# mmp/pbrt-v1

Hardware: AMD Instinct MI355X
Metric: Mrays/s (primary+secondary: every Scene::Intersect + Scene::IntersectP) (higher is better)
Workload: dtype f32

## Files before the change

include/pbrt_hip.h:

```cpp
#ifndef PBRT_HIP_H
#define PBRT_HIP_H
#include <stdint.h>
#include <stddef.h>
#ifdef __cplusplus
extern "C" {
#endif

#define RT_OK 0
#define RT_EINVAL (-1)
#define RT_EDEVICE (-2)
#define RT_ESTATE (-3)
#define RT_ENOMEM (-4)

typedef struct RtScene RtScene;

enum { RT_MAT_MATTE = 0, RT_MAT_MIRROR = 1, RT_MAT_GLASS = 2, RT_MAT_PLASTIC = 3, RT_MAT_UBER = 4, RT_MAT_SHINYMETAL = 5, RT_MAT_TRANSLUCENT = 6 };
typedef struct RtMaterial {
    int32_t type;
    float kd[3];
    float kt[3];
    float sigma;
    float ior;
    float ks[3];
    float roughness;
    float kr[3];
} RtMaterial;

enum { RT_LIGHT_POINT = 0, RT_LIGHT_AREA = 1, RT_LIGHT_SPOT = 2, RT_LIGHT_DISTANT = 3, RT_LIGHT_INFINITE = 4 };
typedef struct RtLight {
    int32_t type;
    float color[3];
    float pos[3];
    int32_t n_samples;
    uint32_t first_tri;
    uint32_t n_tris;
    int32_t reverse_orientation;
    int32_t flip_normal;
    float dir[3];
    float world_to_light[9];
    float cos_total_width, cos_falloff_start;
    int32_t quadric_plus1;
} RtLight;

enum { RT_CAMERA_PERSPECTIVE = 0, RT_CAMERA_ORTHOGRAPHIC = 1, RT_CAMERA_ENVIRONMENT = 2 };
typedef struct RtCamera {
    float raster_to_camera[16];
    float camera_to_world[16];
    float lens_radius, focal_distance, hither, yon;
    float shutter_open, shutter_close;
    int32_t type;
    int32_t x_res, y_res;
} RtCamera;

typedef struct RtVolume {
    int32_t present;
    float world_to_volume[16];
    float p0[3], p1[3];
    float sigma_a[3], sigma_s[3], le[3];
    float g;
} RtVolume;

enum { RT_DENSITY_NONE = 0, RT_DENSITY_EXPONENTIAL = 1, RT_DENSITY_GRID = 2 };
typedef struct RtDensityRegion {
    int32_t kind;
    float a, b;
    float updir[3];
    int32_t nx, ny, nz;
    const float *density;
} RtDensityRegion;

enum { RT_ACCEL_KDTREE = 0, RT_ACCEL_GRID = 1 };
typedef struct RtAccelParams {
    int32_t kind;
    int32_t isect_cost, trav_cost, max_prims, max_depth;
    float empty_bonus;
    int32_t build_threads;
} RtAccelParams;

enum { RT_QUADRIC_SPHERE = 0, RT_QUADRIC_DISK = 1, RT_QUADRIC_CYLINDER = 2, RT_QUADRIC_CONE = 3, RT_QUADRIC_PARABOLOID = 4, RT_QUADRIC_HYPERBOLOID = 5 };
typedef struct RtQuadric {
    int32_t type;
    float object_to_world[16], world_to_object[16];
    float radius, zmin, zmax, theta_min, theta_max, phi_max;
    float p1[3], p2[3], a, c;
} RtQuadric;

enum { RT_SHADING_UV = 1, RT_SHADING_N = 2, RT_SHADING_S = 4 };
typedef struct RtTriShading {
    uint32_t flags;
    uint32_t xform;
    float uv[6];
    float n[9];
    float s[9];
} RtTriShading;

typedef struct RtSceneDesc {
    uint32_t n_tris;
    const float *tri_verts;
    const uint16_t *tri_material;
    const int32_t *tri_light;
    const uint8_t *tri_flags;
    uint32_t n_materials;
    const RtMaterial *materials;
    uint32_t n_lights;
    const RtLight *lights;
    uint32_t n_light_tris;
    const float *light_tris;
    RtCamera camera;
    RtVolume volume;
    RtAccelParams accel;
    uint32_t n_quadrics;
    const RtQuadric *quadrics;
    const int32_t *tri_shading;
    uint32_t n_shading;
    const RtTriShading *shading;
    uint32_t n_xforms;
    const float *xforms;
} RtSceneDesc;

enum { RT_INTEGRATOR_WHITTED = 0, RT_INTEGRATOR_DIRECT = 1, RT_INTEGRATOR_PATH = 2 };
enum { RT_STRATEGY_ALL = 0, RT_STRATEGY_ONE = 1, RT_STRATEGY_WEIGHTED = 2 };
enum { RT_VOLUME_NONE = 0, RT_VOLUME_EMISSION = 1, RT_VOLUME_SINGLE = 2 };
enum { RT_SAMPLER_STRATIFIED = 0, RT_SAMPLER_LOWDISCREPANCY = 1, RT_SAMPLER_RANDOM = 2 };

typedef struct RtRenderDesc {
    int32_t integrator, max_depth, strategy;
    int32_t volume_integrator;
    float step_size;
    int32_t sampler, x_samples, y_samples, jitter, pixel_samples;
    uint32_t seed;
    int32_t x_res, y_res;
    int32_t x_pixel_start, y_pixel_start, x_pixel_count, y_pixel_count;
    int32_t x_start, x_end, y_start, y_end;
    float filter_x_width, filter_y_width;
    float filter_table[256];
    int32_t shard_index, shard_count, tile_pixels;
} RtRenderDesc;

typedef struct RtCounters {
    uint64_t camera_rays;
    uint64_t closest_rays;
    uint64_t any_rays;
    uint64_t nodes_visited;
    uint64_t leaf_refs;
    uint64_t tri_tests;
    uint64_t bad_samples;
    uint64_t stack_overflows;
} RtCounters;

typedef struct RtRay { float o[3], d[3], mint, maxt; } RtRay;
typedef struct RtHit { int32_t prim; float t, b1, b2; } RtHit;
typedef struct RtAccelInfo {
    uint32_t n_nodes, n_leaf_refs, max_depth, n_tris;
    float bounds[6];
    double build_seconds;
    int32_t kind;
    int32_t grid_nvoxels[3];
    float grid_width[3], grid_inv_width[3];
} RtAccelInfo;

const char *rt_last_error(void);
int rt_device_count(int *count);

int rt_scene_create(const RtSceneDesc *desc, int device, RtScene **out);
typedef struct RtPrebuiltAccel {
    int32_t kind;
    uint32_t n_nodes, n_leaf_refs, max_depth;
    const uint32_t *nodes;
    const uint32_t *leaf_refs;
    float bounds[6];
    int32_t grid_nvoxels[3]; float grid_width[3], grid_inv_width[3];
} RtPrebuiltAccel;
int rt_scene_create_prebuilt(const RtSceneDesc *desc, int device, const RtPrebuiltAccel *accel, RtScene **out);
int rt_scene_set_density(RtScene *s, const RtDensityRegion *region);
int rt_scene_destroy(RtScene *s);
int rt_scene_set_stream(RtScene *s, void *hip_stream);
int rt_scene_accel_info(const RtScene *s, RtAccelInfo *info);
int rt_scene_accel_copy(const RtScene *s, uint32_t *nodes, uint32_t *leaf_refs);

typedef struct RtKdTree RtAccel;
int rt_accel_build(const float *tri_verts, uint32_t n_tris, const RtAccelParams *params, RtAccel **out);
int rt_accel_info(const RtAccel *t, RtAccelInfo *info);
int rt_accel_copy(const RtAccel *t, uint32_t *nodes, uint32_t *leaf_refs);
typedef struct RtLeafLayoutInfo { uint64_t n_nodes, n_slots, n_entries; uint32_t stride, pad; } RtLeafLayoutInfo;
int rt_accel_leaf_layout(const RtAccel *t, int runs, int copies, uint32_t *tnodes, uint32_t *slot_prim, uint32_t *entries, RtLeafLayoutInfo *info);
int rt_accel_destroy(RtAccel *t);
typedef struct RtKdTree RtKdTree;
int rt_kdtree_build(const float *tri_verts, uint32_t n_tris, const RtAccelParams *params, RtKdTree **out);
int rt_kdtree_info(const RtKdTree *t, RtAccelInfo *info);
int rt_kdtree_copy(const RtKdTree *t, uint32_t *nodes, uint32_t *leaf_refs);
int rt_kdtree_destroy(RtKdTree *t);

int rt_camera_rays(RtScene *s, const RtRenderDesc *rd, uint64_t first, uint32_t count, RtRay *rays_out);
int rt_trace_closest(RtScene *s, const RtRay *rays, uint32_t n, RtHit *hits_out);
int rt_trace_any(RtScene *s, const RtRay *rays, uint32_t n, uint8_t *occluded_out);

int rt_film_bind(RtScene *s, void *device_accum, int32_t x_pixel_count, int32_t y_pixel_count);
int rt_film_clear(RtScene *s);
int rt_film_read(RtScene *s, float *host_accum);
int rt_film_resolve(RtScene *s, int premultiply_alpha, float *rgb_out, float *alpha_out);

int rt_render(RtScene *s, const RtRenderDesc *rd);
int rt_sync(RtScene *s);
int rt_samples_read(RtScene *s, uint64_t first, uint64_t count, float *out);
int rt_counters(RtScene *s, RtCounters *out);
int rt_counters_reset(RtScene *s);
int rt_set_counting(RtScene *s, int enabled);
int rt_last_render_ms(RtScene *s, float *total_ms, float *kernel_ms);
typedef struct RtRenderStats {
    float total_ms, render_ms, trace_ms, gather_ms;
    int32_t pipeline, iterations, timed_iterations;
    uint32_t slots;
    float shade_ms;
    int32_t bands;
    float march_ms;
    uint64_t weighted_points;
    float weighted_ms[5];
} RtRenderStats;
int rt_film_resolve_device(RtScene *s, const float *dev_accum, uint64_t n, int premultiply, float *dev_rgb, float *dev_alpha);
int rt_film_resolve_device_rgba(RtScene *s, const float *dev_accum, uint64_t n, int premultiply, float *dev_rgba);
int rt_film_pack_parts(RtScene *s, const float *dev_accum, int32_t w, int32_t h, int32_t world, int32_t rows, float *dev_parts);
int rt_last_render_stats(RtScene *s, RtRenderStats *out);

#ifdef __cplusplus
}
#endif
#endif
```

pbrt-v1_amd/__init__.py:

```python
from __future__ import annotations

import ctypes as C
import os
import subprocess
import numpy as np

_HERE = os.path.dirname(os.path.abspath(__file__))
LIB_DIR = os.path.join(_HERE, "lib")
HIP_LIB = os.path.join(LIB_DIR, "libpbrt_hip.so")
if os.environ.get("PBRT_HIP_TUNE") and os.environ.get("PBRT_HIP_LIB_PATH"):
    HIP_LIB = os.environ["PBRT_HIP_LIB_PATH"]
HOST_LIB = os.path.join(LIB_DIR, "libpbrt_host.so")
CSRC = os.path.join(_HERE, "csrc")

HIPCC_FLAGS = ["--offload-arch=gfx950", "-O3", "-std=c++17", "-ffp-contract=off", "-fno-slp-vectorize", "-fPIC", "-shared",
               "-Wno-unused-value"]
HOST_FLAGS = ["-O2", "-std=c++17", "-fPIC", "-shared", "-msse2", "-mfpmath=sse", "-fvisibility=hidden", "-fvisibility-inlines-hidden"]


HIP_UNITS = ("rt_kernels.hip", "rt_scene.hip", "rt_film.hip", "rt_trace.hip", "rt_mega_w.hip", "rt_mega_d.hip", "rt_mega_dw.hip", "rt_mega_p.hip", "rt_pipe_w.hip", "rt_pipe_d.hip",
             "rt_pipe_p.hip", "rt_pipe_v.hip", "rt_march.hip", "kd_build.cpp", "grid_build.cpp", "leaf_layout.cpp")


def build(force: bool = False, verbose: bool = False, defines=(), jobs: int | None = None) -> None:
    from concurrent.futures import ThreadPoolExecutor
    os.makedirs(LIB_DIR, exist_ok=True)
    obj_dir = os.path.join(LIB_DIR, "obj")
    os.makedirs(obj_dir, exist_ok=True)
    hip_dir = os.path.join(CSRC, "hip")
    hip_dep = [os.path.join(hip_dir, f) for f in os.listdir(hip_dir)] + [os.path.join(_HERE, "..", "include", "pbrt_hip.h")]
    headers = [d for d in hip_dep if d.endswith((".h", ".inc"))]
    host_src = [os.path.join(CSRC, "host", "scene_api.cpp")]
    host_dep = [os.path.join(CSRC, "host", f) for f in os.listdir(os.path.join(CSRC, "host"))] + \
               [os.path.join(_HERE, "..", "include", f) for f in ("pbrt_hip.h", "pbrt_hip_desc.h", "pbrt_hip_plugin.h", "pbrt_hip_material.h")]

    def stale(out, deps):
        return force or not os.path.exists(out) or any(os.path.getmtime(d) > os.path.getmtime(out) for d in deps)

    def closure(path, seen=None):
        import re
        seen = set() if seen is None else seen
        if path in seen or not os.path.exists(path):
            return seen
        seen.add(path)
        for inc in re.findall(r'^\s*#\s*include\s+"([^"]+)"', open(path).read(), re.M):
            closure(os.path.normpath(os.path.join(os.path.dirname(path), inc)), seen)
        return seen

    stamp = os.path.join(obj_dir, "defines.txt")
    dtext = " ".join(HIPCC_FLAGS) + " | " + " ".join(HOST_FLAGS) + " | " + " ".join(defines)
    if (open(stamp).read() if os.path.exists(stamp) else "") != dtext:
        force = True
    todo = []
    for u in HIP_UNITS:
        obj = os.path.join(obj_dir, u.rsplit(".", 1)[0] + ".o")
        if stale(obj, sorted(closure(os.path.join(hip_dir, u)))):
            todo.append(["hipcc"] + [f for f in HIPCC_FLAGS if f != "-shared"] + list(defines) + ["-c", os.path.join(hip_dir, u), "-o", obj])
    if todo:
        def run(cmd):
            if verbose:
                print(" ".join(cmd))
            if not cmd[-3].endswith(".hip"):
                subprocess.check_call(cmd)
                return
            r = subprocess.run(cmd + ["-Rpass-analysis=kernel-resource-usage"], capture_output=True, text=True)
            keep = [ln for ln in r.stderr.splitlines() if "remark:" in ln and any(k in ln for k in ("Function Name", " VGPRs:", "VGPRs Spill", "Occupancy", "ScratchSize", "LDS Size"))]
            open(cmd[-1][:-2] + ".resources.txt", "w").write("\n".join(keep) + "\n")
            if r.returncode != 0:
                raise RuntimeError("hipcc failed:\n" + r.stderr[-4000:])
        with ThreadPoolExecutor(max_workers=jobs or min(len(todo), os.cpu_count() or 4)) as ex:
            list(ex.map(run, todo))
        open(stamp, "w").write(dtext)
    objs = [os.path.join(obj_dir, u.rsplit(".", 1)[0] + ".o") for u in HIP_UNITS]
    if stale(HIP_LIB, objs):
        cmd = ["hipcc", "--offload-arch=gfx950", "-shared", "-fPIC"] + objs + ["-o", HIP_LIB]
        if verbose:
            print(" ".join(cmd))
        subprocess.check_call(cmd)
    if stale(HOST_LIB, host_dep):
        cmd = ["g++"] + HOST_FLAGS + host_src + ["-Wl,--version-script=" + os.path.join(CSRC, "host", "exports.map"), "-ldl", "-o", HOST_LIB]
        if verbose:
            print(" ".join(cmd))
        subprocess.check_call(cmd)


class RtCounters(C.Structure):
    _fields_ = [(n, C.c_uint64) for n in ("camera_rays", "closest_rays", "any_rays", "nodes_visited", "leaf_refs",
                                          "tri_tests", "bad_samples", "stack_overflows")]

    def as_dict(self):
        return {n: int(getattr(self, n)) for n, _ in self._fields_}


class RtAccelInfo(C.Structure):
    _fields_ = [("n_nodes", C.c_uint32), ("n_leaf_refs", C.c_uint32), ("max_depth", C.c_uint32), ("n_tris", C.c_uint32),
                ("bounds", C.c_float * 6), ("build_seconds", C.c_double), ("kind", C.c_int32),
                ("grid_nvoxels", C.c_int32 * 3), ("grid_width", C.c_float * 3), ("grid_inv_width", C.c_float * 3)]


class RtLeafLayoutInfo(C.Structure):
    _fields_ = [("n_nodes", C.c_uint64), ("n_slots", C.c_uint64), ("n_entries", C.c_uint64), ("stride", C.c_uint32), ("pad", C.c_uint32)]


class RtPrebuiltAccel(C.Structure):
    _fields_ = [("kind", C.c_int32), ("n_nodes", C.c_uint32), ("n_leaf_refs", C.c_uint32), ("max_depth", C.c_uint32),
                ("nodes", C.c_void_p), ("leaf_refs", C.c_void_p), ("bounds", C.c_float * 6),
                ("grid_nvoxels", C.c_int32 * 3), ("grid_width", C.c_float * 3), ("grid_inv_width", C.c_float * 3)]


class RtRenderStats(C.Structure):
    _fields_ = [("total_ms", C.c_float), ("render_ms", C.c_float), ("trace_ms", C.c_float), ("gather_ms", C.c_float),
                ("pipeline", C.c_int32), ("iterations", C.c_int32), ("timed_iterations", C.c_int32), ("slots", C.c_uint32), ("shade_ms", C.c_float), ("bands", C.c_int32), ("march_ms", C.c_float),
                ("weighted_points", C.c_uint64), ("weighted_ms", C.c_float * 5)]

    def as_dict(self):
        return {n: (list(getattr(self, n)) if n == "weighted_ms" else getattr(self, n)) for n, _ in self._fields_}


class RtVolume(C.Structure):
    _fields_ = [("present", C.c_int32), ("world_to_volume", C.c_float * 16), ("p0", C.c_float * 3), ("p1", C.c_float * 3),
                ("sigma_a", C.c_float * 3), ("sigma_s", C.c_float * 3), ("le", C.c_float * 3), ("g", C.c_float)]


class RtDensityRegion(C.Structure):
    _fields_ = [("kind", C.c_int32), ("a", C.c_float), ("b", C.c_float), ("updir", C.c_float * 3),
                ("nx", C.c_int32), ("ny", C.c_int32), ("nz", C.c_int32), ("density", C.POINTER(C.c_float))]


RT_MATERIAL_NAMES = ("matte", "mirror", "glass", "plastic", "uber", "shinymetal", "translucent")


class RtMaterial(C.Structure):
    _fields_ = [("type", C.c_int32), ("kd", C.c_float * 3), ("kt", C.c_float * 3), ("sigma", C.c_float), ("ior", C.c_float),
                ("ks", C.c_float * 3), ("roughness", C.c_float), ("kr", C.c_float * 3)]


class RtMaterialLobes(C.Structure):
    _fields_ = [(n, C.c_float * 3) for n in ("eta_ks", "eta_kr", "r_kd", "t_kd", "r_ks", "t_ks")] + \
               [(n, C.c_int32) for n in ("has_dr", "has_dt", "has_gr", "has_gt")]


RT_DENSITY_NAMES = {1: "exponential", 2: "volumegrid"}

RT_LIGHT_NAMES = ("point", "area", "spot", "distant", "infinite")


class RtLight(C.Structure):
    _fields_ = [("type", C.c_int32), ("color", C.c_float * 3), ("pos", C.c_float * 3), ("n_samples", C.c_int32), ("first_tri", C.c_uint32),
                ("n_tris", C.c_uint32), ("reverse_orientation", C.c_int32), ("flip_normal", C.c_int32), ("dir", C.c_float * 3),
                ("world_to_light", C.c_float * 9), ("cos_total_width", C.c_float), ("cos_falloff_start", C.c_float), ("quadric_plus1", C.c_int32)]

RAY_DTYPE = np.dtype([("o", np.float32, 3), ("d", np.float32, 3), ("mint", np.float32), ("maxt", np.float32)])
HIT_DTYPE = np.dtype([("prim", np.int32), ("t", np.float32), ("b1", np.float32), ("b2", np.float32)])

_hip = None
_host = None


def code_id(path: str | None = None) -> str:
    import hashlib, struct
    data = open(path or HIP_LIB, "rb").read()
    if data[:4] != b"\x7fELF" or data[4] != 2:
        raise RuntimeError("not a 64-bit ELF file: " + (path or HIP_LIB))
    shoff, = struct.unpack_from("<Q", data, 0x28)
    shentsize, shnum, shstrndx = struct.unpack_from("<HHH", data, 0x3A)
    def sh(i):
        name, typ, flags, addr, off, size = struct.unpack_from("<IIQQQQ", data, shoff + i * shentsize)
        return name, off, size
    _, stroff, _ = sh(shstrndx)
    h = hashlib.sha256()
    found = False
    for i in range(shnum):
        name, off, size = sh(i)
        end = data.index(b"\0", stroff + name)
        if data[stroff + name:end] == b".hip_fatbin":
            h.update(data[off:off + size]); found = True
    if not found:
        raise RuntimeError("no .hip_fatbin section in " + (path or HIP_LIB))
    return h.hexdigest()[:16]


def hip_lib():
    global _hip
    if _hip is None:
        if not os.path.exists(HIP_LIB):
            raise RuntimeError("libpbrt_hip.so is not built (run __graft_entry__.build()); there is no CPU fallback")
        L = C.CDLL(HIP_LIB)
        L.rt_last_error.restype = C.c_char_p
        for name in ("rt_scene_create", "rt_scene_destroy", "rt_scene_set_stream", "rt_scene_accel_info",
                     "rt_scene_accel_copy", "rt_camera_rays", "rt_trace_closest", "rt_trace_any", "rt_film_bind",
                     "rt_film_clear", "rt_film_read", "rt_film_resolve", "rt_render", "rt_sync", "rt_counters",
                     "rt_counters_reset", "rt_last_render_ms", "rt_last_render_stats", "rt_samples_read", "rt_device_count", "rt_set_counting",
                     "rt_kdtree_build", "rt_kdtree_info", "rt_kdtree_copy", "rt_kdtree_destroy",
                     "rt_accel_build", "rt_accel_info", "rt_accel_copy", "rt_accel_destroy", "rt_scene_create_prebuilt", "rt_film_resolve_device",
                     "rt_film_resolve_device_rgba", "rt_film_pack_parts", "rt_accel_leaf_layout", "rt_scene_set_density"):
            getattr(L, name).restype = C.c_int
        L.rt_scene_create.argtypes = [C.c_void_p, C.c_int, C.POINTER(C.c_void_p)]
        L.rt_scene_set_density.argtypes = [C.c_void_p, C.c_void_p]
        L.rt_scene_create_prebuilt.argtypes = [C.c_void_p, C.c_int, C.POINTER(RtPrebuiltAccel), C.POINTER(C.c_void_p)]
        L.rt_scene_destroy.argtypes = [C.c_void_p]
        L.rt_scene_set_stream.argtypes = [C.c_void_p, C.c_void_p]
        L.rt_scene_accel_info.argtypes = [C.c_void_p, C.POINTER(RtAccelInfo)]
        L.rt_scene_accel_copy.argtypes = [C.c_void_p, C.c_void_p, C.c_void_p]
        L.rt_camera_rays.argtypes = [C.c_void_p, C.c_void_p, C.c_uint64, C.c_uint32, C.c_void_p]
        L.rt_trace_closest.argtypes = [C.c_void_p, C.c_void_p, C.c_uint32, C.c_void_p]
        L.rt_trace_any.argtypes = [C.c_void_p, C.c_void_p, C.c_uint32, C.c_void_p]
        L.rt_film_bind.argtypes = [C.c_void_p, C.c_void_p, C.c_int32, C.c_int32]
        L.rt_film_clear.argtypes = [C.c_void_p]
        L.rt_film_read.argtypes = [C.c_void_p, C.c_void_p]
        L.rt_film_resolve.argtypes = [C.c_void_p, C.c_int, C.c_void_p, C.c_void_p]
        L.rt_render.argtypes = [C.c_void_p, C.c_void_p]
        L.rt_film_resolve_device.argtypes = [C.c_void_p, C.c_void_p, C.c_uint64, C.c_int, C.c_void_p, C.c_void_p]
        L.rt_film_resolve_device_rgba.argtypes = [C.c_void_p, C.c_void_p, C.c_uint64, C.c_int, C.c_void_p]
        L.rt_film_pack_parts.argtypes = [C.c_void_p, C.c_void_p, C.c_int32, C.c_int32, C.c_int32, C.c_int32, C.c_void_p]
        L.rt_sync.argtypes = [C.c_void_p]
        L.rt_counters.argtypes = [C.c_void_p, C.POINTER(RtCounters)]
        L.rt_counters_reset.argtypes = [C.c_void_p]
        L.rt_last_render_ms.argtypes = [C.c_void_p, C.POINTER(C.c_float), C.POINTER(C.c_float)]
        L.rt_last_render_stats.argtypes = [C.c_void_p, C.POINTER(RtRenderStats)]
        L.rt_samples_read.argtypes = [C.c_void_p, C.c_uint64, C.c_uint64, C.c_void_p]
        L.rt_device_count.argtypes = [C.POINTER(C.c_int)]
        L.rt_set_counting.argtypes = [C.c_void_p, C.c_int]
        L.rt_kdtree_build.argtypes = [C.c_void_p, C.c_uint32, C.c_void_p, C.POINTER(C.c_void_p)]
        L.rt_kdtree_info.argtypes = [C.c_void_p, C.POINTER(RtAccelInfo)]
        L.rt_kdtree_copy.argtypes = [C.c_void_p, C.c_void_p, C.c_void_p]
        L.rt_kdtree_destroy.argtypes = [C.c_void_p]
        L.rt_accel_build.argtypes = [C.c_void_p, C.c_uint32, C.c_void_p, C.POINTER(C.c_void_p)]
        L.rt_accel_info.argtypes = [C.c_void_p, C.POINTER(RtAccelInfo)]
        L.rt_accel_copy.argtypes = [C.c_void_p, C.c_void_p, C.c_void_p]
        L.rt_accel_destroy.argtypes = [C.c_void_p]
        L.rt_accel_leaf_layout.argtypes = [C.c_void_p, C.c_int, C.c_int, C.c_void_p, C.c_void_p, C.c_void_p, C.POINTER(RtLeafLayoutInfo)]
        _hip = L
    return _hip


def host_lib():
    global _host
    if _host is None:
        if not os.path.exists(HOST_LIB):
            raise RuntimeError("libpbrt_host.so is not built (run __graft_entry__.build())")
        L = C.CDLL(HOST_LIB)
        L.pbrt_host_parse_file.restype = C.c_void_p
        L.pbrt_host_parse_file.argtypes = [C.c_char_p, C.c_int]
        L.pbrt_host_parse_string.restype = C.c_void_p
        L.pbrt_host_parse_string.argtypes = [C.c_char_p, C.c_int]
        L.pbrt_host_free.argtypes = [C.c_void_p]
        L.pbrt_host_frame_count.argtypes = [C.c_void_p]
        L.pbrt_host_frame_valid.argtypes = [C.c_void_p, C.c_int]
        L.pbrt_host_scene_desc.restype = C.c_void_p
        L.pbrt_host_scene_desc.argtypes = [C.c_void_p, C.c_int]
        L.pbrt_host_render_desc.restype = C.c_void_p
        L.pbrt_host_render_desc.argtypes = [C.c_void_p, C.c_int]
        L.pbrt_host_premultiply.argtypes = [C.c_void_p, C.c_int]
        L.pbrt_host_filename.restype = C.c_char_p
        L.pbrt_host_filename.argtypes = [C.c_void_p, C.c_int]
        L.pbrt_host_set_shard.argtypes = [C.c_void_p, C.c_int, C.c_int, C.c_int]
        L.pbrt_host_set_seed.argtypes = [C.c_void_p, C.c_uint]
        L.pbrt_host_film_dims.argtypes = [C.c_void_p, C.POINTER(C.c_int * 8)]
        L.pbrt_host_scene_counts.argtypes = [C.c_void_p, C.POINTER(C.c_uint * 4)]
        L.pbrt_host_camera.restype = C.POINTER(C.c_float)
        L.pbrt_host_camera.argtypes = [C.c_void_p]
        L.pbrt_host_tri_verts.restype = C.POINTER(C.c_float)
        L.pbrt_host_tri_verts.argtypes = [C.c_void_p]
        L.pbrt_host_write_exr.argtypes = [C.c_char_p, C.c_void_p, C.c_void_p] + [C.c_int] * 6
        L.pbrt_host_read_exr_info.argtypes = [C.c_char_p, C.POINTER(C.c_int * 6)]
        L.pbrt_host_read_exr.argtypes = [C.c_char_p, C.c_void_p, C.c_void_p]
        L.pbrt_host_format_f32.restype = C.c_longlong
        L.pbrt_host_format_f32.argtypes = [C.c_void_p, C.c_longlong, C.c_int, C.c_void_p, C.c_longlong]
        L.pbrt_host_format_iota.restype = C.c_longlong
        L.pbrt_host_format_iota.argtypes = [C.c_longlong, C.c_longlong, C.c_int, C.c_void_p, C.c_longlong]
        L.pbrt_host_accel_params.restype = C.c_void_p
        L.pbrt_host_accel_params.argtypes = [C.c_void_p]
        L.pbrt_host_volume.restype = C.POINTER(RtVolume)
        L.pbrt_host_volume.argtypes = [C.c_void_p]
        L.pbrt_host_density_desc.restype = C.POINTER(RtDensityRegion)
        L.pbrt_host_density_desc.argtypes = [C.c_void_p, C.c_int]
        L.pbrt_host_materials.restype = C.POINTER(RtMaterial)
        L.pbrt_host_materials.argtypes = [C.c_void_p]
        L.pbrt_host_material_lobes.argtypes = [C.POINTER(RtMaterial), C.POINTER(RtMaterialLobes)]
        L.pbrt_host_lights.restype = C.POINTER(RtLight)
        L.pbrt_host_lights.argtypes = [C.c_void_p]
        _host = L
    return _host


def write_exr(path, rgb, alpha, total_res=None, offset=(0, 0)):
    rgb = np.ascontiguousarray(rgb, np.float32); alpha = np.ascontiguousarray(alpha, np.float32)
    h, w = alpha.shape
    tw, th = total_res if total_res else (w, h)
    if host_lib().pbrt_host_write_exr(path.encode(), rgb.ctypes.data, alpha.ctypes.data, w, h, tw, th, offset[0], offset[1]) != 0:
        raise IOError("cannot write " + path)


def read_exr(path):
    info = (C.c_int * 6)()
    if host_lib().pbrt_host_read_exr_info(path.encode(), C.byref(info)) != 0:
        raise IOError("cannot read " + path)
    w, h = info[0], info[1]
    rgb = np.zeros((h, w, 3), np.float32); alpha = np.zeros((h, w), np.float32)
    host_lib().pbrt_host_read_exr(path.encode(), rgb.ctypes.data, alpha.ctypes.data)
    return rgb, alpha, dict(total_res=(info[2], info[3]), offset=(info[4], info[5]))


TRI_SHADING_DTYPE = np.dtype([("flags", np.uint32), ("xform", np.uint32), ("uv", np.float32, 6), ("n", np.float32, 9), ("s", np.float32, 9)])


def shading_records(parsed):
    H = host_lib()
    H.pbrt_host_shading.restype = C.c_int
    H.pbrt_host_shading.argtypes = [C.c_void_p, C.POINTER(C.c_void_p), C.POINTER(C.c_void_p), C.POINTER(C.c_void_p), C.POINTER(C.c_uint), C.POINTER(C.c_uint)]
    idx, rec, xf, nrec, nxf = C.c_void_p(), C.c_void_p(), C.c_void_p(), C.c_uint(), C.c_uint()
    H.pbrt_host_shading(parsed.scene_desc, C.byref(idx), C.byref(rec), C.byref(xf), C.byref(nrec), C.byref(nxf))
    if not idx.value:
        return None, np.zeros(0, TRI_SHADING_DTYPE), np.zeros((0, 32), np.float32)
    i = np.ctypeslib.as_array(C.cast(idx, C.POINTER(C.c_int32)), shape=(parsed.n_tris,)).copy()
    r = np.frombuffer(C.string_at(rec, nrec.value * TRI_SHADING_DTYPE.itemsize), TRI_SHADING_DTYPE).copy()
    x = np.ctypeslib.as_array(C.cast(xf, C.POINTER(C.c_float)), shape=(nxf.value, 32)).copy() if nxf.value else np.zeros((0, 32), np.float32)
    return i, r, x


def format_f32(values, per_line: int = 9) -> str:
    v = np.ascontiguousarray(values, np.float32).ravel()
    buf = C.create_string_buffer(int(v.size) * 17 + 64)
    n = host_lib().pbrt_host_format_f32(v.ctypes.data, v.size, per_line, buf, len(buf))
    if n < 0:
        raise RuntimeError("format_f32: buffer too small")
    return buf.raw[:n].decode()


def format_iota(first: int, count: int, per_line: int = 3) -> str:
    buf = C.create_string_buffer(int(count) * 12 + 64)
    n = host_lib().pbrt_host_format_iota(first, count, per_line, buf, len(buf))
    if n < 0:
        raise RuntimeError("format_iota: buffer too small")
    return buf.raw[:n].decode()


def assemble_exr(paths, out) -> float:
    H = host_lib()
    H.pbrt_host_assemble_exr.restype = C.c_float
    H.pbrt_host_assemble_exr.argtypes = [C.c_char_p, C.c_char_p]
    r = H.pbrt_host_assemble_exr("\n".join(paths).encode(), out.encode())
    if r < 0:
        raise IOError("cannot assemble " + out)
    return float(r)


def publish_accel(ds: "DeviceScene", path: str) -> None:
    info = ds.accel_info()
    need = 256 + 8 * int(info.n_nodes) + 4 * int(info.n_leaf_refs)
    st = os.statvfs(os.path.dirname(path) or ".")
    if st.f_bavail * st.f_frsize < need + (64 << 20):
        raise OSError("publish_accel: %s has %d MB free, the accelerator needs %d MB" % (os.path.dirname(path), st.f_bavail * st.f_frsize >> 20, need >> 20))
    nodes, refs = ds.accel_arrays()
    tmp = path + ".tmp%d" % os.getpid()
    try:
        with open(tmp, "wb") as f:
            f.write(bytes(info).ljust(256, b"\0"))
            np.ascontiguousarray(nodes, np.uint32).tofile(f); np.ascontiguousarray(refs, np.uint32).tofile(f)
        os.replace(tmp, path)
    except BaseException:
        if os.path.exists(tmp):
            os.remove(tmp)
        raise


def attach_accel(path: str):
    raw = np.memmap(path, dtype=np.uint8, mode="r")
    info = RtAccelInfo.from_buffer_copy(bytes(raw[:C.sizeof(RtAccelInfo)]))
    nodes = np.frombuffer(raw, np.uint32, count=2 * info.n_nodes, offset=256).reshape(-1, 2)
    refs = np.frombuffer(raw, np.uint32, count=info.n_leaf_refs, offset=256 + 8 * info.n_nodes)
    return nodes, refs, info


class RtError(RuntimeError):
    pass


def _chk(rc):
    if rc != 0:
        raise RtError("rt error %d: %s" % (rc, hip_lib().rt_last_error().decode()))


def device_count() -> int:
    n = C.c_int(0)
    rc = hip_lib().rt_device_count(C.byref(n))
    return int(n.value) if rc == 0 else 0


def build_kdtree(tri_verts: np.ndarray, accel_params_ptr=None):
    tv = np.ascontiguousarray(tri_verts, np.float32).reshape(-1, 9)
    t = C.c_void_p()
    _chk(hip_lib().rt_accel_build(tv.ctypes.data, len(tv), accel_params_ptr, C.byref(t)))
    info = RtAccelInfo()
    _chk(hip_lib().rt_accel_info(t, C.byref(info)))
    nodes = np.zeros((info.n_nodes, 2), np.uint32)
    refs = np.zeros(max(info.n_leaf_refs, 1), np.uint32)
    _chk(hip_lib().rt_accel_copy(t, nodes.ctypes.data, refs.ctypes.data))
    hip_lib().rt_accel_destroy(t)
    return nodes, refs[:info.n_leaf_refs], np.array(list(info.bounds), np.float32), info


def leaf_layout(tri_verts: np.ndarray, accel_params_ptr=None, runs: bool = False, copies: bool = False):
    tv = np.ascontiguousarray(tri_verts, np.float32).reshape(-1, 9)
    t = C.c_void_p()
    _chk(hip_lib().rt_accel_build(tv.ctypes.data, len(tv), accel_params_ptr, C.byref(t)))
    try:
        info = RtAccelInfo()
        _chk(hip_lib().rt_accel_info(t, C.byref(info)))
        nodes = np.zeros((info.n_nodes, 2), np.uint32)
        refs = np.zeros(max(info.n_leaf_refs, 1), np.uint32)
        _chk(hip_lib().rt_accel_copy(t, nodes.ctypes.data, refs.ctypes.data))
        li = RtLeafLayoutInfo()
        _chk(hip_lib().rt_accel_leaf_layout(t, int(runs), int(copies), None, None, None, C.byref(li)))
        tn = np.zeros((li.n_nodes, 2), np.uint32); sp = np.zeros(max(li.n_slots, 1), np.uint32); en = np.zeros(max(li.n_entries, 1), np.uint32)
        _chk(hip_lib().rt_accel_leaf_layout(t, int(runs), int(copies), tn.ctypes.data, sp.ctypes.data, en.ctypes.data, C.byref(li)))
    finally:
        hip_lib().rt_accel_destroy(t)
    return nodes, refs[:info.n_leaf_refs], tn, sp[:li.n_slots], en[:li.n_entries], int(li.stride)


def fit_tile(extent: int, size: int) -> int:
    best = None
    for t in range(max(1, size * 3 // 4), max(2, size * 5 // 4) + 1):
        pad = -(-extent // t) * t - extent
        key = (pad, abs(t - size))
        if best is None or key < best[0]:
            best = (key, t)
    return best[1]


class ParsedScene:

    def __init__(self, text: str | None = None, path: str | None = None, quiet: bool = True, frame: int = 0):
        H = host_lib()
        if path is not None:
            self._h = H.pbrt_host_parse_file(path.encode(), int(quiet))
        else:
            from . import scenes as _scenes
            text = _scenes.for_product(text)
            self._h = H.pbrt_host_parse_string(text.encode(), int(quiet))
        self.warnings = H.pbrt_host_warnings()
        self.errors = H.pbrt_host_errors()
        self.n_frames = H.pbrt_host_frame_count(self._h)
        if self.n_frames == 0:
            raise RtError("scene description has no WorldEnd (errors: %d)" % self.errors)
        self.frame = frame
        self.valid = bool(H.pbrt_host_frame_valid(self._h, frame))
        self.scene_desc = H.pbrt_host_scene_desc(self._h, frame)
        self.render_desc = H.pbrt_host_render_desc(self._h, frame)
        self.premultiply = bool(H.pbrt_host_premultiply(self._h, frame))
        dims = (C.c_int * 8)()
        H.pbrt_host_film_dims(self.render_desc, C.byref(dims))
        self.width, self.height = dims[0], dims[1]
        self.sample_extent = (dims[2], dims[3], dims[4], dims[5])
        self.spp = dims[6]
        self.integrator = dims[7]
        cnt = (C.c_uint * 4)()
        H.pbrt_host_scene_counts(self.scene_desc, C.byref(cnt))
        self.n_tris, self.n_materials, self.n_lights, self.n_light_tris = (int(c) for c in cnt)

    @property
    def n_camera_samples(self) -> int:
        x0, x1, y0, y1 = self.sample_extent
        return (x1 - x0) * (y1 - y0) * self.spp

    def set_shard(self, index: int, count: int, tile_pixels=64, fit: bool = False):
        if isinstance(tile_pixels, (tuple, list)):
            w, h = int(tile_pixels[0]), int(tile_pixels[1])
            if fit:
                x0, x1, y0, y1 = self.sample_extent
                w, h = fit_tile(x1 - x0, w), fit_tile(y1 - y0, h)
            used = (w, h)
            tile_pixels = -(w | (h << 16))
        else:
            used = int(tile_pixels)
        host_lib().pbrt_host_set_shard(self.render_desc, index, count, int(tile_pixels))
        return used

    def set_seed(self, seed: int):
        host_lib().pbrt_host_set_seed(self.render_desc, seed)

    def camera_matrices(self):
        p = host_lib().pbrt_host_camera(self.scene_desc)
        a = np.ctypeslib.as_array(p, shape=(32,)).copy()
        return a[:16].reshape(4, 4), a[16:].reshape(4, 4)

    def accel_params_ptr(self):
        return host_lib().pbrt_host_accel_params(self.scene_desc)

    def accel_params(self) -> dict:
        a = np.ctypeslib.as_array(C.cast(self.accel_params_ptr(), C.POINTER(C.c_int32)), shape=(7,))
        return {"kind": int(a[0]), "isect_cost": int(a[1]), "trav_cost": int(a[2]), "max_prims": int(a[3]), "max_depth": int(a[4]),
                "empty_bonus": float(a[5:6].view(np.float32)[0]), "build_threads": int(a[6])}

    def render_view(self) -> dict:
        a = np.ctypeslib.as_array(C.cast(self.render_desc, C.POINTER(C.c_int32)), shape=(11,))
        return {"integrator": int(a[0]), "max_depth": int(a[1]), "strategy": int(a[2]), "volume_integrator": int(a[3]),
                "step_size": float(a[4:5].view(np.float32)[0]), "sampler": int(a[5]), "x_samples": int(a[6]), "y_samples": int(a[7]),
                "jitter": int(a[8]), "pixel_samples": int(a[9]), "seed": int(a[10:11].view(np.uint32)[0])}

    def volume(self) -> dict | None:
        v = host_lib().pbrt_host_volume(self.scene_desc).contents
        if not v.present:
            return None
        out = {"world_to_volume": np.array(v.world_to_volume, np.float32).reshape(4, 4), "p0": list(v.p0), "p1": list(v.p1),
               "sigma_a": list(v.sigma_a), "sigma_s": list(v.sigma_s), "le": list(v.le), "g": float(v.g), "density": None}
        dp = self.density_desc()
        if dp:
            d = dp.contents
            dens = {"kind": RT_DENSITY_NAMES[d.kind]}
            if d.kind == 1:
                dens.update(a=float(d.a), b=float(d.b), updir=[float(x) for x in d.updir])
            else:
                dens.update(nx=int(d.nx), ny=int(d.ny), nz=int(d.nz),
                            values=np.ctypeslib.as_array(d.density, shape=(d.nz, d.ny, d.nx)).copy())
            out["density"] = dens
        return out

    def materials(self) -> list:
        H = host_lib()
        tab = H.pbrt_host_materials(self.scene_desc)
        f3 = lambda a: np.array(list(a), np.float32)
        out = []
        for i in range(self.n_materials):
            m = tab[i]
            name = RT_MATERIAL_NAMES[m.type]
            d = {"type": name}
            if name == "matte":
                d.update(Kd=f3(m.kd), sigma=float(m.sigma))
            elif name == "mirror":
                d.update(Kr=f3(m.kd))
            elif name == "glass":
                d.update(Kr=f3(m.kd), Kt=f3(m.kt), index=float(m.ior))
            elif name == "plastic":
                d.update(Kd=f3(m.kd), Ks=f3(m.ks), roughness=float(m.roughness))
            elif name == "uber":
                d.update({"opacity*Kd": f3(m.kd), "opacity*Ks": f3(m.ks), "opacity*Kr": f3(m.kr), "1-opacity": f3(m.kt), "roughness": float(m.roughness)})
            else:
                lb = RtMaterialLobes()
                H.pbrt_host_material_lobes(C.byref(m), C.byref(lb))
                if name == "shinymetal":
                    d.update(Ks=f3(m.ks), Kr=f3(m.kr), roughness=float(m.roughness), eta_Ks=f3(lb.eta_ks), eta_Kr=f3(lb.eta_kr),
                             lobes=["glossy_reflection", "specular_reflection"])
                else:
                    d.update({"Kd": f3(m.kd), "Ks": f3(m.ks), "reflect": f3(m.kr), "transmit": f3(m.kt), "roughness": float(m.roughness),
                              "reflect*Kd": f3(lb.r_kd), "transmit*Kd": f3(lb.t_kd), "reflect*Ks": f3(lb.r_ks), "transmit*Ks": f3(lb.t_ks)})
                    d["lobes"] = [n for n, on in (("diffuse_reflection", lb.has_dr), ("diffuse_transmission", lb.has_dt),
                                                  ("glossy_reflection", lb.has_gr), ("glossy_transmission", lb.has_gt)) if on]
            out.append(d)
        return out

    def lights(self) -> list:
        tab = host_lib().pbrt_host_lights(self.scene_desc)
        f3 = lambda a: np.array(list(a), np.float32)
        out = []
        for i in range(self.n_lights):
            l = tab[i]
            name = RT_LIGHT_NAMES[l.type]
            d = {"type": name, "nsamples": int(l.n_samples), ("I" if name in ("point", "spot") else "L"): f3(l.color)}
            if name in ("point", "spot"):
                d["from"] = f3(l.pos)
            elif name == "distant":
                d["dir"] = f3(l.dir)
            elif name == "area":
                d["n_tris"] = int(l.n_tris)
            out.append(d)
        return out

    def density_desc(self):
        return host_lib().pbrt_host_density_desc(self._h, self.frame)

    def kdtree(self):
        return build_kdtree(self.tri_verts(), self.accel_params_ptr())

    def tri_verts(self):
        if self.n_tris == 0:
            return np.zeros((0, 3, 3), np.float32)
        p = host_lib().pbrt_host_tri_verts(self.scene_desc)
        return np.ctypeslib.as_array(p, shape=(self.n_tris, 3, 3)).copy()

    def serialize(self) -> bytes:
        H = host_lib()
        H.pbrt_host_serialize.restype = C.c_longlong
        H.pbrt_host_serialize.argtypes = [C.c_void_p, C.c_int, C.c_void_p, C.c_longlong]
        n = H.pbrt_host_serialize(self._h, self.frame, None, 0)
        buf = C.create_string_buffer(int(n))
        H.pbrt_host_serialize(self._h, self.frame, buf, n)
        return buf.raw

    def close(self):
        if self._h:
            host_lib().pbrt_host_free(self._h)
            self._h = None

    def __del__(self):
        try:
            self.close()
        except Exception:
            pass


class DeviceScene:

    def __init__(self, parsed: ParsedScene, device: int = -1, prebuilt=None):
        self.parsed = parsed
        self._s = C.c_void_p()
        if prebuilt is None:
            _chk(hip_lib().rt_scene_create(parsed.scene_desc, device, C.byref(self._s)))
        else:
            nodes, refs, info = prebuilt
            nodes = np.ascontiguousarray(nodes, np.uint32); refs = np.ascontiguousarray(refs if len(refs) else np.zeros(1, np.uint32), np.uint32)
            pa = RtPrebuiltAccel(kind=info.kind, n_nodes=info.n_nodes, n_leaf_refs=info.n_leaf_refs, max_depth=info.max_depth,
                                 nodes=nodes.ctypes.data, leaf_refs=refs.ctypes.data)
            for i in range(6): pa.bounds[i] = info.bounds[i]
            for i in range(3):
                pa.grid_nvoxels[i] = info.grid_nvoxels[i]; pa.grid_width[i] = info.grid_width[i]; pa.grid_inv_width[i] = info.grid_inv_width[i]
            _chk(hip_lib().rt_scene_create_prebuilt(parsed.scene_desc, device, C.byref(pa), C.byref(self._s)))
        dens = parsed.density_desc()
        if dens:
            rc = hip_lib().rt_scene_set_density(self._s, dens)
            if rc != 0:
                err = hip_lib().rt_last_error().decode(errors="replace")
                hip_lib().rt_scene_destroy(self._s); self._s = C.c_void_p()
                raise RtError("rt_scene_set_density failed (%d): %s" % (rc, err))
        self._film_bound = False

    def accel_info(self) -> RtAccelInfo:
        info = RtAccelInfo()
        _chk(hip_lib().rt_scene_accel_info(self._s, C.byref(info)))
        return info

    def accel_arrays(self):
        info = self.accel_info()
        nodes = np.zeros((info.n_nodes, 2), np.uint32)
        refs = np.zeros(max(info.n_leaf_refs, 1), np.uint32)
        _chk(hip_lib().rt_scene_accel_copy(self._s, nodes.ctypes.data, refs.ctypes.data))
        return nodes, refs[:info.n_leaf_refs]

    def set_stream(self, stream_ptr: int):
        _chk(hip_lib().rt_scene_set_stream(self._s, C.c_void_p(stream_ptr)))

    def bind_film(self, device_ptr: int | None = None):
        _chk(hip_lib().rt_film_bind(self._s, C.c_void_p(device_ptr) if device_ptr else None,
                                     self.parsed.width, self.parsed.height))
        self._film_bound = True

    def clear_film(self):
        _chk(hip_lib().rt_film_clear(self._s))

    def render(self, sync: bool = True):
        if not self._film_bound:
            self.bind_film()
        _chk(hip_lib().rt_render(self._s, self.parsed.render_desc))
        if sync:
            self.sync()

    def sync(self):
        _chk(hip_lib().rt_sync(self._s))

    def resolve_device(self, accum_ptr: int, n: int, rgb_ptr: int, alpha_ptr: int, premultiply: bool | None = None):
        pm = self.parsed.premultiply if premultiply is None else premultiply
        _chk(hip_lib().rt_film_resolve_device(self._s, C.c_void_p(accum_ptr), n, int(pm), C.c_void_p(rgb_ptr), C.c_void_p(alpha_ptr)))

    def resolve_device_rgba(self, accum_ptr: int, n: int, rgba_ptr: int, premultiply: bool | None = None):
        pm = self.parsed.premultiply if premultiply is None else premultiply
        _chk(hip_lib().rt_film_resolve_device_rgba(self._s, C.c_void_p(accum_ptr), n, int(pm), C.c_void_p(rgba_ptr)))

    def pack_parts(self, accum_ptr: int, world: int, rows: int, parts_ptr: int):
        _chk(hip_lib().rt_film_pack_parts(self._s, C.c_void_p(accum_ptr), self.parsed.width, self.parsed.height, world, rows, C.c_void_p(parts_ptr)))

    def film_accum(self) -> np.ndarray:
        out = np.zeros((5, self.parsed.height, self.parsed.width), np.float32)
        _chk(hip_lib().rt_film_read(self._s, out.ctypes.data))
        return out

    def film(self, premultiply: bool | None = None, out=None):
        h, w = self.parsed.height, self.parsed.width
        if out is None:
            rgb = np.empty((h, w, 3), np.float32); alpha = np.empty((h, w), np.float32)
        else:
            rgb, alpha = out
            if rgb.shape != (h, w, 3) or alpha.shape != (h, w) or rgb.dtype != np.float32 or alpha.dtype != np.float32 \
                    or not rgb.flags.c_contiguous or not alpha.flags.c_contiguous:
                raise ValueError("film(out=...): need C-contiguous float32 arrays of shape (H,W,3) and (H,W)")
        pm = self.parsed.premultiply if premultiply is None else premultiply
        _chk(hip_lib().rt_film_resolve(self._s, int(pm), rgb.ctypes.data, alpha.ctypes.data))
        return rgb, alpha

    def counters(self) -> dict:
        c = RtCounters()
        _chk(hip_lib().rt_counters(self._s, C.byref(c)))
        return c.as_dict()

    def set_counting(self, enabled: bool):
        _chk(hip_lib().rt_set_counting(self._s, int(enabled)))

    def reset_counters(self):
        _chk(hip_lib().rt_counters_reset(self._s))

    def last_ms(self):
        a, b = C.c_float(0), C.c_float(0)
        _chk(hip_lib().rt_last_render_ms(self._s, C.byref(a), C.byref(b)))
        return float(a.value), float(b.value)

    def samples(self, first: int = 0, count: int | None = None) -> np.ndarray:
        n = self.parsed.n_camera_samples - first if count is None else count
        out = np.zeros((n, 8), np.float32)
        _chk(hip_lib().rt_samples_read(self._s, first, n, out.ctypes.data))
        return out

    def last_stats(self) -> dict:
        st = RtRenderStats()
        _chk(hip_lib().rt_last_render_stats(self._s, C.byref(st)))
        return st.as_dict()

    def camera_rays(self, first: int, count: int) -> np.ndarray:
        rays = np.zeros(count, RAY_DTYPE)
        _chk(hip_lib().rt_camera_rays(self._s, self.parsed.render_desc, first, count, rays.ctypes.data))
        return rays

    def trace_closest(self, rays: np.ndarray) -> np.ndarray:
        rays = np.ascontiguousarray(rays, RAY_DTYPE)
        hits = np.zeros(len(rays), HIT_DTYPE)
        _chk(hip_lib().rt_trace_closest(self._s, rays.ctypes.data, len(rays), hits.ctypes.data))
        return hits

    def trace_any(self, rays: np.ndarray) -> np.ndarray:
        rays = np.ascontiguousarray(rays, RAY_DTYPE)
        occ = np.zeros(len(rays), np.uint8)
        _chk(hip_lib().rt_trace_any(self._s, rays.ctypes.data, len(rays), occ.ctypes.data))
        return occ

    def close(self):
        if self._s:
            hip_lib().rt_scene_destroy(self._s)
            self._s = C.c_void_p()

    def __del__(self):
        try:
            self.close()
        except Exception:
            pass


def render_text(scene_text: str, device: int = -1):
    ps = ParsedScene(text=scene_text)
    ds = DeviceScene(ps, device)
    ds.render()
    rgb, alpha = ds.film()
    cnt = ds.counters()
    ms = ds.last_ms()[0]
    ds.close()
    return rgb, alpha, cnt, ms
```

pbrt-v1_amd/csrc/hip/rt_device.h:

```cpp
#pragma once
#include "rt_math.h"
#include "../../../include/pbrt_hip.h"

namespace rt {

struct DevTri { float4 q0, q1, q2; };
#define RT_PRIM_QUADRIC (1u << 17)
struct DevQuadric {
    float w2o[16], o2w[16];
    float radius, zmin, zmax, theta_min, theta_max, phi_max;
    int type, pad;
    float p1[3], p2[3], a, c;
};

#define RT_PRIM_SHADING (1u << 18)
struct DevTriShading {
    unsigned flags, xform;
    float uv[6];
    float dpdu[3];
    float n[9], s[9];
    float pad[3];
};

struct DevMaterial {
    int type;
    float r[3];
    float t[3];
    float on_a, on_b;
    float ior;
    int has_r, has_t;
    float ks[3];
    float exponent;
    float kr[3];
    int has_g, has_kr;
};

struct DevLight {
    int type;
    float color[3];
    float pos[3];
    int n_samples;
    unsigned first_tri, n_tris;
    int reverse_orientation, flip_normal;
    float area;
    float dir[3];
    int quadric;
    float w2l[9];
    float cos_total, cos_falloff;
};

#define RT_MAX_DIM_REQ 12
struct DimReq { unsigned f_base, u_base; unsigned short n; unsigned short dims; };

struct DevScene {
    const DevTri *tris;
    const DevQuadric *quadrics;
    const float4 *tri_shade;
    const uint2 *nodes;
    const uint2 *tnodes;
    const uint4 *tpairs;
    unsigned root_x, root_y;
    unsigned top_pairs, leaf_runs;
    const float4 *ltris;
    const unsigned *lrefs;
    const unsigned *leaf_refs;
    const int *tri_shading_idx;
    const DevTriShading *tri_shading;
    const float *xforms;
    const DevMaterial *materials;
    const DevLight *lights;
    const float *light_tris;
    unsigned n_tris, n_lights;
    float bounds[6];
    int accel_kind;
    int nvox[3];
    float gwidth[3], ginv_width[3];
    RtCamera cam;
    RtVolume vol;
    int dens_kind;
    float dens_a, dens_b, dens_up[3];
    int dens_n[3];
    const float *dens_grid;
    int n_infinite;
};

#define RT_INTEG_DIRECT_WEIGHTED 3

struct DevFrame {
    int integrator, max_depth, strategy, volume_integrator;
    float step_size;
    int sampler, xs, ys, jitter, spp;
    unsigned seed;
    int x_pixel_start, y_pixel_start, x_pixel_count, y_pixel_count;
    int x_start, x_end, y_start, y_end;
    float fxw, fyw, inv_fxw, inv_fyw;
    const float *filter_table;
    float *accum;
    float4 *samples;
    int shard_index, shard_count, tile_pixels;
    int tile_w, tile_h, tiles_x;
    int dbg_x, dbg_y;
    int exit_thresh;
    int phase_sync;
    int high_occupancy;
    int leaf_min;
    int mega_tile;
    int xcd_bands;
    int trav_mode;
    int pipeline;
    unsigned long long total_work;
    unsigned long long total_pixels;
    int n1d, n2d;
    unsigned lhs_total;
    unsigned pixgen_draws;
    DimReq one_d[RT_MAX_DIM_REQ];
    DimReq two_d[RT_MAX_DIM_REQ];
    const DimReq *light_dims;
    int dims_max_n;
    unsigned long long *work_counter;
    unsigned long long *counters;
    uint2 *spill;
    float *frames;
    float *vol_rays, *vol_state, *vol_samp;
    int vol_nmax;
    unsigned n_threads;
    int weighted_phase;
    unsigned *wt_base;
    float *wt_rec;
    float2 *wt_pick;
    int wt_mixed;
    unsigned wt_nd;
    const unsigned *wt_recbase;
    int dens_cap;
#ifdef RT_TAIL_PROBE
    unsigned long long *probe;
#endif
};

#if defined(__HIP_DEVICE_COMPILE__)
#define RT_G __attribute__((address_space(1)))
#define RT_L __attribute__((address_space(3)))
#else
#define RT_G
#define RT_L
#endif
typedef const DevMaterial RT_G &MatRef;
typedef const DevLight RT_G &LightRef;
#define RT_MAT(sc, i) (*((const DevMaterial RT_G *)(sc).materials + (i)))
#define RT_LIGHT(sc, i) (*((const DevLight RT_G *)(sc).lights + (i)))
#define RT_GPTR(T, p) ((T RT_G *)(p))

#define RT_SAMPLE_XY 1
__host__ __device__ inline unsigned long long sample_slot(unsigned lp, unsigned s, int spp) {
    return ((unsigned long long)(lp >> 6) * unsigned(spp) + s) * 128ull + (lp & 63u) * 2u;
}

}
```

pbrt-v1_amd/csrc/hip/rt_host.h:

```cpp
#pragma once
#include "rt_render_kernel.h"
#include "rt_pipeline.h"
#include "rt_pipe_vertex.h"
#include "rt_pipe_march.h"
#include "rt_internal.h"
#include <cstdio>
#include <cstdlib>
#include <cstring>
#include <string>
#include <vector>
#include <cmath>
#include <chrono>
#include <atomic>
#include <thread>

namespace rt {
const char *knob(const char *name);
int fail(int code, const std::string &msg);
const char *last_error();
void hip_warn(hipError_t e, const char *what);
}
using namespace rt;
#define HIPCHK(expr)                                                                                   \
    do {                                                                                               \
        hipError_t e_ = (expr);                                                                        \
        if (e_ != hipSuccess)                                                                          \
            return rt::fail(RT_EDEVICE, std::string(#expr) + ": " + hipGetErrorString(e_));            \
    } while (0)
#define HIPWARN(expr) rt::hip_warn((expr), #expr)

namespace rt { extern const RenderKernelFn g_render_kernels_whitted[16], g_render_kernels_direct[16], g_render_kernels_path[16], g_render_kernels_weighted[8]; }
namespace rt { extern const PipeShadeFn g_pipe_shade_whitted[6], g_pipe_shade_direct[6], g_pipe_shade_path[6]; extern const PipeTraceFn g_pipe_trace[8]; extern const PipeShadeFn g_pipe_vertex[3];
               extern const PipeMarchFn g_pipe_march[6]; }
static inline RenderKernelFn render_kernel_of(int variant) {
    const RenderKernelFn *t = (variant % 3 == 0) ? g_render_kernels_whitted : (variant % 3 == 1) ? g_render_kernels_direct : g_render_kernels_path;
    return t[variant < 24 ? variant / 3 : variant < 36 ? 8 + (variant - 24) / 3 : 12 + (variant - 36) / 3];
}

struct RtScene {
    int device = 0;
    hipStream_t stream = nullptr;
    bool own_stream = false;
    KdTree tree;
    GridAccelData gridacc;
    int accel_kind = RT_ACCEL_KDTREE;
    double per_leaf = -1.0;
    bool has_ext = false;
    DevScene dev{};
    std::vector<void *> allocs;
    float *accum = nullptr; bool own_accum = false; int film_w = 0, film_h = 0;
    float *filter_dev = nullptr;
    unsigned long long *work_counter = nullptr, *counters = nullptr;
    uint2 *spill = nullptr; size_t spill_entries = 0;
    float *frames = nullptr; size_t frames_floats = 0;
    unsigned grid = 0, n_threads = 0;
    unsigned grids[48] = {0};
    unsigned wgrids[8] = {0};
    DimReq *light_dims = nullptr; size_t light_dims_cap = 0;
    std::vector<DimReq> light_dims_host;
    const unsigned *light_draw_flags = nullptr; unsigned n_drawing_lights = 0;
    unsigned *wt_recbase = nullptr; size_t wt_recbase_cap = 0;
    unsigned n_infinite = 0;
    int light_draws = 0;
    unsigned *wt_base = nullptr; size_t wt_base_cap = 0; float *wt_rec = nullptr; size_t wt_rec_cap = 0; float2 *wt_pick = nullptr; size_t wt_pick_cap = 0;
    unsigned long long *wt_sums = nullptr;
    unsigned long long *wt_total = nullptr;
    unsigned long long wt_points = 0; bool last_weighted = false;
    hipEvent_t wt_ev[6] = {nullptr, nullptr, nullptr, nullptr, nullptr, nullptr};
    DevScene *dev_scene = nullptr; DevFrame *dev_frame = nullptr;
    float4 *samples = nullptr; size_t samples_cap = 0;
    int samples_spp = 1;
    unsigned long long samples_last = 0;
    float ms_render = 0.f, ms_gather = 0.f; hipEvent_t ev2 = nullptr;
    float *resolve_buf = nullptr; size_t resolve_cap = 0;
    float *vol_buf = nullptr; size_t vol_cap = 0;
    RtVolume volume{};
    int density_kind = RT_DENSITY_NONE;
    double vol_world[6] = {0, 0, 0, 0, 0, 0};
    bool rendered = false;
    int spill_depth = 0;
    hipEvent_t ev0 = nullptr, ev1 = nullptr;
    bool have_timing = false;
    bool counting = true;
    uint32_t n_tris = 0;
    size_t n_leaf_tri_units = 0, n_leaf_entries = 0;
    PipePool pool{}; unsigned pool_cap = 0; int pool_vec = 0; PipePool *dev_pool = nullptr;
    unsigned *h_qcount = nullptr;
    unsigned trace_grids[8] = {0}, march_grids[6] = {0};
    std::vector<hipEvent_t> pipe_ev;
    std::vector<hipEvent_t> pipe_fence;
    bool last_pipeline = false, last_marches = false; int pipe_iters = 0, pipe_timed = 0; unsigned pipe_slots = 0;
    float4 *trace_buf = nullptr; size_t trace_cap = 0;
    int n_cus = 0;
    unsigned *trace_qc = nullptr;
};
#define RT_PIPE_QN 4096
#define RT_PIPE_TIMED 256
#define RT_PIPE_BATCH 4

template <class T>
static inline int upload(RtScene *s, const T *host, size_t n, const T **dev) {
    void *p = nullptr;
    size_t bytes = (n ? n : 1) * sizeof(T);
    HIPCHK(hipMalloc(&p, bytes));
    s->allocs.push_back(p);
    if (n) HIPCHK(hipMemcpy(p, host, n * sizeof(T), hipMemcpyHostToDevice));
    *dev = static_cast<const T *>(p);
    return RT_OK;
}

template <class T>
static inline int ensure(RtScene *s, T **buf, size_t *cap, size_t need) {
    if (need <= *cap) return RT_OK;
    if (*buf) { HIPCHK(hipStreamSynchronize(s->stream)); HIPWARN(hipFree(*buf)); *buf = nullptr; *cap = 0; }
    HIPCHK(hipMalloc((void **)buf, need * sizeof(T)));
    *cap = need;
    return RT_OK;
}

template <class F> static inline int guarded(const char *what, F &&f) {
    try { return f(); }
    catch (const std::bad_alloc &) { return rt::fail(RT_ENOMEM, std::string(what) + ": out of host memory"); }
    catch (const std::exception &e) { return rt::fail(RT_ESTATE, std::string(what) + ": " + e.what()); }
}

struct FilmGather { int which = 0, grx = 0, gry = 0, cols = 0, rows = 0, slot_ncs = 0; size_t slot_lds = 0, col_bytes = 0; };
int film_gather_plan(RtScene *s, const rt::DevFrame &fr, FilmGather &g);
int film_gather_launch(RtScene *s, const rt::DevFrame &fr, const FilmGather &g, const rt::DevFrame *dfr, int row0, int row_end);
```

pbrt-v1_amd/csrc/hip/rt_kernels.hip:

```cpp
#include "rt_host.h"
#include "rt_weighted.h"

namespace rt {
__global__ void camera_kernel(DevScene sc, DevFrame fr, unsigned long long first, unsigned count, RtRay *out) {
    const unsigned i = blockIdx.x * blockDim.x + threadIdx.x;
    if (i >= count) return;
    const unsigned long long n = first + i;
    Lane ln; Ray r;
    setup_sample(sc, fr, ln, n / fr.spp, int(n % fr.spp), r);
    out[i].o[0] = r.o.x; out[i].o[1] = r.o.y; out[i].o[2] = r.o.z;
    out[i].d[0] = r.d.x; out[i].d[1] = r.d.y; out[i].d[2] = r.d.z;
    out[i].mint = r.mint; out[i].maxt = r.maxt;
}

}

namespace rt {
const char *knob(const char *name) {
#ifdef RT_NO_TUNABLES
    (void)name; return nullptr;
#else
    static const bool on = std::getenv("PBRT_HIP_TUNE") != nullptr;
    return on ? std::getenv(name) : nullptr;
#endif
}
static thread_local std::string g_err;
int fail(int code, const std::string &msg) { g_err = msg; return code; }
const char *last_error() { return g_err.c_str(); }
void hip_warn(hipError_t e, const char *what) {
    if (e != hipSuccess) std::fprintf(stderr, "libpbrt_hip: %s failed: %s\n", what, hipGetErrorString(e));
}
}

static int render_pipeline(RtScene *s, const RtRenderDesc *rd, DevFrame &fr, int vol_levels, int vol_nmax, size_t vol_samp_words) {
    const int integ = rd->integrator;
    bool by_vertex = integ == RT_INTEGRATOR_PATH && !s->volume.present;
    if (const char *e = knob("PBRT_HIP_PIPE_VERTEX")) by_vertex = by_vertex && std::atoi(e) != 0;
    const size_t frame_words = integ != RT_INTEGRATOR_PATH ? size_t(rd->max_depth + 2) * RT_FRAME_WORDS : 0;
    const size_t vol_words = s->volume.present ? size_t(vol_levels) * 8 + 13 + vol_samp_words : 0;
    const size_t slot_bytes = size_t(RT_PIPE_VEC) * 16 + 2 * 16 + 3 * 16 + 4 * 16 + 3 * 4 + (frame_words + vol_words) * 4;
    unsigned want = s->volume.present ? 1u << 25 : 1u << 23;
    {
        size_t free_b = 0, total_b = 0;
        HIPCHK(hipMemGetInfo(&free_b, &total_b));
        const size_t held = size_t(s->pool_cap) * (size_t(RT_PIPE_VEC) * 16 + 9 * 16 + 12) + (s->frames_floats + s->vol_cap) * 4;
        size_t budget = (free_b + held) / 2;
        if (const char *e = knob("PBRT_HIP_PIPE_MEM_MB")) budget = size_t(std::max(1, std::atoi(e))) << 20;
        if (slot_bytes * want > budget) want = unsigned(std::max<size_t>(budget / slot_bytes, 2 * RT_BLOCK));
    }
    if (const char *e = knob("PBRT_HIP_PIPE_SLOTS")) want = unsigned(std::max(256, std::atoi(e)));
    unsigned long long tw = fr.total_work ? fr.total_work : 1;
    unsigned n_slots = unsigned(std::min<unsigned long long>(want, tw));
    n_slots = (n_slots + RT_BLOCK - 1) / RT_BLOCK * RT_BLOCK;
    if (n_slots >= (1u << 30)) return fail(RT_EINVAL, "rt_render: more than 2^30 pipeline slots");
    const int vec = RT_PIPE_VEC;
    if (n_slots > s->pool_cap) {
        HIPCHK(hipStreamSynchronize(s->stream));
        HIPWARN(hipFree(s->pool.state)); HIPWARN(hipFree(s->pool.ray_o)); HIPWARN(hipFree(s->pool.hit)); HIPWARN(hipFree(s->pool.q_o)); HIPWARN(hipFree(s->pool.q_slot));
        { unsigned *qc = s->pool.q_count; unsigned long long *ww = s->pool.wave_work; s->pool = PipePool{}; s->pool.q_count = qc; s->pool.wave_work = ww; }
        s->pool_cap = 0;
        HIPCHK(hipMalloc((void **)&s->pool.state, size_t(vec) * n_slots * sizeof(float4)));
        HIPCHK(hipMalloc((void **)&s->pool.ray_o, size_t(2) * n_slots * sizeof(float4)));
        HIPCHK(hipMalloc((void **)&s->pool.hit, size_t(3) * n_slots * sizeof(float4)));
        HIPCHK(hipMalloc((void **)&s->pool.q_o, size_t(4) * n_slots * sizeof(float4)));
        HIPCHK(hipMalloc((void **)&s->pool.q_slot, size_t(3) * n_slots * sizeof(unsigned)));
        HIPWARN(hipFree(s->pool.wave_work)); s->pool.wave_work = nullptr;
        HIPCHK(hipMalloc((void **)&s->pool.wave_work, size_t(n_slots / 64 + 1) * 2 * sizeof(unsigned long long)));
        s->pool_cap = n_slots;
    }
    if (!s->pool.q_count) HIPCHK(hipMalloc((void **)&s->pool.q_count, size_t(RT_PIPE_QN) * RT_QC_STRIDE * sizeof(unsigned)));
    PipePool pl = s->pool;
    pl.n_slots = n_slots; pl.ray_d = pl.ray_o + n_slots; pl.q_d = pl.q_o + size_t(2) * n_slots; pl.q_march = pl.q_slot + size_t(2) * n_slots;
    if (by_vertex) pl.ray_d = pl.q_o;
    if (integ != RT_INTEGRATOR_PATH) {
        int rc = ensure(s, &s->frames, &s->frames_floats, frame_words * n_slots); if (rc) return rc;
    }
    if (s->volume.present) {
        int rc = ensure(s, &s->vol_buf, &s->vol_cap, vol_words * n_slots); if (rc) return rc;
        fr.vol_rays = s->vol_buf; fr.vol_state = s->vol_buf + size_t(vol_levels) * 8 * n_slots;
        fr.vol_samp = fr.vol_state + size_t(13) * n_slots; fr.vol_nmax = vol_nmax;
    }
    fr.frames = s->frames; fr.n_threads = n_slots;
    if (s->pipe_ev.empty()) {
        s->pipe_ev.resize(6 * RT_PIPE_TIMED); s->pipe_fence.resize(RT_PIPE_QN / RT_PIPE_BATCH);
        for (auto &e : s->pipe_ev) HIPCHK(hipEventCreate(&e));
        for (auto &e : s->pipe_fence) HIPCHK(hipEventCreateWithFlags(&e, hipEventDisableTiming));
    }
    const int f = s->counting ? 1 : (s->has_ext ? 2 : 0);
    const PipeShadeFn *st = integ == RT_INTEGRATOR_WHITTED ? g_pipe_shade_whitted : integ == RT_INTEGRATOR_DIRECT ? g_pipe_shade_direct : g_pipe_shade_path;
    const PipeShadeFn shade = by_vertex ? g_pipe_vertex[f] : st[(s->volume.present ? 3 : 0) + f];
    const int tk = (s->accel_kind == RT_ACCEL_GRID ? 4 : 0) + (s->counting ? (s->has_ext ? 1 : 3) : (s->has_ext ? 2 : 0));
    const PipeTraceFn trace = g_pipe_trace[tk];
    const unsigned trace_grid = s->trace_grids[tk];
    const bool marches = s->volume.present;
    const int mk = (s->accel_kind == RT_ACCEL_GRID ? 3 : 0) + f;
    const unsigned march_grid = s->march_grids[mk];
    HIPCHK(hipMemcpyAsync(s->dev_frame, &fr, sizeof(DevFrame), hipMemcpyHostToDevice, s->stream));
    HIPCHK(hipMemcpyAsync(s->dev_pool, &pl, sizeof(PipePool), hipMemcpyHostToDevice, s->stream));
    HIPCHK(hipMemsetAsync(s->work_counter, 0, sizeof(unsigned long long), s->stream));
    HIPCHK(hipMemsetAsync(pl.state + n_slots, 0, size_t(n_slots) * sizeof(float4), s->stream));
    HIPCHK(hipMemsetAsync(pl.wave_work, 0, size_t(n_slots / 64 + 1) * 2 * sizeof(unsigned long long), s->stream));
    HIPCHK(hipEventRecord(s->ev0, s->stream));
    int iter = 0, checked = 0, batch = 0;
    bool done = false;
    const int max_iters = 1 << 20;
    while (!done) {
        for (int k = 0; k < RT_PIPE_BATCH; ++k, ++iter) {
            const unsigned qi = unsigned(iter % RT_PIPE_QN);
            PipeLaunch pk{}; pk.qi = qi; pk.slot_base = 0; pk.q_base = 0;
            HIPCHK(hipMemsetAsync(pl.q_count + size_t(RT_QC_STRIDE) * qi, 0, RT_QC_STRIDE * sizeof(unsigned), s->stream));
            if (iter < RT_PIPE_TIMED) HIPCHK(hipEventRecord(s->pipe_ev[6 * iter + 2], s->stream));
            hipLaunchKernelGGL(shade, dim3(n_slots / RT_BLOCK), dim3(RT_BLOCK), 0, s->stream, (const DevScene *)s->dev_scene,
                               (const DevFrame *)s->dev_frame, (const PipePool *)s->dev_pool, pk);
            if (iter < RT_PIPE_TIMED) HIPCHK(hipEventRecord(s->pipe_ev[6 * iter + 3], s->stream));
            TraceJob job{};
            job.q_o = pl.q_o; job.q_d = pl.q_d; job.q_slot = pl.q_slot; job.q_count = pl.q_count + size_t(RT_QC_STRIDE) * qi; job.hit = pl.hit;
            job.n_slots = n_slots; job.q_base = pk.q_base; job.spill = s->spill; job.n_threads = s->n_threads; job.counters = s->counters;
            if (by_vertex) { job.by_slot = 1; job.q_o = pl.ray_o; job.q_d = pl.ray_d; }
            if (iter < RT_PIPE_TIMED) HIPCHK(hipEventRecord(s->pipe_ev[6 * iter], s->stream));
            hipLaunchKernelGGL(trace, dim3(trace_grid), dim3(RT_BLOCK), 0, s->stream, (const DevScene *)s->dev_scene, job);
            if (iter < RT_PIPE_TIMED) HIPCHK(hipEventRecord(s->pipe_ev[6 * iter + 1], s->stream));
            if (marches) {
                MarchJob mj{};
                mj.q_march = pl.q_march; mj.q_count = pl.q_count + size_t(RT_QC_STRIDE) * qi;
                mj.spill = s->spill; mj.n_threads = s->n_threads; mj.counters = s->counters;
                if (iter < RT_PIPE_TIMED) HIPCHK(hipEventRecord(s->pipe_ev[6 * iter + 4], s->stream));
                hipLaunchKernelGGL(g_pipe_march[mk], dim3(march_grid), dim3(RT_BLOCK), 0, s->stream, (const DevScene *)s->dev_scene, (const DevFrame *)s->dev_frame,
                                   (const PipePool *)s->dev_pool, mj);
                if (iter < RT_PIPE_TIMED) HIPCHK(hipEventRecord(s->pipe_ev[6 * iter + 5], s->stream));
            }
            HIPCHK(hipMemcpyAsync(s->h_qcount + size_t(RT_QC_STRIDE) * qi, pl.q_count + size_t(RT_QC_STRIDE) * qi, (RT_QC_MARCH + 1) * sizeof(unsigned), hipMemcpyDeviceToHost, s->stream));
        }
        HIPCHK(hipGetLastError());
        HIPCHK(hipEventRecord(s->pipe_fence[batch % (RT_PIPE_QN / RT_PIPE_BATCH)], s->stream));
        if (batch >= 1) {
            HIPCHK(hipEventSynchronize(s->pipe_fence[(batch - 1) % (RT_PIPE_QN / RT_PIPE_BATCH)]));
            for (int k = 0; k < RT_PIPE_BATCH; ++k, ++checked) {
                const unsigned *q = s->h_qcount + size_t(RT_QC_STRIDE) * (checked % RT_PIPE_QN);
                if (q[0] + q[RT_QC_ANY] + q[RT_QC_MARCH] == 0) { done = true; break; }
            }
        }
        ++batch;
        if (iter > max_iters) return fail(RT_ESTATE, "rt_render: the queue pipeline did not terminate");
    }
    s->last_marches = marches;
    s->pipe_slots = n_slots; s->pipe_iters = checked + 1; s->pipe_timed = std::min(s->pipe_iters, RT_PIPE_TIMED);
    HIPCHK(hipEventRecord(s->ev1, s->stream));
    s->last_pipeline = true;
    return RT_OK;
}

extern "C" {


const char *rt_last_error(void) { return rt::last_error(); }

int rt_device_count(int *count) {
    if (!count) return fail(RT_EINVAL, "rt_device_count: null");
    int n = 0;
    hipError_t e = hipGetDeviceCount(&n);
    if (e != hipSuccess) { *count = 0; return fail(RT_EDEVICE, std::string("hipGetDeviceCount: ") + hipGetErrorString(e)); }
    *count = n; return RT_OK;
}
static int make_frame(RtScene *s, const RtRenderDesc *rd, DevFrame &fr, bool need_film) {
    auto round_up_pow2 = [](unsigned v) { v--; v |= v >> 1; v |= v >> 2; v |= v >> 4; v |= v >> 8; v |= v >> 16; return v + 1; };
    if (rd->sampler < RT_SAMPLER_STRATIFIED || rd->sampler > RT_SAMPLER_RANDOM) return fail(RT_EINVAL, "unknown sampler");
    if (rd->sampler == RT_SAMPLER_LOWDISCREPANCY) { if (rd->pixel_samples < 1) return fail(RT_EINVAL, "bad pixelsamples"); }
    else if (rd->x_samples < 1 || rd->y_samples < 1) return fail(RT_EINVAL, "bad xsamples/ysamples");
    std::memset(&fr, 0, sizeof fr);
    fr.integrator = rd->integrator; fr.max_depth = rd->max_depth; fr.strategy = rd->strategy;
    fr.volume_integrator = rd->volume_integrator; fr.step_size = rd->step_size;
    fr.sampler = rd->sampler; fr.xs = rd->x_samples; fr.ys = rd->y_samples; fr.jitter = rd->jitter;
    fr.spp = rd->sampler == RT_SAMPLER_LOWDISCREPANCY ? int(round_up_pow2(unsigned(rd->pixel_samples))) : rd->x_samples * rd->y_samples;
    fr.seed = rd->seed;
    fr.x_pixel_start = rd->x_pixel_start; fr.y_pixel_start = rd->y_pixel_start;
    fr.x_pixel_count = rd->x_pixel_count; fr.y_pixel_count = rd->y_pixel_count;
    fr.x_start = rd->x_start; fr.x_end = rd->x_end; fr.y_start = rd->y_start; fr.y_end = rd->y_end;
    if (fr.x_end <= fr.x_start || fr.y_end <= fr.y_start) return fail(RT_EINVAL, "empty sample extent");
    fr.fxw = rd->filter_x_width; fr.fyw = rd->filter_y_width;
    fr.inv_fxw = 1.f / fr.fxw; fr.inv_fyw = 1.f / fr.fyw;
    fr.filter_table = s->filter_dev; fr.accum = s->accum;
    fr.shard_index = rd->shard_index; fr.shard_count = rd->shard_count < 1 ? 1 : rd->shard_count;
    fr.tile_pixels = rd->tile_pixels < 1 ? 1 : rd->tile_pixels;
    if (fr.shard_index < 0 || fr.shard_index >= fr.shard_count) return fail(RT_EINVAL, "bad shard index");
    fr.total_pixels = (unsigned long long)(fr.x_end - fr.x_start) * (unsigned long long)(fr.y_end - fr.y_start);
    if (fr.total_pixels * fr.spp > 0xFFFFFFFFull) return fail(RT_EINVAL, "more than 2^32 camera samples per frame");
    unsigned long long n_tiles = 0;
    if (rd->tile_pixels < 0) {
        const int tw = (-rd->tile_pixels) & 0xffff, th = (-rd->tile_pixels) >> 16;
        if (tw < 1 || th < 1 || tw > 4096 || th > 4096) return fail(RT_EINVAL, "bad 2-D tile size");
        fr.tile_w = tw; fr.tile_h = th; fr.tile_pixels = tw * th;
        fr.tiles_x = (fr.x_end - fr.x_start + tw - 1) / tw;
        n_tiles = (unsigned long long)fr.tiles_x * (unsigned long long)((fr.y_end - fr.y_start + th - 1) / th);
        if (n_tiles * fr.tile_pixels * fr.spp > 0xFFFFFFFFull) return fail(RT_EINVAL, "more than 2^32 camera samples per frame (2-D tiles, border tiles included)");
    } else n_tiles = (fr.total_pixels + fr.tile_pixels - 1) / fr.tile_pixels;
    const unsigned long long my_tiles = n_tiles > (unsigned long long)fr.shard_index
        ? (n_tiles - fr.shard_index + fr.shard_count - 1) / fr.shard_count : 0;
    fr.total_work = my_tiles * fr.tile_pixels * fr.spp;

    std::vector<int> n1, n2;
    const int nl = int(s->dev.n_lights);
    if (rd->integrator == RT_INTEGRATOR_DIRECT && rd->strategy == RT_STRATEGY_ALL) {
        std::vector<DevLight> lights(nl);
        if (nl) HIPCHK(hipMemcpy(lights.data(), s->dev.lights, nl * sizeof(DevLight), hipMemcpyDeviceToHost));
        for (int i = 0; i < nl; ++i) { int ns = lights[i].n_samples; if (rd->sampler == RT_SAMPLER_LOWDISCREPANCY) ns = int(round_up_pow2(unsigned(ns)));
            if (ns > 65535) return fail(RT_EINVAL, "rt_render: more than 65535 samples per light (the sample table holds counts in 16 bits)");
            n2.push_back(ns); n2.push_back(ns); n1.push_back(ns); }
    } else if (rd->integrator == RT_INTEGRATOR_DIRECT) { n2 = {1, 1}; n1 = {1, 1}; }
    else if (rd->integrator == RT_INTEGRATOR_PATH) { n1.assign(9, 1); n2.assign(9, 1); }
    else if (rd->integrator != RT_INTEGRATOR_WHITTED) return fail(RT_EINVAL, "unknown integrator");
    n1.push_back(1); n1.push_back(1);
    const bool all_lights = rd->integrator == RT_INTEGRATOR_DIRECT && rd->strategy == RT_STRATEGY_ALL;
    std::vector<DimReq> d1(n1.size()), d2(n2.size());
    unsigned c = 0;
    const unsigned P = unsigned(fr.spp);
    if (rd->sampler == RT_SAMPLER_STRATIFIED) {
        for (size_t i = 0; i < n1.size(); ++i) { d1[i] = DimReq{c, c + unsigned(n1[i]), (unsigned short)n1[i], 1}; c += 2u * n1[i]; }
        for (size_t i = 0; i < n2.size(); ++i) { d2[i] = DimReq{c, c + 2u * n2[i], (unsigned short)n2[i], 2}; c += 4u * n2[i]; }
        fr.lhs_total = c;
        fr.pixgen_draws = fr.jitter ? 7u * P : 2u * P;
    } else if (rd->sampler == RT_SAMPLER_RANDOM) {
        for (size_t i = 0; i < n1.size(); ++i) { d1[i] = DimReq{c, 0, (unsigned short)n1[i], 1}; c += unsigned(n1[i]); }
        for (size_t i = 0; i < n2.size(); ++i) { d2[i] = DimReq{c, 0, (unsigned short)n2[i], 2}; c += 2u * n2[i]; }
        fr.lhs_total = c;
        fr.pixgen_draws = 5u * P;
    } else {
        c = (2 + 2 * P) + (2 + 2 * P) + (1 + 2 * P);
        for (size_t i = 0; i < n1.size(); ++i) { d1[i] = DimReq{c, 0, (unsigned short)n1[i], 1}; c += 1u + unsigned(n1[i]) * P + P; }
        for (size_t i = 0; i < n2.size(); ++i) { d2[i] = DimReq{c, 0, (unsigned short)n2[i], 2}; c += 2u + unsigned(n2[i]) * P + P; }
        fr.lhs_total = 0;
        fr.pixgen_draws = c;
    }
    {
        unsigned long long draws = 0;
        for (int n : n1) draws += 2ull * unsigned(n) * (P + 1);
        for (int n : n2) draws += 4ull * unsigned(n) * (P + 1);
        if (draws > 0x3fffffffull) return fail(RT_EINVAL, "rt_render: the lights' sample requests need more than 2^30 random numbers per camera sample");
    }
    fr.light_dims = nullptr;
    fr.dims_max_n = 0;
    for (const DimReq &r : d2) fr.dims_max_n = std::max(fr.dims_max_n, int(r.n));
    if (all_lights) {
        std::vector<DimReq> tab(size_t(nl) * 3 + 1, DimReq{0, 0, 0, 0});
        for (int i = 0; i < nl; ++i) { tab[3 * size_t(i)] = d2[2 * size_t(i)]; tab[3 * size_t(i) + 1] = d2[2 * size_t(i) + 1]; tab[3 * size_t(i) + 2] = d1[size_t(i)]; }
        std::vector<DimReq> &up = s->light_dims_host;
        if (!s->light_dims || up.size() != tab.size() || std::memcmp(up.data(), tab.data(), tab.size() * sizeof(DimReq)) != 0) {
            int rc = ensure(s, &s->light_dims, &s->light_dims_cap, tab.size()); if (rc) return rc;
            up.swap(tab);
            HIPCHK(hipStreamSynchronize(s->stream));
            HIPCHK(hipMemcpy(s->light_dims, up.data(), up.size() * sizeof(DimReq), hipMemcpyHostToDevice));
        }
        fr.light_dims = s->light_dims;
        d1.erase(d1.begin(), d1.begin() + nl);
        d2.clear();
    }
    if (d1.size() > RT_MAX_DIM_REQ || d2.size() > RT_MAX_DIM_REQ) return fail(RT_ESTATE, "rt_render: sample table overflow");
    fr.n1d = int(d1.size()); fr.n2d = int(d2.size());
    std::memset(fr.one_d, 0, sizeof fr.one_d); std::memset(fr.two_d, 0, sizeof fr.two_d);
    for (size_t i = 0; i < d1.size(); ++i) fr.one_d[i] = d1[i];
    for (size_t i = 0; i < d2.size(); ++i) fr.two_d[i] = d2[i];
    {
        const size_t nn = s->tree.nodes.size();
        if (s->per_leaf < 0.0) {
            size_t leaves = 0, refs = 0;
            if (s->accel_kind == RT_ACCEL_KDTREE) for (const Node &n : s->tree.nodes) if ((n.x & 3u) == 3u && (n.x >> 2)) { ++leaves; refs += n.x >> 2; }
            s->per_leaf = leaves ? double(refs) / double(leaves) : 1.0;
        }
        const double per_leaf = s->per_leaf;
        const bool tiny = nn <= 4096 && per_leaf >= 1.5;
        const bool tiny_path = tiny && rd->integrator == RT_INTEGRATOR_PATH;
        fr.trav_mode = (tiny && !tiny_path) ? 3 : 2;
        fr.exit_thresh = tiny ? (rd->integrator == RT_INTEGRATOR_PATH ? 8 : 0) : 32;
        if (RT_MEGA_BYV && tiny && rd->integrator == RT_INTEGRATOR_PATH && !s->volume.present && !s->has_ext) fr.exit_thresh = 16;
        fr.high_occupancy = (tiny && !tiny_path) ? 0 : 1;
        if (const char *e = knob("PBRT_HIP_HIGH_OCC")) fr.high_occupancy = std::atoi(e);
        fr.leaf_min = tiny ? 8 : RT_TRACE_LEAF_MIN;
        if (const char *e = knob("PBRT_HIP_LEAF_MIN")) fr.leaf_min = std::max(1, std::atoi(e));
        if (const char *e = knob("PBRT_HIP_TRAV_MODE")) fr.trav_mode = std::atoi(e);
        fr.xcd_bands = rd->integrator != RT_INTEGRATOR_PATH ? 1 : 0;
        if (const char *e = knob("PBRT_HIP_XCD_BANDS")) fr.xcd_bands = std::atoi(e) != 0;
        if (const char *e = knob("PBRT_HIP_EXIT_THRESH")) fr.exit_thresh = std::atoi(e);
        fr.dbg_x = fr.dbg_y = -1000000;
        if (const char *e = knob("PBRT_HIP_DEBUG_PIXEL")) std::sscanf(e, "%d,%d", &fr.dbg_x, &fr.dbg_y);
        fr.phase_sync = tiny ? 1 : 0;
        if (const char *e = knob("PBRT_HIP_PHASE_SYNC")) fr.phase_sync = std::atoi(e);
        fr.pipeline = (!tiny && s->volume.present) ? 1 : 0;
        if (const char *e = knob("PBRT_HIP_PIPELINE")) fr.pipeline = std::atoi(e) != 0;
        if (fr.max_depth > 250 || fr.max_depth < 0) fr.pipeline = 0;
        if (fr.dims_max_n >= 65535) fr.pipeline = 0;
        if (s->dev.n_lights >= 65535u) fr.pipeline = 0;
        if (rd->integrator == RT_INTEGRATOR_DIRECT && rd->strategy == RT_STRATEGY_WEIGHTED) fr.pipeline = 0;
        if (fr.shard_count == 1 && !fr.pipeline) {
            fr.tile_w = fr.tile_h = fr.tiles_x = 0; fr.tile_pixels = 1;
            fr.total_work = fr.total_pixels * fr.spp;
            fr.mega_tile = 32;
            if (const char *e = knob("PBRT_HIP_MEGA_TILE")) fr.mega_tile = std::max(0, std::atoi(e));
            if (fr.mega_tile > 4096 || fr.total_work > 0xffffffffull) fr.mega_tile = 0;
        }
        if (fr.trav_mode != 3 || fr.high_occupancy) fr.trav_mode = 2;
    }
    fr.work_counter = s->work_counter; fr.counters = s->counters; fr.spill = s->spill; fr.n_threads = s->n_threads;
    fr.frames = s->frames;
    if (need_film && !s->accum) return fail(RT_ESTATE, "rt_render: no film bound (call rt_film_bind first)");
    if (need_film && (fr.x_pixel_count != s->film_w || fr.y_pixel_count != s->film_h))
        return fail(RT_EINVAL, "rt_render: film size does not match the bound film");
    return RT_OK;
}

int rt_camera_rays(RtScene *s, const RtRenderDesc *rd, uint64_t first, uint32_t count, RtRay *rays_out) {
    if (!s || !rd || !rays_out) return fail(RT_EINVAL, "null argument");
    HIPCHK(hipSetDevice(s->device));
    DevFrame fr; int rc = make_frame(s, rd, fr, false); if (rc) return rc;
    RtRay *dev = nullptr;
    HIPCHK(hipMalloc((void **)&dev, size_t(count ? count : 1) * sizeof(RtRay)));
    hipLaunchKernelGGL(camera_kernel, dim3((count + 255) / 256), dim3(256), 0, s->stream, s->dev, fr,
                       (unsigned long long)first, count, dev);
    HIPCHK(hipGetLastError());
    HIPCHK(hipStreamSynchronize(s->stream));
    HIPCHK(hipMemcpy(rays_out, dev, size_t(count) * sizeof(RtRay), hipMemcpyDeviceToHost));
    HIPWARN(hipFree(dev));
    return RT_OK;
}

static int trace_common(RtScene *s, const RtRay *rays, uint32_t n, int any, RtHit *hits, uint8_t *occ) {
    if (!s || !rays || (!hits && !occ)) return fail(RT_EINVAL, "null argument");
    HIPCHK(hipSetDevice(s->device));
    if (n == 0) return RT_OK;
    if (size_t(n) > s->trace_cap) {
        if (s->trace_buf) { HIPCHK(hipStreamSynchronize(s->stream)); HIPWARN(hipFree(s->trace_buf)); s->trace_buf = nullptr; s->trace_cap = 0; }
        HIPCHK(hipMalloc((void **)&s->trace_buf, size_t(n) * 3 * sizeof(float4))); s->trace_cap = n;
    }
    std::vector<float4> host(size_t(n) * 2);
    for (uint32_t i = 0; i < n; ++i) {
        host[i] = make_float4(rays[i].o[0], rays[i].o[1], rays[i].o[2], rays[i].mint);
        host[size_t(n) + i] = make_float4(rays[i].d[0], rays[i].d[1], rays[i].d[2], rays[i].maxt);
    }
    unsigned qc[RT_QC_STRIDE] = {0};
    qc[0] = any ? 0u : n; qc[RT_QC_ANY] = any ? n : 0u;
    HIPCHK(hipMemcpyAsync(s->trace_buf, host.data(), host.size() * sizeof(float4), hipMemcpyHostToDevice, s->stream));
    HIPCHK(hipMemcpyAsync(s->trace_qc, qc, sizeof qc, hipMemcpyHostToDevice, s->stream));
    TraceJob job{};
    job.q_o = s->trace_buf; job.q_d = s->trace_buf + n; job.q_slot = nullptr; job.q_count = s->trace_qc; job.hit = s->trace_buf + 2 * size_t(n);
    job.n_slots = 0; job.spill = s->spill; job.n_threads = s->n_threads; job.counters = s->counters;
    const int k = (s->accel_kind == RT_ACCEL_GRID ? 4 : 0) + (s->has_ext ? 1 : 3);
    HIPWARN(hipEventRecord(s->ev0, s->stream));
    hipLaunchKernelGGL(g_pipe_trace[k], dim3(s->trace_grids[k]), dim3(RT_BLOCK), 0, s->stream, (const DevScene *)s->dev_scene, job);
    HIPWARN(hipEventRecord(s->ev1, s->stream)); HIPWARN(hipEventRecord(s->ev2, s->stream)); s->have_timing = true; s->last_pipeline = false;
    HIPCHK(hipGetLastError());
    HIPCHK(hipMemcpyAsync(host.data(), s->trace_buf + 2 * size_t(n), size_t(n) * sizeof(float4), hipMemcpyDeviceToHost, s->stream));
    HIPCHK(hipStreamSynchronize(s->stream));
    for (uint32_t i = 0; i < n; ++i) {
        int prim; std::memcpy(&prim, &host[i].x, 4);
        if (any) occ[i] = prim >= 0 ? 1 : 0;
        else { hits[i].prim = prim; hits[i].t = host[i].y; hits[i].b1 = host[i].z; hits[i].b2 = host[i].w; }
    }
    return RT_OK;
}
int rt_trace_closest(RtScene *s, const RtRay *rays, uint32_t n, RtHit *hits_out) { return trace_common(s, rays, n, 0, hits_out, nullptr); }
int rt_trace_any(RtScene *s, const RtRay *rays, uint32_t n, uint8_t *occluded_out) { return trace_common(s, rays, n, 1, nullptr, occluded_out); }
int rt_render(RtScene *s, const RtRenderDesc *rd) {
    if (!s || !rd) return fail(RT_EINVAL, "null argument");
    HIPCHK(hipSetDevice(s->device));
    if (rd->integrator < RT_INTEGRATOR_WHITTED || rd->integrator > RT_INTEGRATOR_PATH) return fail(RT_EINVAL, "unknown integrator");
    if (rd->max_depth < 0) return fail(RT_EINVAL, "rt_render: negative maxdepth");
    if (!rd->filter_table) return fail(RT_EINVAL, "rt_render: no filter table");
    DevFrame fr; int rc = make_frame(s, rd, fr, true); if (rc) return rc;
    const bool weighted = rd->integrator == RT_INTEGRATOR_DIRECT && rd->strategy == RT_STRATEGY_WEIGHTED;
    if (rd->integrator == RT_INTEGRATOR_DIRECT && (rd->strategy < RT_STRATEGY_ALL || rd->strategy > RT_STRATEGY_WEIGHTED)) return fail(RT_EINVAL, "rt_render: unknown direct lighting strategy");
    if (weighted) {
        if (fr.shard_count != 1) return fail(RT_EINVAL, "rt_render: strategy \"weighted\" is a recurrence over the whole frame in the sampler's order (transport.cpp:71-122): one shard only");
        if (s->volume.present && s->light_draws != 0) return fail(RT_EINVAL, "rt_render: strategy \"weighted\" in a participating medium needs lights whose estimates draw no random numbers "
                                                                            "(point / spot / distant / single-triangle / quadric lights): an emitter of several triangles draws its triangle, and the medium makes "
                                                                            "the draw's position in the stream depend on occlusion");
        if (s->n_infinite != 0) return fail(RT_EINVAL, "rt_render: strategy \"weighted\" with an infinite light is not supported (the light draws a random number per estimate); "
                                                       "use strategy \"one\" or \"all\"");
        if (s->dev.n_lights > 2048u) return fail(RT_EINVAL, "rt_render: strategy \"weighted\" holds the per-light tables of its recurrence in LDS: at most 2048 lights");
        if (fr.total_work >= 0xffffffffull) return fail(RT_EINVAL, "rt_render: strategy \"weighted\": more than 2^32 - 2 camera samples in the frame");
    }
    const bool skip_film = knob("PBRT_HIP_DEBUG_NOFILM") != nullptr;
    FilmGather fg; rc = film_gather_plan(s, fr, fg); if (rc) return rc;
    int vol_levels = 0, vol_nmax = 0; size_t vol_samp_words = 0;
    fr.dens_cap = 0;
    if (s->volume.present) {
        if (!(rd->step_size > 0.f)) return fail(RT_EINVAL, "rt_render: volume integrator stepsize must be positive");
        if (rd->volume_integrator != RT_VOLUME_EMISSION && rd->volume_integrator != RT_VOLUME_SINGLE) return fail(RT_EINVAL, "rt_render: unknown volume integrator");
        const float ex = s->volume.p1[0] - s->volume.p0[0], ey = s->volume.p1[1] - s->volume.p0[1], ez = s->volume.p1[2] - s->volume.p0[2];
        const double diag = std::sqrt(double(ex) * ex + double(ey) * ey + double(ez) * ez);
        const double nsteps = std::ceil(diag / rd->step_size) + 2;
        if (nsteps > 65536) return fail(RT_EINVAL, "rt_render: stepsize too small for the medium (more than 65536 march steps)");
        vol_nmax = int(nsteps);
        if (s->density_kind != RT_DENSITY_NONE) {
            const double *wb = s->vol_world;
            const double wx = wb[3] - wb[0], wy = wb[4] - wb[1], wz = wb[5] - wb[2];
            const double wdiag = std::sqrt(wx * wx + wy * wy + wz * wz);
            const float half = .5f * rd->step_size;
            const double taus = std::ceil(wdiag / double(half)) + 2;
            if (taus > double(1 << 20)) return fail(RT_EINVAL, "rt_render: stepsize too small for the density region (an optical-depth march would take more than 2^20 samples)");
            double u[6] = {wb[0], wb[1], wb[2], wb[3], wb[4], wb[5]};
            const float *c2w = s->dev.cam.camera_to_world;
            const double cam[3] = {c2w[3], c2w[7], c2w[11]};
            for (int i = 0; i < 3; ++i) { u[i] = std::min(u[i], cam[i]); u[3 + i] = std::max(u[3 + i], cam[i]); }
            const float *sb = s->dev.bounds;
            if (sb[0] <= sb[3] && sb[1] <= sb[4] && sb[2] <= sb[5])
                for (int i = 0; i < 3; ++i) { u[i] = std::min(u[i], double(sb[i])); u[3 + i] = std::max(u[3 + i], double(sb[3 + i])); }
            const double ux = u[3] - u[0], uy = u[4] - u[1], uz = u[5] - u[2];
            const float tmax = std::nextafter(float(std::sqrt(ux * ux + uy * uy + uz * uz)), INFINITY);
            volatile float tv = tmax;
            const float adv = tv + half;
            if (!std::isfinite(tmax) || !(adv > tmax))
                return fail(RT_EINVAL, "rt_render: stepsize too small for the density region: at the scene's ray parameters t + .5 * stepsize == t, the optical-depth march would not advance");
            fr.dens_cap = int(taus);
            vol_nmax = std::max(vol_nmax, int(std::ceil(wdiag / rd->step_size)) + 2);
            if (vol_nmax > 65536) return fail(RT_EINVAL, "rt_render: stepsize too small for the medium (more than 65536 march steps)");
        }
        vol_levels = (rd->integrator == RT_INTEGRATOR_PATH) ? 1 : rd->max_depth + 2;
        vol_samp_words = rd->volume_integrator == RT_VOLUME_SINGLE ? size_t(3) * vol_nmax : 0;
    }
    {
        size_t cap = s->samples_cap;
        const size_t local_pixels = size_t(fr.total_work / fr.spp);
        const size_t need = ((local_pixels + 63) / 64 * 64 + 64) * size_t(fr.spp) * 2;
        rc = ensure(s, &s->samples, &cap, need); if (rc) return rc;
        if (cap != s->samples_cap) HIPCHK(hipMemsetAsync(s->samples, 0, cap * sizeof(float4), s->stream));
        s->samples_cap = cap;
    }
    fr.samples = s->samples; s->samples_last = fr.total_work; s->samples_spp = fr.spp;
    HIPCHK(hipMemcpyAsync(s->filter_dev, rd->filter_table, 256 * sizeof(float), hipMemcpyHostToDevice, s->stream));
    { hipError_t pre = hipGetLastError(); if (pre != hipSuccess) return fail(RT_EDEVICE, std::string("pending HIP error before launch: ") + hipGetErrorString(pre)); }
    s->rendered = true;
    if (fr.pipeline) {
        rc = render_pipeline(s, rd, fr, vol_levels, vol_nmax, vol_samp_words); if (rc) return rc;
        s->last_weighted = false;
    } else {
        if (rd->integrator != RT_INTEGRATOR_PATH) {
            rc = ensure(s, &s->frames, &s->frames_floats, size_t(rd->max_depth + 2) * RT_FRAME_WORDS * s->n_threads); if (rc) return rc;
            fr.frames = s->frames;
        }
        if (s->volume.present) {
            rc = ensure(s, &s->vol_buf, &s->vol_cap, (size_t(vol_levels) * 8 + 13 + vol_samp_words) * s->n_threads); if (rc) return rc;
            fr.vol_rays = s->vol_buf; fr.vol_state = s->vol_buf + size_t(vol_levels) * 8 * s->n_threads;
            fr.vol_samp = fr.vol_state + size_t(13) * s->n_threads; fr.vol_nmax = vol_nmax;
        }
        int variant = (((s->volume.present ? 1 : 0) * 2 + (s->accel_kind == RT_ACCEL_GRID ? 1 : 0)) * 2 + (s->counting ? 1 : 0)) * 3 + rd->integrator;
        if (fr.high_occupancy && !s->counting) variant = 24 + ((s->volume.present ? 1 : 0) * 2 + (s->accel_kind == RT_ACCEL_GRID ? 1 : 0)) * 3 + rd->integrator;
        if (s->has_ext && !s->counting) variant = 36 + ((s->volume.present ? 1 : 0) * 2 + (s->accel_kind == RT_ACCEL_GRID ? 1 : 0)) * 3 + rd->integrator;
        if (s->grids[variant] == 0) return fail(RT_ESTATE, "render kernel variant has no resident grid");
        fr.weighted_phase = 0; fr.wt_base = nullptr; fr.wt_rec = nullptr; fr.wt_pick = nullptr; fr.wt_mixed = 0; fr.wt_nd = 0; fr.wt_recbase = nullptr;
        if (weighted) {
            const int wk = ((s->volume.present ? 1 : 0) * 2 + (s->accel_kind == RT_ACCEL_GRID ? 1 : 0)) * 2 + (s->counting ? 1 : 0);
            const int nL = int(s->dev.n_lights), R = 1 + 2 * nL;
            if (!s->wt_total) { HIPCHK(hipHostMalloc((void **)&s->wt_total, sizeof(unsigned long long), hipHostMallocDefault)); HIPCHK(hipMalloc((void **)&s->wt_sums, RT_WSCAN_BLOCKS * sizeof(unsigned long long))); for (hipEvent_t &e : s->wt_ev) HIPCHK(hipEventCreate(&e)); }
            rc = ensure(s, &s->wt_base, &s->wt_base_cap, size_t(fr.total_work) + 1); if (rc) return rc;
            fr.wt_base = s->wt_base;
            auto pass = [&](int phase) -> int {
                fr.weighted_phase = phase;
                HIPCHK(hipMemcpyAsync(s->dev_frame, &fr, sizeof(DevFrame), hipMemcpyHostToDevice, s->stream));
                HIPCHK(hipMemsetAsync(s->work_counter, 0, 64 * sizeof(unsigned long long), s->stream));
                hipLaunchKernelGGL(g_render_kernels_weighted[wk], dim3(s->wgrids[wk]), dim3(RT_BLOCK), 0, s->stream, (const DevScene *)s->dev_scene, (const DevFrame *)s->dev_frame);
                HIPCHK(hipGetLastError());
                return RT_OK;
            };
            HIPCHK(hipEventRecord(s->ev0, s->stream));
            if ((rc = pass(1))) return rc;
            HIPCHK(hipEventRecord(s->wt_ev[0], s->stream));
            hipLaunchKernelGGL(weighted_scan_sums_kernel, dim3(RT_WSCAN_BLOCKS), dim3(RT_WSCAN_THREADS), 0, s->stream, (const unsigned *)s->wt_base, (unsigned long long)fr.total_work, s->wt_sums);
            hipLaunchKernelGGL(weighted_scan_top_kernel, dim3(1), dim3(RT_WSCAN_THREADS), 0, s->stream, s->wt_base, (unsigned long long)fr.total_work, s->wt_sums, s->wt_total);
            hipLaunchKernelGGL(weighted_scan_apply_kernel, dim3(RT_WSCAN_BLOCKS), dim3(RT_WSCAN_THREADS), 0, s->stream, s->wt_base, (unsigned long long)fr.total_work, (const unsigned long long *)s->wt_sums);
            HIPCHK(hipGetLastError());
            HIPCHK(hipEventRecord(s->wt_ev[1], s->stream));
            HIPCHK(hipStreamSynchronize(s->stream));
            const unsigned long long n_points = *s->wt_total;
            auto late_fail = [&](int code, const char *msg) { s->last_weighted = false; s->last_pipeline = false; s->have_timing = false; s->wt_points = 0; return fail(code, msg); };
            if (n_points >= 0xffffffffull) return late_fail(RT_EINVAL, "rt_render: strategy \"weighted\": more than 2^32 - 2 shading points in the frame");
            s->wt_points = n_points;
            const bool mixed = s->light_draws < 0;
            const int nD = int(s->n_drawing_lights);
            size_t rec_floats = size_t(n_points) * size_t(R);
            fr.wt_mixed = mixed ? 1 : 0; fr.wt_nd = unsigned(nD); fr.wt_recbase = nullptr;
            if (mixed) {
                {
                    const double W = double(fr.total_work ? fr.total_work : 1), Pavg = double(n_points) / W;
                    const double at_least = double(n_points) * double(1 + 2 * (nL - nD)) + double(nD) * W * Pavg * (Pavg + 1.0);
                    if (at_least >= 4294967295.0) return late_fail(RT_EINVAL, "rt_render: strategy \"weighted\" with lights of mixed RNG use: the survey's records exceed 2^32 floats (quadratic in a sample's shading points)");
                }
                rc = ensure(s, &s->wt_recbase, &s->wt_recbase_cap, size_t(fr.total_work) + 1); if (rc) return late_fail(rc, rt_last_error());
                const unsigned long long nw = fr.total_work;
                if (nw) hipLaunchKernelGGL(weighted_sizes_kernel, dim3(unsigned((nw + 255) / 256)), dim3(256), 0, s->stream, (const unsigned *)s->wt_base, nw, unsigned(1 + 2 * (nL - nD)), unsigned(nD), s->wt_recbase);
                hipLaunchKernelGGL(weighted_scan_sums_kernel, dim3(RT_WSCAN_BLOCKS), dim3(RT_WSCAN_THREADS), 0, s->stream, (const unsigned *)s->wt_recbase, nw, s->wt_sums);
                hipLaunchKernelGGL(weighted_scan_top_kernel, dim3(1), dim3(RT_WSCAN_THREADS), 0, s->stream, s->wt_recbase, nw, s->wt_sums, s->wt_total);
                hipLaunchKernelGGL(weighted_scan_apply_kernel, dim3(RT_WSCAN_BLOCKS), dim3(RT_WSCAN_THREADS), 0, s->stream, s->wt_recbase, nw, (const unsigned long long *)s->wt_sums);
                HIPCHK(hipGetLastError());
                HIPCHK(hipStreamSynchronize(s->stream));
                if (*s->wt_total >= 0xffffffffull) return late_fail(RT_EINVAL, "rt_render: strategy \"weighted\" with lights of mixed RNG use: the survey's records exceed 2^32 floats");
                rec_floats = size_t(*s->wt_total);
                fr.wt_recbase = s->wt_recbase;
            }
            rc = ensure(s, &s->wt_rec, &s->wt_rec_cap, rec_floats + 1); if (rc) return late_fail(rc, rt_last_error());
            rc = ensure(s, &s->wt_pick, &s->wt_pick_cap, size_t(n_points) + 1); if (rc) return late_fail(rc, rt_last_error());
            fr.wt_rec = s->wt_rec; fr.wt_pick = s->wt_pick;
            if (n_points > 0) {
                if ((rc = pass(2))) return rc;
                HIPCHK(hipEventRecord(s->wt_ev[2], s->stream));
                const size_t state_f = nL <= 64 ? 0 : size_t((3 * nL + 2) & ~1);
                int chunk = int((size_t(64) * 1024 / 4 - state_f - 2) / size_t(R + 2));
                chunk = chunk > 1024 ? 1024 : chunk < 1 ? 1 : chunk;
                const size_t lds = (state_f + size_t((chunk * R + 1) & ~1) + size_t(chunk) * 2) * sizeof(float);
                if (mixed) {
                    const int group = 256;
                    const size_t fixed = size_t(5 * nL + 2) + 2 * size_t(group + 1);
                    const size_t room = size_t(64) * 1024 / 4 - fixed - 4;
                    const int cap_points = int(room / 4 / 2), cap_floats = int(room - size_t(cap_points) * 2) & ~1;
                    const size_t mlds = (fixed + size_t(cap_floats) + 2 + size_t(cap_points) * 2) * sizeof(float);
                    hipLaunchKernelGGL(weighted_recurrence_mixed_kernel, dim3(1), dim3(64), mlds, s->stream, (const float *)s->wt_rec, s->wt_pick, (const unsigned *)s->wt_base,
                                       (const unsigned *)s->wt_recbase, (unsigned long long)fr.total_work, nL, nD, s->light_draw_flags, group, cap_floats, cap_points);
                } else {
                auto rk = nL <= 64 ? weighted_recurrence_lanes_kernel : weighted_recurrence_lds_kernel;
                hipLaunchKernelGGL(rk, dim3(1), dim3(64), lds, s->stream, (const float *)s->wt_rec, s->wt_pick, n_points, nL, chunk);
                }
                HIPCHK(hipGetLastError());
                HIPCHK(hipEventRecord(s->wt_ev[3], s->stream));
            } else { HIPCHK(hipEventRecord(s->wt_ev[2], s->stream)); HIPCHK(hipEventRecord(s->wt_ev[3], s->stream)); }
            if ((rc = pass(3))) return rc;
            HIPCHK(hipEventRecord(s->ev1, s->stream));
            s->last_pipeline = false; s->last_weighted = true;
        } else {
#ifdef RT_TAIL_PROBE
        static unsigned long long *probe = nullptr;
        const size_t n_waves = size_t(s->grids[variant]) * (RT_BLOCK / 64);
        if (!probe) HIPCHK(hipMalloc((void **)&probe, size_t(s->n_threads / 64 + 64) * 4 * sizeof(unsigned long long)));
        HIPCHK(hipMemsetAsync(probe, 0, n_waves * 4 * sizeof(unsigned long long), s->stream));
        fr.probe = probe;
#endif
        HIPCHK(hipMemcpyAsync(s->dev_frame, &fr, sizeof(DevFrame), hipMemcpyHostToDevice, s->stream));
        HIPCHK(hipMemsetAsync(s->work_counter, 0, 64 * sizeof(unsigned long long), s->stream));
        HIPCHK(hipEventRecord(s->ev0, s->stream));
        hipLaunchKernelGGL(render_kernel_of(variant), dim3(s->grids[variant]), dim3(RT_BLOCK), 0, s->stream,
                           (const DevScene *)s->dev_scene, (const DevFrame *)s->dev_frame);
        HIPCHK(hipGetLastError());
        HIPCHK(hipEventRecord(s->ev1, s->stream));
#ifdef RT_TAIL_PROBE
        {
            std::vector<unsigned long long> h(n_waves * 4);
            HIPCHK(hipStreamSynchronize(s->stream));
            HIPCHK(hipMemcpy(h.data(), probe, h.size() * sizeof(unsigned long long), hipMemcpyDeviceToHost));
            unsigned long long t0 = ~0ull, t0max = 0, e0 = ~0ull, e1 = 0, x1 = 0, smin = ~0ull, smax = 0, stot = 0;
            std::vector<double> ends, drain;
            for (size_t w = 0; w < n_waves; ++w) {
                const unsigned long long *r = &h[4 * w];
                if (!r[2]) continue;
                t0 = std::min(t0, r[0]); t0max = std::max(t0max, r[0]); x1 = std::max(x1, r[2]);
                if (r[1]) { e0 = std::min(e0, r[1]); e1 = std::max(e1, r[1]); drain.push_back(double(r[2] - r[1]) * 1e-2); }
                smin = std::min(smin, r[3]); smax = std::max(smax, r[3]); stot += r[3];
                ends.push_back(double(r[2]));
            }
            std::sort(ends.begin(), ends.end()); std::sort(drain.begin(), drain.end());
            auto q = [&](const std::vector<double> &v, double f) { return v.empty() ? 0.0 : v[size_t(f * (v.size() - 1))]; };
            std::fprintf(stderr, "RT_TAIL_PROBE waves=%zu span=%.1f us | starts spread %.1f us | list first seen empty at %.1f us, last at %.1f us | wave ends (us after start): p1 %.1f p10 %.1f p50 %.1f p90 %.1f p99 %.1f max %.1f | "
                                 "drain per wave (end - empty, us): p10 %.1f p50 %.1f p90 %.1f p99 %.1f max %.1f | samples per wave min %llu mean %.1f max %llu\n",
                         ends.size(), double(x1 - t0) * 1e-2, double(t0max - t0) * 1e-2, double(e0 - t0) * 1e-2, double(e1 - t0) * 1e-2,
                         (q(ends, .01) - double(t0)) * 1e-2, (q(ends, .1) - double(t0)) * 1e-2, (q(ends, .5) - double(t0)) * 1e-2, (q(ends, .9) - double(t0)) * 1e-2, (q(ends, .99) - double(t0)) * 1e-2, (q(ends, 1.) - double(t0)) * 1e-2,
                         q(drain, .1), q(drain, .5), q(drain, .9), q(drain, .99), q(drain, 1.), smin, double(stot) / double(std::max<size_t>(ends.size(), 1)), smax);
        }
#endif
        s->last_pipeline = false; s->last_weighted = false;
        }
    }
    if (!skip_film) { rc = film_gather_launch(s, fr, fg, (const DevFrame *)s->dev_frame, 0, fr.y_pixel_count); if (rc) return rc; }
    HIPCHK(hipEventRecord(s->ev2, s->stream));
    s->have_timing = true;
#ifdef RT_PROFILE
    {
        unsigned long long v[24];
        HIPCHK(hipStreamSynchronize(s->stream));
        HIPCHK(hipMemcpy(v, s->counters, sizeof v, hipMemcpyDeviceToHost));
        std::fprintf(stderr, "RT_PROFILE shade_cyc=%llu trav_cyc=%llu outer=%llu inner=%llu rounds=%llu act_lane_rounds=%llu rays_at_trav_start=%llu desc_cyc=%llu leaf_cyc=%llu chunks=%llu pooled_rounds=%llu leaf_iters=%llu\n",
                     v[8], v[9], v[10], v[11], v[12], v[13], v[14], v[15], v[16], v[17], v[18], v[19]);
#ifdef RT_PROFILE_STAGES
        {
            unsigned long long st[32];
            HIPCHK(hipMemcpy(st, s->counters + 24, sizeof st, hipMemcpyDeviceToHost));
            static const char *names[16] = {"FETCH", "VERTEX", "DIRECT_NEXT", "SHADOW_DONE", "MIS_DONE", "ED_BSDF", "ED_DONE", "BOUNCE", "SPECULAR", "SPEC_TRANS", "RETURN", "VOL_BEGIN", "VOL_STEP", "POP", "FINISH", "EXIT"};
            for (int i = 0; i < 16; ++i) if (st[2 * i + 1])
                std::fprintf(stderr, "RT_PROFILE_STAGE %-12s cycles=%llu passes=%llu lane_visits=%llu\n", names[i], st[2 * i], st[2 * i + 1] >> 40, st[2 * i + 1] & ((1ull << 40) - 1));
            HIPCHK(hipMemsetAsync(s->counters + 24, 0, 32 * sizeof(unsigned long long), s->stream));
        }
#endif
        HIPCHK(hipMemsetAsync(s->counters + 8, 0, 16 * sizeof(unsigned long long), s->stream));
    }
#endif
    return RT_OK;
}
int rt_sync(RtScene *s) {
    if (!s) return fail(RT_EINVAL, "null scene");
    HIPCHK(hipSetDevice(s->device));
    HIPCHK(hipStreamSynchronize(s->stream));
    return RT_OK;
}

int rt_counters(RtScene *s, RtCounters *out) {
    if (!s || !out) return fail(RT_EINVAL, "null argument");
    HIPCHK(hipSetDevice(s->device));
    HIPCHK(hipStreamSynchronize(s->stream));
    unsigned long long v[8];
    HIPCHK(hipMemcpy(v, s->counters, sizeof v, hipMemcpyDeviceToHost));
    out->camera_rays = v[0]; out->closest_rays = v[1]; out->any_rays = v[2]; out->nodes_visited = v[3];
    out->leaf_refs = v[4]; out->tri_tests = v[5]; out->bad_samples = v[6]; out->stack_overflows = v[7];
    return RT_OK;
}
int rt_counters_reset(RtScene *s) {
    if (!s) return fail(RT_EINVAL, "null scene");
    HIPCHK(hipSetDevice(s->device));
    HIPCHK(hipMemsetAsync(s->counters, 0, 24 * sizeof(unsigned long long), s->stream));
    return RT_OK;
}
int rt_set_counting(RtScene *s, int enabled) {
    if (!s) return fail(RT_EINVAL, "null scene");
    s->counting = enabled != 0;
    return RT_OK;
}
int rt_last_render_ms(RtScene *s, float *total_ms, float *kernel_ms) {
    if (!s || !s->have_timing) return fail(RT_ESTATE, "no timed launch yet");
    HIPCHK(hipSetDevice(s->device));
    HIPCHK(hipEventSynchronize(s->ev2));
    float k = 0.f, t = 0.f;
    HIPCHK(hipEventElapsedTime(&k, s->ev0, s->ev1));
    HIPCHK(hipEventElapsedTime(&t, s->ev0, s->ev2));
    if (total_ms) *total_ms = t;
    if (kernel_ms) *kernel_ms = k;
    return RT_OK;
}
int rt_last_render_stats(RtScene *s, RtRenderStats *out) {
    if (!s || !out) return fail(RT_EINVAL, "null argument");
    if (!s->have_timing) return fail(RT_ESTATE, "no timed launch yet");
    HIPCHK(hipSetDevice(s->device));
    HIPCHK(hipEventSynchronize(s->ev2));
    std::memset(out, 0, sizeof *out);
    HIPCHK(hipEventElapsedTime(&out->render_ms, s->ev0, s->ev1));
    HIPCHK(hipEventElapsedTime(&out->total_ms, s->ev0, s->ev2));
    out->gather_ms = out->total_ms - out->render_ms;
    out->pipeline = s->last_pipeline ? 1 : 0;
    if (s->last_pipeline) {
        out->iterations = s->pipe_iters; out->timed_iterations = s->pipe_timed;
        float sum = 0.f;
        float sum2 = 0.f, sum3 = 0.f;
        for (int i = 0; i < s->pipe_timed; ++i) {
            float ms = 0.f; HIPCHK(hipEventElapsedTime(&ms, s->pipe_ev[6 * i], s->pipe_ev[6 * i + 1])); sum += ms;
            HIPCHK(hipEventElapsedTime(&ms, s->pipe_ev[6 * i + 2], s->pipe_ev[6 * i + 3])); sum2 += ms;
            if (s->last_marches) { HIPCHK(hipEventElapsedTime(&ms, s->pipe_ev[6 * i + 4], s->pipe_ev[6 * i + 5])); sum3 += ms; }
        }
        out->trace_ms = sum; out->shade_ms = sum2; out->march_ms = sum3;
        out->slots = s->pipe_slots;
    } else out->trace_ms = out->render_ms;
    out->bands = s->last_pipeline ? 0 : 1;
    if (s->last_weighted) {
        out->weighted_points = s->wt_points;
        hipEvent_t seq[6] = {s->ev0, s->wt_ev[0], s->wt_ev[1], s->wt_ev[2], s->wt_ev[3], s->ev1};
        for (int i = 0; i < 5; ++i) HIPCHK(hipEventElapsedTime(&out->weighted_ms[i], seq[i], seq[i + 1]));
    }
    return RT_OK;
}

}
```

pbrt-v1_amd/csrc/hip/rt_render_kernel.h:

```cpp
#pragma once
#include "rt_integrate.h"

namespace rt {

#ifndef RT_MEGA_CHUNK
#define RT_MEGA_CHUNK 64
#endif
static_assert(RT_MEGA_CHUNK >= 64, "one fresh chunk must cover a whole wave's fetch");
RT_DEV unsigned long long uniform64(unsigned long long v) {
    const unsigned lo = __builtin_amdgcn_readfirstlane(unsigned(v)), hi = __builtin_amdgcn_readfirstlane(unsigned(v >> 32));
    return (unsigned long long)hi << 32 | lo;
}


RT_DEV unsigned long long band_lo(unsigned long long total, unsigned r, unsigned n) {
    if (r >= n) return total;
    return (total / RT_MEGA_CHUNK) * r / n * RT_MEGA_CHUNK;
}

#ifndef RT_MIN_WAVES
#define RT_MIN_WAVES 1
#endif
#ifndef RT_MEGA_BYV
#define RT_MEGA_BYV 1
#endif


#ifndef RT_HIGH_OCC_WAVES
#define RT_HIGH_OCC_WAVES 4
#endif
template <bool COUNT, int INTEG, int ACCEL, bool VOL, int MINW, bool EXT>
__global__ __launch_bounds__(RT_BLOCK, MINW) void render_kernel(const DevScene *__restrict__ scp,
                                                                       const DevFrame *__restrict__ frp) {
    __shared__ uint2 lds_stack[RT_STACK_LDS * RT_BLOCK];
    constexpr bool POOL = MINW < RT_HIGH_OCC_WAVES;
    constexpr int PN = POOL ? RT_BLOCK : 64;
    __shared__ unsigned long long pool_key[PN];
    __shared__ float4 pool_res[PN];
    __shared__ unsigned pool_head[PN];
    __shared__ float4 pool_ray[3 * PN];
    __shared__ float lds_tm_own[POOL ? 1 : RT_STACK_LDS * RT_BLOCK];
    float RT_L *lds_tm = (float RT_L *)lds_tm_own;
    const DevScene &sc = *scp;
    const DevFrame &fr = *frp;
    const unsigned wave0 = POOL ? (threadIdx.x & ~63u) : 0u;
    const PoolLds pool = {(unsigned long long RT_L *)pool_key + wave0, (float4 RT_L *)pool_res + wave0, (unsigned RT_L *)pool_head + wave0,
                          (float4 RT_L *)pool_ray + 3 * wave0};
    const unsigned gtid = blockIdx.x * RT_BLOCK + threadIdx.x;
    const int lane = threadIdx.x & 63;
    constexpr bool BYV = RT_MEGA_BYV != 0 && !POOL && INTEG == RT_INTEGRATOR_PATH && !VOL && !EXT && !COUNT;
    Lane ln;
    ln.vf = 0u;
    ln.stage = ST_FETCH; ln.has_ray = false; ln.fsp = 0; ln.tv.active = false; ln.tv.hit_prim = -1;
    ln.L = mk3(0.f); ln.thr = mk3(1.f); ln.alpha = 0.f; ln.depth = 0; ln.specular = false;
    TravCounters tc; tc.nodes = tc.leaf_refs = tc.tris = tc.spills = 0;
    RT_PFT(tc.c_desc = tc.c_leaf = tc.n_chunks = tc.n_pooled = tc.n_iter = 0;)
    unsigned c_cam = 0, c_closest = 0, c_any = 0, c_bad = 0;

#ifdef RT_PROFILE
    unsigned long long pf_shade = 0, pf_trav = 0, pf_outer = 0, pf_inner = 0, pf_rounds = 0, pf_act = 0, pf_rays = 0, pf_t0 = 0;
#define RT_PF(x) x
#else
#define RT_PF(x)
#endif
#ifdef RT_TAIL_PROBE
    const unsigned long long tp_start = __builtin_amdgcn_s_memrealtime();
    unsigned long long tp_empty = 0, tp_taken = 0;
#endif
    unsigned long long w_next = 0, w_end = 0;
    const unsigned n_bands = fr.xcd_bands ? 8u : 1u, home = fr.xcd_bands ? (blockIdx.x & 7u) : 0u;
    unsigned band_shift = 0;

    int phase = (INTEG == RT_INTEGRATOR_PATH && fr.phase_sync && !BYV) ? 1 : -1;
    for (;;) {
        RT_PF(pf_t0 = __builtin_readcyclecounter(); ++pf_outer;)
        do {
            RT_PF(++pf_inner;)
            if constexpr (BYV) advance_pass_byv<COUNT, ACCEL, EXT>(sc, fr, ln, gtid, &c_closest, &c_any, &c_bad);
            else advance_pass<COUNT, INTEG, VOL, EXT>(sc, fr, ln, gtid, &c_closest, &c_any, &c_bad, phase);
            const unsigned long long want = phase == 0 ? 0ull : __ballot(!ln.has_ray && ln.stage == ST_FETCH);
            if (want) {
                const unsigned n_want = unsigned(__popcll(want));
                const unsigned long long have = w_end - w_next;
                unsigned long long fresh = 0, fresh_end = 0;
                if (have < n_want) {
                    const int leader = __ffsll((long long)want) - 1;
#pragma unroll 1
                    while (band_shift < n_bands) {
                        const unsigned r = (home + band_shift) % n_bands;
                        const unsigned long long lo = band_lo(fr.total_work, r, n_bands), hi = band_lo(fr.total_work, r + 1u, n_bands);
                        unsigned long long base = 0;
                        if (lane == leader) base = atomicAdd(fr.work_counter + 8u * r, (unsigned long long)RT_MEGA_CHUNK);
                        base = uniform64(__shfl(base, leader));
                        if (lo + base < hi) { fresh = lo + base; fresh_end = fresh + RT_MEGA_CHUNK < hi ? fresh + RT_MEGA_CHUNK : hi; break; }
                        ++band_shift;
                    }
                }
                const bool none_left = band_shift >= n_bands;
#ifdef RT_TAIL_PROBE
                if (none_left && !tp_empty) tp_empty = __builtin_amdgcn_s_memrealtime();
#endif
                const unsigned long long rk = __popcll(want & ((1ull << lane) - 1ull));
                const unsigned long long w_mine = rk < have ? w_next + rk : fresh + (rk - have);
                const bool got = rk < have || w_mine < fresh_end;
                if (have < n_want) {
                    const unsigned long long took = n_want - have < fresh_end - fresh ? n_want - have : fresh_end - fresh;
                    w_next = fresh + took; w_end = fresh_end;
                } else w_next += n_want;
                if (!ln.has_ray && ln.stage == ST_FETCH && !got) { if (none_left) ln.stage = ST_EXIT; }
                else if (!ln.has_ray && ln.stage == ST_FETCH) {
                    const unsigned long long w = w_mine;
#ifdef RT_TAIL_PROBE
                    tp_taken += 1;
#endif
                    {
                        unsigned long long pixel; int s;
                        bool ok;
                        if (fr.mega_tile > 0) { unsigned px; tile_order_to_sample(fr, unsigned(w), px, s); pixel = px; ok = true; }
                        else ok = work_to_sample(fr, w, pixel, s);
                        if (ok) {
                            Ray ray;
                            setup_sample(sc, fr, ln, pixel, s, ray);
                            ln.work = fr.mega_tile > 0 ? uint32_t(pixel * unsigned(fr.spp) + unsigned(s)) : uint32_t(w);
                            if (INTEG == RT_INTEG_DIRECT_WEIGHTED) ln.ord = fr.weighted_phase == 1 ? 0u : RT_GPTR(const unsigned, fr.wt_base)[ln.work];
                            ln.L = mk3(0.f); ln.thr = mk3(1.f); ln.alpha = 0.f; ln.depth = 0; ln.fsp = 0;
                            ln.specular = false;
                            if (COUNT) ++c_cam;
                            accel_begin<ACCEL>(ln.tv, sc, ray, false);
                            if (VOL) vol_store_ray(fr, 0, gtid, ray);
                            ln.has_ray = true; ln.stage = ST_VERTEX;
                            if (BYV) ln.vf = BV_B | BV_CUR_B;
                        }
                    }
                }
            }
        } while (__any(!ln.has_ray && stage_in_phase(ln.stage, phase)));
        if (phase >= 0) phase ^= 1;
        RT_PF({ unsigned long long t1 = __builtin_readcyclecounter(); pf_shade += t1 - pf_t0; pf_t0 = t1; pf_rays += __popcll(__ballot(ln.has_ray && ln.tv.active)); })
        if (!__any(ln.has_ray)) {
            if (!__any(ln.stage != ST_EXIT)) break;
            continue;
        }
        for (;;) {
            if constexpr (BYV) {
                const bool next = ln.has_ray && !ln.tv.active && (ln.vf & (BV_QM | BV_QB)) != 0u;
                if (__any(next)) { if (next) byv_ray_advance<COUNT, ACCEL, EXT>(sc, ln, &c_closest, &c_any); }
            }
            const bool act = ln.has_ray && ln.tv.active;
            const unsigned long long am = __ballot(act);
            if (!am) break;
            RT_PF(++pf_rounds; pf_act += __popcll(am);)
            if (fr.exit_thresh > 0 && __popcll(am) <= fr.exit_thresh && __any(!act && ln.stage != ST_EXIT)) break;
            if (POOL && fr.trav_mode == 3) accel_round_pooled<COUNT, ACCEL, EXT>(ln.tv, ln.has_ray, sc, (uint2 RT_L *)lds_stack, RT_GPTR(uint2, fr.spill), fr.n_threads, gtid, tc, pool);
            else trace_round<COUNT, ACCEL, EXT, RT_STACK_LDS, !POOL>(ln.tv, ln.has_ray, sc, (uint2 RT_L *)lds_stack, lds_tm, RT_GPTR(uint2, fr.spill), fr.n_threads, gtid, tc, fr.leaf_min);
        }
        if (ln.has_ray && !ln.tv.active && !(BYV && (ln.vf & (BV_QM | BV_QB)) != 0u)) ln.has_ray = false;
        RT_PF(pf_trav += __builtin_readcyclecounter() - pf_t0;)
    }
#ifdef RT_PROFILE
    if (lane == 0) {
        unsigned long long v[12] = {pf_shade, pf_trav, pf_outer, pf_inner, pf_rounds, pf_act, pf_rays, tc.c_desc, tc.c_leaf, tc.n_chunks, tc.n_pooled, tc.n_iter};
        for (int k = 0; k < 12; ++k) atomicAdd(fr.counters + 8 + k, v[k]);
    }
#endif

#ifdef RT_TAIL_PROBE
    {
        for (int off = 32; off > 0; off >>= 1) tp_taken += __shfl_down(tp_taken, off);
        if (lane == 0 && fr.probe) {
            unsigned long long *o = fr.probe + size_t(gtid >> 6) * 4u;
            o[0] = tp_start; o[1] = tp_empty; o[2] = __builtin_amdgcn_s_memrealtime(); o[3] = tp_taken;
        }
    }
#endif
    if (COUNT && !(INTEG == RT_INTEG_DIRECT_WEIGHTED && fr.weighted_phase != 3)) {
        unsigned long long v[8] = {c_cam, c_closest, c_any, tc.nodes, tc.leaf_refs, tc.tris, c_bad, tc.spills};
#pragma unroll
        for (int k = 0; k < 8; ++k) {
            unsigned long long x = v[k];
            for (int off = 32; off > 0; off >>= 1) x += __shfl_down(x, off);
            if (lane == 0 && x) atomicAdd(fr.counters + k, x);
        }
    }
}

typedef void (*RenderKernelFn)(const DevScene *, const DevFrame *);

}
```

pbrt-v1_amd/csrc/hip/rt_scene.hip:

```cpp
#include "rt_host.h"
#include "../../../include/pbrt_hip_material.h"

static void host_tri_frame(const float *v, bool flip, float nn[3], float sn[3]) {
    const float du1 = 0.f - 1.f, du2 = 1.f - 1.f, dv1 = 0.f - 1.f, dv2 = 0.f - 1.f;
    const float determinant = du1 * dv2 - dv1 * du2;
    const float invdet = 1.f / determinant;
    float dpdu[3], dpdv[3];
    for (int a = 0; a < 3; ++a) {
        const float dp1 = v[a] - v[6 + a], dp2 = v[3 + a] - v[6 + a];
        dpdu[a] = invdet * ((dv2 * dp1) - (dv1 * dp2));
        dpdv[a] = invdet * ((-du2 * dp1) + (du1 * dp2));
    }
    float c[3] = {(dpdu[1] * dpdv[2]) - (dpdu[2] * dpdv[1]), (dpdu[2] * dpdv[0]) - (dpdu[0] * dpdv[2]), (dpdu[0] * dpdv[1]) - (dpdu[1] * dpdv[0])};
    float inv = 1.f / sqrtf(c[0] * c[0] + c[1] * c[1] + c[2] * c[2]);
    for (int a = 0; a < 3; ++a) { nn[a] = c[a] * inv; if (flip) nn[a] = -1.f * nn[a]; }
    inv = 1.f / sqrtf(dpdu[0] * dpdu[0] + dpdu[1] * dpdu[1] + dpdu[2] * dpdu[2]);
    for (int a = 0; a < 3; ++a) sn[a] = dpdu[a] * inv;
}

static void leaf_records_fill_host(const RefVec &slot_prim, const std::vector<DevTri> &tris, std::vector<float4> &ltris) {
    ltris.assign(slot_prim.size() * RT_TRI_STRIDE + 4, make_float4(0.f, 0.f, 0.f, 0.f));
    for (size_t i = 0; i < slot_prim.size(); ++i) {
        const uint32_t prim = slot_prim[i];
        float4 q2 = tris[prim].q2; std::memcpy(&q2.w, &prim, 4);
// ... 238 lines not shown
    tick("accelerator");
    PairBlockOrder pbo;
    std::thread order_thread;
    struct Joiner { std::thread &t; ~Joiner() { if (t.joinable()) t.join(); } } joiner{order_thread};
    if (s->accel_kind == RT_ACCEL_KDTREE) order_thread = std::thread([&] { pair_blocks_order(s->tree.nodes, pbo); });
    LeafLayout ll;
    int ll_status = 0;
    bool runs = s->tree.leaf_refs.size() + s->tree.nodes.size() / 2 <= 32768;
    if (const char *e = knob("PBRT_HIP_LEAF_RUNS")) runs = std::atoi(e) != 0;
    const bool copies = knob("PBRT_HIP_LEAF_COPIES") != nullptr;
    std::thread layout_thread;
    Joiner joiner2{layout_thread};
    if (s->accel_kind == RT_ACCEL_KDTREE) layout_thread = std::thread([&] {
        try { ll_status = leaf_cursor_layout(s->tree.nodes, s->tree.leaf_refs, d->n_tris, copies, runs, ll) ? 1 : -1; } catch (...) { ll_status = -2; }
    });
    std::vector<DevTri> tris(d->n_tris);
    uint32_t n_quadric_slots = 0;
    for (uint32_t i = 0; i < d->n_tris; ++i) {
        const float *v = d->tri_verts + size_t(9) * i;
        uint32_t bits = uint32_t(d->tri_material[i]) | (uint32_t(d->tri_flags[i] & 1u) << 16);
        int32_t light = d->tri_light[i];
        float fb, fl; std::memcpy(&fb, &bits, 4); std::memcpy(&fl, &light, 4);
        if (d->tri_flags[i] & 2u) {
            bits |= RT_PRIM_QUADRIC; std::memcpy(&fb, &bits, 4);
            float fi; std::memcpy(&fi, &n_quadric_slots, 4); ++n_quadric_slots;
            tris[i].q0 = make_float4(fi, 0.f, 0.f, 0.f); tris[i].q1 = make_float4(0.f, 0.f, 0.f, 0.f); tris[i].q2 = make_float4(0.f, fb, fl, 0.f);
            continue;
        }
        const float e1[3] = {v[3] - v[0], v[4] - v[1], v[5] - v[2]}, e2[3] = {v[6] - v[0], v[7] - v[1], v[8] - v[2]};
        tris[i].q0 = make_float4(v[0], v[1], v[2], e1[0]);
        tris[i].q1 = make_float4(e1[1], e1[2], e2[0], e2[1]);
        tris[i].q2 = make_float4(e2[2], fb, fl, 0.f);
    }
    std::vector<float4> shade(size_t(2) * d->n_tris);
    if (n_quadric_slots != d->n_quadrics || (d->n_quadrics && !d->quadrics)) return fail(RT_EINVAL, "rt_scene_create: quadric slots do not match n_quadrics");
    s->has_ext = s->has_ext || d->n_quadrics > 0;
    std::vector<DevTriShading> dshading; std::vector<int> shading_idx;
    if (d->tri_shading) {
        if (d->n_shading && !d->shading) return fail(RT_EINVAL, "rt_scene_create: tri_shading without shading records");
        shading_idx.assign(d->n_tris, -1);
    }
    for (uint32_t i = 0; i < d->n_tris; ++i) {
        float nn[3] = {0.f, 0.f, 0.f}, sn[3] = {0.f, 0.f, 0.f};
        const int sh = (d->tri_shading && !(d->tri_flags[i] & 2u)) ? d->tri_shading[i] : -1;
        bool smooth = false;
        if (sh >= 0) {
            if (uint32_t(sh) >= d->n_shading) return fail(RT_EINVAL, "rt_scene_create: shading record index out of range");
            const RtTriShading &r = d->shading[sh];
            if ((r.flags & (RT_SHADING_N | RT_SHADING_S)) && (r.xform >= d->n_xforms || !d->xforms)) return fail(RT_EINVAL, "rt_scene_create: shading record refers to a transform out of range");
            float dpdu[3];
            host_tri_frame_uv(d->tri_verts + size_t(9) * i, r.uv, (d->tri_flags[i] & 1u) != 0, nn, dpdu);
            const float inv = 1.f / sqrtf(dpdu[0] * dpdu[0] + dpdu[1] * dpdu[1] + dpdu[2] * dpdu[2]);
            for (int a = 0; a < 3; ++a) sn[a] = dpdu[a] * inv;
            if (r.flags & (RT_SHADING_N | RT_SHADING_S)) {
                smooth = true; s->has_ext = true;
                DevTriShading o; std::memset(&o, 0, sizeof o);
                o.flags = r.flags; o.xform = r.xform;
                std::memcpy(o.uv, r.uv, sizeof o.uv); std::memcpy(o.dpdu, dpdu, sizeof o.dpdu);
                std::memcpy(o.n, r.n, sizeof o.n); std::memcpy(o.s, r.s, sizeof o.s);
                shading_idx[i] = int(dshading.size()); dshading.push_back(o);
            }
        } else if (!(d->tri_flags[i] & 2u)) host_tri_frame(d->tri_verts + size_t(9) * i, (d->tri_flags[i] & 1u) != 0, nn, sn);
        uint32_t bits = uint32_t(d->tri_material[i]) | (uint32_t(d->tri_flags[i] & 1u) << 16) | ((d->tri_flags[i] & 2u) ? RT_PRIM_QUADRIC : 0u) |
                        (smooth ? RT_PRIM_SHADING : 0u);
        int32_t light = d->tri_light[i];
        float fb, fl; std::memcpy(&fb, &bits, 4); std::memcpy(&fl, &light, 4);
        shade[2 * i] = make_float4(nn[0], nn[1], nn[2], fb);
        shade[2 * i + 1] = make_float4(sn[0], sn[1], sn[2], fl);
    }
    int rc;
    if ((rc = upload(s, shade.data(), shade.size(), &s->dev.tri_shade))) return rc;
    if (!dshading.empty()) {
        if ((rc = upload(s, shading_idx.data(), shading_idx.size(), &s->dev.tri_shading_idx))) return rc;
        if ((rc = upload(s, dshading.data(), dshading.size(), &s->dev.tri_shading))) return rc;
        if ((rc = upload(s, d->xforms, size_t(d->n_xforms) * 32, &s->dev.xforms))) return rc;
    }
    if ((rc = upload(s, tris.data(), tris.size(), &s->dev.tris))) return rc;
    {
        std::vector<DevQuadric> dq(d->n_quadrics);
        for (uint32_t i = 0; i < d->n_quadrics; ++i) {
            const RtQuadric &q = d->quadrics[i]; DevQuadric &o = dq[i];
            if (q.type < RT_QUADRIC_SPHERE || q.type > RT_QUADRIC_HYPERBOLOID) return fail(RT_EINVAL, "rt_scene_create: unknown quadric type");
            std::memcpy(o.w2o, q.world_to_object, sizeof o.w2o); std::memcpy(o.o2w, q.object_to_world, sizeof o.o2w);
            o.radius = q.radius; o.zmin = q.zmin; o.zmax = q.zmax; o.theta_min = q.theta_min; o.theta_max = q.theta_max; o.phi_max = q.phi_max;
            o.type = q.type; o.pad = 0;
            for (int c = 0; c < 3; ++c) { o.p1[c] = q.p1[c]; o.p2[c] = q.p2[c]; }
            o.a = q.a; o.c = q.c;
        }
        if ((rc = upload(s, dq.data(), dq.size(), &s->dev.quadrics))) return rc;
    }
    tick("triangle / shading records");
    auto upload_nodes = [&](const NodeVec &v, const uint2 **dev) -> int {
        void *p = nullptr;
        HIPCHK(hipMalloc(&p, (v.size() + 1) * sizeof(uint2)));
        s->allocs.push_back(p);
        if (!v.empty()) HIPCHK(hipMemcpy(p, v.data(), v.size() * sizeof(uint2), hipMemcpyHostToDevice));
        const uint2 pad = make_uint2(3u, 0u);
        HIPCHK(hipMemcpy((uint2 *)p + v.size(), &pad, sizeof pad, hipMemcpyHostToDevice));
        *dev = (const uint2 *)p;
        return RT_OK;
    };
    const uint2 *nodes_dev = nullptr;
    if ((rc = upload_nodes(s->tree.nodes, &nodes_dev))) return rc;
    if ((rc = upload(s, s->tree.leaf_refs.data(), s->tree.leaf_refs.size(), &s->dev.leaf_refs))) return rc;
    s->dev.nodes = nodes_dev;
    s->dev.tnodes = nodes_dev;
    if (s->accel_kind == RT_ACCEL_KDTREE) {
        tick("node / leaf-list upload");
        layout_thread.join();
        if (ll_status == -2) return fail(RT_ENOMEM, "rt_scene_create: out of host memory while laying out the leaf entries");
        if (ll_status != 1) return fail(RT_EINVAL, "rt_scene_create: primitive records beyond 2^30 float4 units or leaf entries beyond 2^31");
        s->dev.leaf_runs = runs ? 1u : 0u;
        const NodeVec &tn = ll.tnodes;
        tick("leaf entries (rest)");
        if ((rc = upload_nodes(tn, &s->dev.tnodes))) return rc;
        if ((rc = upload(s, ll.lrefs.data(), ll.lrefs.size(), &s->dev.lrefs))) return rc;
        {
            const unsigned *slot_prim_dev = nullptr;
            if ((rc = upload(s, ll.slot_prim.data(), ll.slot_prim.size(), &slot_prim_dev))) return rc;
            const size_t units = ll.n_slots * RT_TRI_STRIDE + 4;
            void *p = nullptr;
            HIPCHK(hipMalloc(&p, units * sizeof(float4)));
            s->allocs.push_back(p);
            s->dev.ltris = (const float4 *)p;
            HIPCHK(hipMemsetAsync(p, 0, units * sizeof(float4), s->stream));
            if (ll.n_slots) hipLaunchKernelGGL(derive_leaf_records_kernel, dim3(unsigned((ll.n_slots + 255) / 256)), dim3(256), 0, s->stream, slot_prim_dev,
                                               (const DevTri *)s->dev.tris, (float4 *)p, ll.n_slots);
            HIPCHK(hipGetLastError());
            if (knob("PBRT_HIP_VERIFY_DERIVED")) {
                std::vector<float4> lt, back(units); leaf_records_fill_host(ll.slot_prim, tris, lt);
                HIPCHK(hipStreamSynchronize(s->stream));
                HIPCHK(hipMemcpy(back.data(), p, units * sizeof(float4), hipMemcpyDeviceToHost));
                if (lt.size() != units || std::memcmp(back.data(), lt.data(), units * sizeof(float4)) != 0) return fail(RT_ESTATE, "rt_scene_create: the device-built primitive records differ from the host fill");
            }
            s->n_leaf_tri_units = units;
            s->n_leaf_entries = ll.lrefs.size();
        }
        tick("primitive records (device)");
        std::vector<uint4> pairs;
        order_thread.join();
        pair_blocks_fill(tn, pbo, pairs, s->dev.root_x, s->dev.root_y);
        s->dev.top_pairs = pbo.top;
        if (pairs.empty() || pairs.size() >= (size_t(1) << 30)) return fail(RT_EINVAL, "rt_scene_create: pair records beyond 2^30");
        tick("pair blocks");
        if ((rc = upload(s, pairs.data(), pairs.size(), &s->dev.tpairs))) return rc;
        tick("pair upload");
    }
    std::vector<DevMaterial> mats(d->n_materials);
    for (uint32_t i = 0; i < d->n_materials; ++i) {
        const RtMaterial &m = d->materials[i]; DevMaterial &o = mats[i];
        o.type = m.type; o.ior = m.ior; o.on_a = 1.f; o.on_b = -1.f;
        for (int c = 0; c < 3; ++c) { o.r[c] = m.kd[c]; o.t[c] = m.kt[c]; }
        o.has_r = (m.kd[0] != 0.f || m.kd[1] != 0.f || m.kd[2] != 0.f);
        o.has_t = (m.kt[0] != 0.f || m.kt[1] != 0.f || m.kt[2] != 0.f);
        for (int c = 0; c < 3; ++c) o.ks[c] = m.ks[c];
        o.exponent = 0.f;
        for (int c = 0; c < 3; ++c) o.kr[c] = m.kr[c];
        o.has_g = (m.ks[0] != 0.f || m.ks[1] != 0.f || m.ks[2] != 0.f); o.has_kr = (m.kr[0] != 0.f || m.kr[1] != 0.f || m.kr[2] != 0.f);
        if (m.type == RT_MAT_PLASTIC || m.type == RT_MAT_UBER) { s->has_ext = true; float e = 1.f / m.roughness; if (e > 1000.f || std::isnan(e)) e = 1000.f; o.exponent = e; }
        if (m.type == RT_MAT_SHINYMETAL || m.type == RT_MAT_TRANSLUCENT) {
            RtMaterialLobes lb; rt_material_lobes(&m, &lb);
            const bool shiny = m.type == RT_MAT_SHINYMETAL;
            for (int c = 0; c < 3; ++c) {
                o.r[c] = lb.r_kd[c]; o.t[c] = lb.t_kd[c];
                o.ks[c] = shiny ? lb.eta_ks[c] : lb.r_ks[c]; o.kr[c] = shiny ? lb.eta_kr[c] : lb.t_ks[c];
            }
            o.has_r = lb.has_dr; o.has_t = lb.has_dt; o.has_g = lb.has_gr; o.has_kr = lb.has_gt;
            s->has_ext = true; float e = 1.f / m.roughness; if (e > 1000.f || std::isnan(e)) e = 1000.f; o.exponent = e;
        }
        if (m.type < RT_MAT_MATTE || m.type > RT_MAT_TRANSLUCENT) return fail(RT_EINVAL, "rt_scene_create: unknown material type");
        if (m.type == RT_MAT_MATTE && m.sigma != 0.f) {
            float sigma = (3.14159265358979323846f / 180.f) * m.sigma;
            float sigma2 = sigma * sigma;
            o.on_a = 1.f - (sigma2 / (2.f * (sigma2 + 0.33f)));
            o.on_b = 0.45f * sigma2 / (sigma2 + 0.09f);
        }
    }
    if ((rc = upload(s, mats.data(), mats.size(), &s->dev.materials))) return rc;

    std::vector<float> ltris(size_t(d->n_light_tris) * 16, 0.f);
    std::vector<DevLight> lights(d->n_lights);
    for (uint32_t i = 0; i < d->n_lights; ++i) {
        const RtLight &L = d->lights[i]; DevLight &o = lights[i];
        o.type = L.type; o.n_samples = L.n_samples < 1 ? 1 : L.n_samples;
        for (int c = 0; c < 3; ++c) { o.color[c] = L.color[c]; o.pos[c] = L.pos[c]; }
        o.first_tri = L.first_tri; o.n_tris = L.n_tris; o.reverse_orientation = L.reverse_orientation;
        o.flip_normal = L.flip_normal; o.area = 0.f;
        for (int c = 0; c < 3; ++c) o.dir[c] = L.dir[c];
        for (int c = 0; c < 9; ++c) o.w2l[c] = L.world_to_light[c];
        o.cos_total = L.cos_total_width; o.cos_falloff = L.cos_falloff_start;
        o.quadric = L.quadric_plus1 - 1;
        if (L.quadric_plus1 < 0 || uint32_t(L.quadric_plus1) > d->n_quadrics) return fail(RT_EINVAL, "rt_scene_create: light refers to a quadric out of range");
        if (L.type < RT_LIGHT_POINT || L.type > RT_LIGHT_INFINITE) return fail(RT_EINVAL, "rt_scene_create: unknown light type");
        if (L.type == RT_LIGHT_INFINITE) { s->has_ext = true; ++s->n_infinite; }
        if (L.type != RT_LIGHT_AREA) continue;
        if (size_t(L.first_tri) + L.n_tris > d->n_light_tris) return fail(RT_EINVAL, "rt_scene_create: light triangle range out of bounds");
        float area = 0.f; std::vector<float> areas;
        for (uint32_t k = 0; k < L.n_tris; ++k) {
            const float *v = d->light_tris + size_t(L.first_tri + k) * 9;
            float *q = &ltris[size_t(L.first_tri + k) * 16];
            std::memcpy(q, v, 9 * sizeof(float));
            { float nl[3], sn_unused[3]; host_tri_frame(v, L.flip_normal != 0, nl, sn_unused); q[12] = nl[0]; q[13] = nl[1]; q[14] = nl[2]; }
            float ax = v[3] - v[0], ay = v[4] - v[1], az = v[5] - v[2];
            float bx = v[6] - v[0], by = v[7] - v[1], bz = v[8] - v[2];
            float cx = (ay * bz) - (az * by), cy = (az * bx) - (ax * bz), cz = (ax * by) - (ay * bx);
            float a = 0.5f * sqrtf(cx * cx + cy * cy + cz * cz);
            q[9] = a; area += a; areas.push_back(a);
        }
        float prev = 0.f;
        for (uint32_t k = 0; k < L.n_tris; ++k) {
            float c = prev + areas[k] / area;
            ltris[size_t(L.first_tri + k) * 16 + 10] = c; prev = c;
        }
        o.area = (L.n_tris == 1) ? areas[0] : area;
    }
    if ((rc = upload(s, lights.data(), lights.size(), &s->dev.lights))) return rc;
    if ((rc = upload(s, ltris.data(), ltris.size(), &s->dev.light_tris))) return rc;
    {
        std::vector<unsigned> flags(d->n_lights ? d->n_lights : 1, 0u);
        s->n_drawing_lights = 0;
        for (uint32_t i = 0; i < d->n_lights; ++i) {
            const int draws = (d->lights[i].type == RT_LIGHT_AREA && d->lights[i].quadric_plus1 == 0 && d->lights[i].n_tris > 1) ? 1 : 0;
            if (i == 0) s->light_draws = draws; else if (draws != s->light_draws) s->light_draws = -1;
            flags[i] = unsigned(draws); s->n_drawing_lights += unsigned(draws);
        }
        if ((rc = upload(s, flags.data(), flags.size(), &s->light_draw_flags))) return rc;
    }

    s->dev.n_tris = d->n_tris; s->dev.n_lights = d->n_lights; s->dev.n_infinite = int(s->n_infinite);
    s->dev.accel_kind = s->accel_kind;
    for (int a = 0; a < 3; ++a) { s->dev.nvox[a] = s->gridacc.nvox[a]; s->dev.gwidth[a] = s->gridacc.width[a]; s->dev.ginv_width[a] = s->gridacc.inv_width[a]; }
    std::memcpy(s->dev.bounds, s->tree.bounds, sizeof s->dev.bounds);
    s->dev.cam = d->camera; s->dev.vol = d->volume; s->volume = d->volume;

    hipDeviceProp_t prop;
    HIPCHK(hipGetDeviceProperties(&prop, s->device));
    s->n_cus = prop.multiProcessorCount;
    {
        unsigned mx = 0;
        for (int k = 0; k < 48; ++k) {
            int per_cu = 0;
            HIPCHK(hipOccupancyMaxActiveBlocksPerMultiprocessor(&per_cu, (const void *)render_kernel_of(k), RT_BLOCK, 0));
            if (per_cu < 1) per_cu = 1;
            s->grids[k] = unsigned(prop.multiProcessorCount) * unsigned(per_cu);
            mx = s->grids[k] > mx ? s->grids[k] : mx;
        }
        for (int k = 0; k < 8; ++k) {
            int per_cu = 0;
            HIPCHK(hipOccupancyMaxActiveBlocksPerMultiprocessor(&per_cu, (const void *)g_render_kernels_weighted[k], RT_BLOCK, 0));
            s->wgrids[k] = unsigned(prop.multiProcessorCount) * unsigned(per_cu < 1 ? 1 : per_cu);
            mx = s->wgrids[k] > mx ? s->wgrids[k] : mx;
        }
        s->grid = mx;
    }
    s->n_threads = s->grid * RT_BLOCK;
    s->spill_depth = s->tree.max_depth > RT_TRACE_STACK ? s->tree.max_depth - RT_TRACE_STACK + 1 : 1;
    HIPCHK(hipMalloc((void **)&s->work_counter, 64 * sizeof(unsigned long long)));
    HIPCHK(hipMalloc((void **)&s->counters, 64 * sizeof(unsigned long long)));
    HIPCHK(hipMemsetAsync(s->counters, 0, 64 * sizeof(unsigned long long), s->stream));
    HIPCHK(hipMalloc((void **)&s->filter_dev, 256 * sizeof(float)));
    HIPCHK(hipMalloc((void **)&s->dev_scene, sizeof(DevScene)));
    HIPCHK(hipMalloc((void **)&s->dev_frame, sizeof(DevFrame)));
    HIPCHK(hipMemcpy(s->dev_scene, &s->dev, sizeof(DevScene), hipMemcpyHostToDevice));
    HIPCHK(hipEventCreate(&s->ev2));
    for (int k = 0; k < 8; ++k) {
        int per_cu = 0;
        HIPCHK(hipOccupancyMaxActiveBlocksPerMultiprocessor(&per_cu, (const void *)g_pipe_trace[k], RT_BLOCK, 0));
        if (const char *e = knob("PBRT_HIP_TRACE_BLOCKS_PER_CU")) per_cu = std::min(per_cu, std::max(1, std::atoi(e)));
        s->trace_grids[k] = unsigned(prop.multiProcessorCount) * unsigned(per_cu < 1 ? 1 : per_cu);
        if (s->trace_grids[k] * RT_BLOCK > s->n_threads) s->n_threads = s->trace_grids[k] * RT_BLOCK;
    }
    for (int k = 0; k < 6; ++k) {
        int per_cu = 0;
        HIPCHK(hipOccupancyMaxActiveBlocksPerMultiprocessor(&per_cu, (const void *)g_pipe_march[k], RT_BLOCK, 0));
        s->march_grids[k] = unsigned(prop.multiProcessorCount) * unsigned(per_cu < 1 ? 1 : per_cu);
        if (s->march_grids[k] * RT_BLOCK > s->n_threads) s->n_threads = s->march_grids[k] * RT_BLOCK;
    }
    HIPCHK(hipMalloc((void **)&s->spill, size_t(s->spill_depth) * s->n_threads * sizeof(uint4)));
    HIPCHK(hipMalloc((void **)&s->dev_pool, sizeof(PipePool)));
    HIPCHK(hipMalloc((void **)&s->trace_qc, RT_QC_STRIDE * sizeof(unsigned)));
    HIPCHK(hipHostMalloc((void **)&s->h_qcount, size_t(RT_PIPE_QN) * RT_QC_STRIDE * sizeof(unsigned), hipHostMallocDefault));
    HIPCHK(hipStreamSynchronize(s->stream));
    guard.p = nullptr;
    *out = s;
    return RT_OK;
}

int rt_scene_destroy(RtScene *s) {
    if (!s) return RT_OK;
    HIPWARN(hipSetDevice(s->device));
    if (s->stream) hipStreamSynchronize(s->stream);
    for (void *p : s->allocs) HIPWARN(hipFree(p));
    if (s->own_accum && s->accum) HIPWARN(hipFree(s->accum));
    HIPWARN(hipFree(s->spill)); HIPWARN(hipFree(s->work_counter)); HIPWARN(hipFree(s->counters)); HIPWARN(hipFree(s->filter_dev));
    if (s->frames) HIPWARN(hipFree(s->frames));
    if (s->samples) HIPWARN(hipFree(s->samples));
    if (s->resolve_buf) HIPWARN(hipFree(s->resolve_buf));
    if (s->vol_buf) HIPWARN(hipFree(s->vol_buf));
    if (s->light_dims) HIPWARN(hipFree(s->light_dims));
    if (s->wt_base) HIPWARN(hipFree(s->wt_base));
    if (s->wt_recbase) HIPWARN(hipFree(s->wt_recbase));
    if (s->wt_rec) HIPWARN(hipFree(s->wt_rec));
    if (s->wt_pick) HIPWARN(hipFree(s->wt_pick));
    if (s->wt_total) HIPWARN(hipHostFree(s->wt_total));
    if (s->wt_sums) HIPWARN(hipFree(s->wt_sums));
    for (hipEvent_t e : s->wt_ev) if (e) HIPWARN(hipEventDestroy(e));
    HIPWARN(hipFree(s->dev_scene)); HIPWARN(hipFree(s->dev_frame));
    HIPWARN(hipFree(s->pool.state)); HIPWARN(hipFree(s->pool.ray_o)); HIPWARN(hipFree(s->pool.hit)); HIPWARN(hipFree(s->pool.q_o));
    HIPWARN(hipFree(s->pool.q_slot)); HIPWARN(hipFree(s->pool.q_count)); HIPWARN(hipFree(s->pool.wave_work)); HIPWARN(hipFree(s->dev_pool));
    HIPWARN(hipFree(s->trace_buf)); HIPWARN(hipFree(s->trace_qc));
    if (s->h_qcount) HIPWARN(hipHostFree(s->h_qcount));
    for (hipEvent_t e : s->pipe_ev) HIPWARN(hipEventDestroy(e));
    for (hipEvent_t e : s->pipe_fence) HIPWARN(hipEventDestroy(e));
    if (s->ev2) HIPWARN(hipEventDestroy(s->ev2));
    if (s->ev0) HIPWARN(hipEventDestroy(s->ev0));
    if (s->ev1) HIPWARN(hipEventDestroy(s->ev1));
    if (s->own_stream && s->stream) HIPWARN(hipStreamDestroy(s->stream));
    delete s;
    return RT_OK;
}

int rt_scene_set_stream(RtScene *s, void *hip_stream) {
    if (!s) return fail(RT_EINVAL, "null scene");
    if (s->own_stream && s->stream) { HIPWARN(hipStreamSynchronize(s->stream)); HIPWARN(hipStreamDestroy(s->stream)); }
    s->stream = static_cast<hipStream_t>(hip_stream); s->own_stream = false;
    return RT_OK;
}

int rt_scene_set_density(RtScene *s, const RtDensityRegion *r) {
    if (!s || !r) return fail(RT_EINVAL, "rt_scene_set_density: null argument");
    if (s->rendered) return fail(RT_ESTATE, "rt_scene_set_density: the scene has rendered a frame already");
    if (s->density_kind != RT_DENSITY_NONE) return fail(RT_ESTATE, "rt_scene_set_density: the scene has a density region already");
    if (!s->volume.present) return fail(RT_EINVAL, "rt_scene_set_density: the scene has no medium (RtSceneDesc.volume.present == 0)");
    if (r->kind != RT_DENSITY_EXPONENTIAL && r->kind != RT_DENSITY_GRID) return fail(RT_EINVAL, "rt_scene_set_density: unknown density kind");
    double a[4][8];
    for (int i = 0; i < 4; ++i) for (int j = 0; j < 4; ++j) { a[i][j] = s->volume.world_to_volume[4 * i + j]; a[i][4 + j] = i == j ? 1.0 : 0.0; }
    for (int c = 0; c < 4; ++c) {
        int piv = c;
        for (int i = c + 1; i < 4; ++i) if (std::fabs(a[i][c]) > std::fabs(a[piv][c])) piv = i;
        if (!(std::fabs(a[piv][c]) > 0.0)) return fail(RT_EINVAL, "rt_scene_set_density: singular world_to_volume");
        for (int j = 0; j < 8; ++j) std::swap(a[c][j], a[piv][j]);
        const double inv = 1.0 / a[c][c];
        for (int j = 0; j < 8; ++j) a[c][j] *= inv;
        for (int i = 0; i < 4; ++i) if (i != c) { const double f = a[i][c]; for (int j = 0; j < 8; ++j) a[i][j] -= f * a[c][j]; }
    }
    double wb[6] = {INFINITY, INFINITY, INFINITY, -INFINITY, -INFINITY, -INFINITY};
    for (int k = 0; k < 8; ++k) {
        const double q[3] = {(k & 1) ? s->volume.p1[0] : s->volume.p0[0], (k & 2) ? s->volume.p1[1] : s->volume.p0[1], (k & 4) ? s->volume.p1[2] : s->volume.p0[2]};
        double w[4];
        for (int i = 0; i < 4; ++i) w[i] = a[i][4] * q[0] + a[i][5] * q[1] + a[i][6] * q[2] + a[i][7];
        for (int i = 0; i < 3; ++i) { const double v = w[3] != 1.0 ? w[i] / w[3] : w[i]; wb[i] = std::min(wb[i], v); wb[3 + i] = std::max(wb[3 + i], v); }
    }
    for (double v : wb) if (!std::isfinite(v)) return fail(RT_EINVAL, "rt_scene_set_density: the volume's world bound is not finite");
    HIPCHK(hipSetDevice(s->device));
    const float *grid = nullptr;
    if (r->kind == RT_DENSITY_GRID) {
        const long long total = (long long)r->nx * r->ny * r->nz;
        if (r->nx <= 0 || r->ny <= 0 || r->nz <= 0 || total > 0x7fffffffLL) return fail(RT_EINVAL, "rt_scene_set_density: grid counts must be positive with nx*ny*nz < 2^31");
        if (!r->density) return fail(RT_EINVAL, "rt_scene_set_density: null density grid");
        int rc = upload(s, r->density, size_t(total), &grid); if (rc) return rc;
    }
    DevScene &d = s->dev;
    d.dens_kind = r->kind; d.dens_a = r->a; d.dens_b = r->b;
    for (int i = 0; i < 3; ++i) d.dens_up[i] = r->updir[i];
    d.dens_n[0] = r->nx; d.dens_n[1] = r->ny; d.dens_n[2] = r->nz; d.dens_grid = grid;
    HIPCHK(hipStreamSynchronize(s->stream));
    HIPCHK(hipMemcpy(s->dev_scene, &s->dev, sizeof(DevScene), hipMemcpyHostToDevice));
    std::memcpy(s->vol_world, wb, sizeof wb);
    s->density_kind = r->kind;
    s->has_ext = true;
    return RT_OK;
}

int rt_scene_accel_info(const RtScene *s, RtAccelInfo *info) {
    if (!s || !info) return fail(RT_EINVAL, "null argument");
    fill_info(s->tree, s->gridacc, s->accel_kind, s->n_tris, info);
    return RT_OK;
}

int rt_scene_accel_copy(const RtScene *s, uint32_t *nodes, uint32_t *leaf_refs) {
    if (!s) return fail(RT_EINVAL, "null scene");
    if (nodes) std::memcpy(nodes, s->tree.nodes.data(), s->tree.nodes.size() * sizeof(Node));
    if (leaf_refs) std::memcpy(leaf_refs, s->tree.leaf_refs.data(), s->tree.leaf_refs.size() * sizeof(uint32_t));
    return RT_OK;
}

struct RtKdTree { KdTree tree; GridAccelData grid; int kind = RT_ACCEL_KDTREE; uint32_t n_tris = 0; };
static void fill_info(const KdTree &tree, const GridAccelData &g, int kind, uint32_t n_tris, RtAccelInfo *info) {
    info->n_nodes = uint32_t(tree.nodes.size()); info->n_leaf_refs = uint32_t(tree.leaf_refs.size());
    info->max_depth = uint32_t(tree.max_depth); info->n_tris = n_tris;
    std::memcpy(info->bounds, tree.bounds, sizeof info->bounds); info->build_seconds = tree.build_seconds;
    info->kind = kind;
    for (int a = 0; a < 3; ++a) {
        info->grid_nvoxels[a] = kind == RT_ACCEL_GRID ? g.nvox[a] : 0;
        info->grid_width[a] = kind == RT_ACCEL_GRID ? g.width[a] : 0.f;
        info->grid_inv_width[a] = kind == RT_ACCEL_GRID ? g.inv_width[a] : 0.f;
    }
}
int rt_accel_build(const float *tri_verts, uint32_t n_tris, const RtAccelParams *params, RtAccel **out) {
    if (!out || (n_tris && !tri_verts)) return fail(RT_EINVAL, "rt_accel_build: null argument");
    RtAccelParams p; std::memset(&p, 0, sizeof p);
    if (params) p = *params;
    if (p.kind != RT_ACCEL_GRID && p.kind != RT_ACCEL_KDTREE) return fail(RT_EINVAL, "rt_accel_build: unknown accelerator kind");
    return guarded("rt_accel_build", [&] {
        std::unique_ptr<RtKdTree> t(new RtKdTree()); t->n_tris = n_tris; t->kind = p.kind;
        if (p.kind == RT_ACCEL_GRID) {
            build_grid(tri_verts, n_tris, t->grid);
            t->tree.nodes = t->grid.voxels; t->tree.leaf_refs = t->grid.refs; t->tree.max_depth = 0;
            std::memcpy(t->tree.bounds, t->grid.bounds, sizeof t->tree.bounds); t->tree.build_seconds = t->grid.build_seconds;
        } else build_kdtree(tri_verts, n_tris, p, t->tree);
        *out = t.release(); return RT_OK;
    });
}
int rt_accel_info(const RtAccel *t, RtAccelInfo *info) {
    if (!t || !info) return fail(RT_EINVAL, "null argument");
    fill_info(t->tree, t->grid, t->kind, t->n_tris, info);
    return RT_OK;
}
int rt_accel_copy(const RtAccel *t, uint32_t *nodes, uint32_t *leaf_refs) {
    if (!t) return fail(RT_EINVAL, "null accelerator");
    if (nodes) std::memcpy(nodes, t->tree.nodes.data(), t->tree.nodes.size() * sizeof(Node));
    if (leaf_refs) std::memcpy(leaf_refs, t->tree.leaf_refs.data(), t->tree.leaf_refs.size() * sizeof(uint32_t));
    return RT_OK;
}
int rt_accel_destroy(RtAccel *t) { delete t; return RT_OK; }
int rt_accel_leaf_layout(const RtAccel *t, int runs, int copies, uint32_t *tnodes, uint32_t *slot_prim, uint32_t *entries, RtLeafLayoutInfo *info) {
    if (!t || !info) return fail(RT_EINVAL, "rt_accel_leaf_layout: null argument");
    if (t->kind != RT_ACCEL_KDTREE) return fail(RT_EINVAL, "rt_accel_leaf_layout: not a kd-tree");
    return guarded("rt_accel_leaf_layout", [&] {
        LeafLayout ll;
        if (!leaf_cursor_layout(t->tree.nodes, t->tree.leaf_refs, t->n_tris, copies != 0, runs != 0, ll)) return fail(RT_EINVAL, "rt_accel_leaf_layout: primitive records beyond 2^30 float4 units or leaf entries beyond 2^31");
        info->n_nodes = ll.tnodes.size(); info->n_slots = ll.n_slots; info->n_entries = ll.lrefs.size(); info->stride = RT_TRI_STRIDE;
        if (tnodes && !ll.tnodes.empty()) std::memcpy(tnodes, ll.tnodes.data(), ll.tnodes.size() * sizeof(Node));
        if (slot_prim && ll.n_slots) std::memcpy(slot_prim, ll.slot_prim.data(), ll.n_slots * sizeof(uint32_t));
        if (entries) std::memcpy(entries, ll.lrefs.data(), ll.lrefs.size() * sizeof(uint32_t));
        return int(RT_OK);
    });
}
int rt_kdtree_build(const float *tri_verts, uint32_t n_tris, const RtAccelParams *params, RtKdTree **out) {
    if (params && params->kind != RT_ACCEL_KDTREE) return fail(RT_EINVAL, "rt_kdtree_build: not a kd-tree description");
    return rt_accel_build(tri_verts, n_tris, params, out);
}
int rt_kdtree_info(const RtKdTree *t, RtAccelInfo *info) { return rt_accel_info(t, info); }
int rt_kdtree_copy(const RtKdTree *t, uint32_t *nodes, uint32_t *leaf_refs) { return rt_accel_copy(t, nodes, leaf_refs); }
int rt_kdtree_destroy(RtKdTree *t) { return rt_accel_destroy(t); }

}
```

Before: 3416.

## Trace primary camera rays as wave-coherent packets before the megakernel

Adds a packet traversal kernel that walks the kd-tree once per 64-lane wave with a shared LDS stack ring and a global spill pool. It precomputes camera-ray hits into a buffer, and the megakernel skips its own primary traversal when a packet hit is present. The goal is to cut divergent per-lane traversal cost for coherent primary rays. The cost is an extra kernel launch, a hit buffer in memory, a budget abort path that falls back to per-ray tracing, and possible wasted work when rays in a wave diverge.

```diff
diff --git a/include/pbrt_hip.h b/include/pbrt_hip.h
--- a/include/pbrt_hip.h
+++ b/include/pbrt_hip.h
@@ -222,6 +222,15 @@
 int rt_film_pack_parts(RtScene *s, const float *dev_accum, int32_t w, int32_t h, int32_t world, int32_t rows, float *dev_parts);
 int rt_last_render_stats(RtScene *s, RtRenderStats *out);
 
+#define RT_HIT_PACKET_ABORTED INT32_MIN
+int rt_trace_camera_packets(RtScene *s, const RtRenderDesc *rd, uint64_t first, uint32_t count, RtHit *hits_out);
+typedef struct RtPacketStats { uint64_t waves, aborted, spill_areas; float ms; int32_t pad; } RtPacketStats;
+int rt_last_packet_stats(RtScene *s, RtPacketStats *out);
+int rt_packet_walk_host(const uint32_t *nodes, uint32_t n_nodes, const uint32_t *leaf_refs, uint32_t n_leaf_refs, const float *bounds,
+                        const float *tri_verts, uint32_t n_tris, int runs, const RtRay *rays, uint32_t n_rays,
+                        uint32_t budget, uint32_t ring_entries, uint32_t spill_entries,
+                        RtHit *packet_hits, uint32_t *packet_counts, RtHit *ray_hits, uint32_t *ray_counts, uint8_t *wave_status);
+
 #ifdef __cplusplus
 }
 #endif
diff --git a/pbrt-v1_amd/__init__.py b/pbrt-v1_amd/__init__.py
--- a/pbrt-v1_amd/__init__.py
+++ b/pbrt-v1_amd/__init__.py
@@ -19,7 +19,7 @@
 
 
 HIP_UNITS = ("rt_kernels.hip", "rt_scene.hip", "rt_film.hip", "rt_trace.hip", "rt_mega_w.hip", "rt_mega_d.hip", "rt_mega_dw.hip", "rt_mega_p.hip", "rt_pipe_w.hip", "rt_pipe_d.hip",
-             "rt_pipe_p.hip", "rt_pipe_v.hip", "rt_march.hip", "kd_build.cpp", "grid_build.cpp", "leaf_layout.cpp")
+             "rt_pipe_p.hip", "rt_pipe_v.hip", "rt_march.hip", "rt_packet.hip", "kd_build.cpp", "grid_build.cpp", "leaf_layout.cpp", "packet_host.cpp")
 
 
 def build(force: bool = False, verbose: bool = False, defines=(), jobs: int | None = None) -> None:
@@ -117,6 +117,13 @@
         return {n: (list(getattr(self, n)) if n == "weighted_ms" else getattr(self, n)) for n, _ in self._fields_}
 
 
+class RtPacketStats(C.Structure):
+    _fields_ = [("waves", C.c_uint64), ("aborted", C.c_uint64), ("spill_areas", C.c_uint64), ("ms", C.c_float), ("pad", C.c_int32)]
+
+    def as_dict(self):
+        return {"waves": int(self.waves), "aborted": int(self.aborted), "spill_areas": int(self.spill_areas), "ms": float(self.ms)}
+
+
 class RtVolume(C.Structure):
     _fields_ = [("present", C.c_int32), ("world_to_volume", C.c_float * 16), ("p0", C.c_float * 3), ("p1", C.c_float * 3),
                 ("sigma_a", C.c_float * 3), ("sigma_s", C.c_float * 3), ("le", C.c_float * 3), ("g", C.c_float)]
@@ -193,7 +200,8 @@
                      "rt_counters_reset", "rt_last_render_ms", "rt_last_render_stats", "rt_samples_read", "rt_device_count", "rt_set_counting",
                      "rt_kdtree_build", "rt_kdtree_info", "rt_kdtree_copy", "rt_kdtree_destroy",
                      "rt_accel_build", "rt_accel_info", "rt_accel_copy", "rt_accel_destroy", "rt_scene_create_prebuilt", "rt_film_resolve_device",
-                     "rt_film_resolve_device_rgba", "rt_film_pack_parts", "rt_accel_leaf_layout", "rt_scene_set_density"):
+                     "rt_film_resolve_device_rgba", "rt_film_pack_parts", "rt_accel_leaf_layout", "rt_scene_set_density",
+                     "rt_trace_camera_packets", "rt_last_packet_stats", "rt_packet_walk_host"):
             getattr(L, name).restype = C.c_int
         L.rt_scene_create.argtypes = [C.c_void_p, C.c_int, C.POINTER(C.c_void_p)]
         L.rt_scene_set_density.argtypes = [C.c_void_p, C.c_void_p]
@@ -230,6 +238,10 @@
         L.rt_accel_copy.argtypes = [C.c_void_p, C.c_void_p, C.c_void_p]
         L.rt_accel_destroy.argtypes = [C.c_void_p]
         L.rt_accel_leaf_layout.argtypes = [C.c_void_p, C.c_int, C.c_int, C.c_void_p, C.c_void_p, C.c_void_p, C.POINTER(RtLeafLayoutInfo)]
+        L.rt_trace_camera_packets.argtypes = [C.c_void_p, C.c_void_p, C.c_uint64, C.c_uint32, C.c_void_p]
+        L.rt_last_packet_stats.argtypes = [C.c_void_p, C.POINTER(RtPacketStats)]
+        L.rt_packet_walk_host.argtypes = [C.c_void_p, C.c_uint32, C.c_void_p, C.c_uint32, C.c_void_p, C.c_void_p, C.c_uint32, C.c_int, C.c_void_p, C.c_uint32,
+                                          C.c_uint32, C.c_uint32, C.c_uint32, C.c_void_p, C.c_void_p, C.c_void_p, C.c_void_p, C.c_void_p]
         _hip = L
     return _hip
 
@@ -420,6 +432,24 @@
     return nodes, refs[:info.n_leaf_refs], tn, sp[:li.n_slots], en[:li.n_entries], int(li.stride)
 
 
+HIT_PACKET_ABORTED = -(1 << 31)
+
+
+def packet_walk_host(nodes, leaf_refs, bounds, tri_verts, rays, budget: int = 1 << 30, ring_entries: int = 24, spill_entries: int = 40, runs: bool = False):
+    nodes = np.ascontiguousarray(nodes, np.uint32).reshape(-1, 2); refs = np.ascontiguousarray(leaf_refs, np.uint32)
+    refs_arg = refs if len(refs) else np.zeros(1, np.uint32)
+    b = np.ascontiguousarray(bounds, np.float32); tv = np.ascontiguousarray(tri_verts, np.float32).reshape(-1, 9)
+    rays = np.ascontiguousarray(rays, RAY_DTYPE); n = len(rays)
+    ph = np.zeros(n, HIT_DTYPE); rh = np.zeros(n, HIT_DTYPE); pc = np.zeros((n, 3), np.uint32); rc = np.zeros((n, 3), np.uint32)
+    st = np.zeros(max((n + 63) // 64, 1), np.uint8)
+    code = hip_lib().rt_packet_walk_host(nodes.ctypes.data, len(nodes), refs_arg.ctypes.data, len(refs), b.ctypes.data, tv.ctypes.data, len(tv), int(runs),
+                                         rays.ctypes.data, n, budget, ring_entries, spill_entries, ph.ctypes.data, pc.ctypes.data, rh.ctypes.data,
+                                         rc.ctypes.data, st.ctypes.data)
+    if code != 0:
+        raise RtError("rt_packet_walk_host failed (%d)" % code)
+    return ph, pc, rh, rc, st[:(n + 63) // 64]
+
+
 def fit_tile(extent: int, size: int) -> int:
     best = None
     for t in range(max(1, size * 3 // 4), max(2, size * 5 // 4) + 1):
@@ -726,6 +756,16 @@
         _chk(hip_lib().rt_trace_closest(self._s, rays.ctypes.data, len(rays), hits.ctypes.data))
         return hits
 
+    def trace_camera_packets(self, first: int, count: int) -> np.ndarray:
+        hits = np.zeros(count, HIT_DTYPE)
+        _chk(hip_lib().rt_trace_camera_packets(self._s, self.parsed.render_desc, first, count, hits.ctypes.data))
+        return hits
+
+    def last_packet_stats(self) -> dict:
+        st = RtPacketStats()
+        _chk(hip_lib().rt_last_packet_stats(self._s, C.byref(st)))
+        return st.as_dict()
+
     def trace_any(self, rays: np.ndarray) -> np.ndarray:
         rays = np.ascontiguousarray(rays, RAY_DTYPE)
         occ = np.zeros(len(rays), np.uint8)
diff --git a/pbrt-v1_amd/csrc/hip/packet_host.cpp b/pbrt-v1_amd/csrc/hip/packet_host.cpp
--- /dev/null
+++ b/pbrt-v1_amd/csrc/hip/packet_host.cpp
@@ -0,0 +1,162 @@
+#define RT_PK_HOST 1
+#include "rt_packet.h"
+#include "rt_internal.h"
+#include <new>
+
+namespace rt {
+namespace {
+
+struct HostTree {
+    LeafLayout ll;
+    std::vector<PkF4> ltris;
+    PkTree t;
+};
+
+bool host_tree(const uint32_t *nodes, uint32_t n_nodes, const uint32_t *leaf_refs, uint32_t n_leaf_refs, const float *bounds, const float *tri_verts,
+               uint32_t n_tris, bool runs, HostTree &o) {
+    NodeVec nv(n_nodes); RefVec rv(n_leaf_refs);
+    for (uint32_t i = 0; i < n_nodes; ++i) { nv[i].x = nodes[2 * size_t(i)]; nv[i].y = nodes[2 * size_t(i) + 1]; }
+    for (uint32_t i = 0; i < n_leaf_refs; ++i) rv[i] = leaf_refs[i];
+    for (uint32_t i = 0; i < n_nodes; ++i) {
+        const Node n = nv[i];
+        if ((n.x & 3u) != 3u) { if (n.y >= n_nodes || i + 1 >= n_nodes) return false; continue; }
+        const uint32_t np = n.x >> 2;
+        if (np == 1) { if (n.y >= n_tris) return false; }
+        else if (np > 1) { if (size_t(n.y) + np > n_leaf_refs) return false; for (uint32_t k = 0; k < np; ++k) if (rv[n.y + k] >= n_tris) return false; }
+    }
+    if (!leaf_cursor_layout(nv, rv, n_tris, false, runs, o.ll)) return false;
+    const PkF4 zero = {0.f, 0.f, 0.f, 0.f};
+    o.ltris.assign(o.ll.n_slots * RT_TRI_STRIDE + 4, zero);
+    for (size_t i = 0; i < o.ll.n_slots; ++i) {
+        const uint32_t prim = o.ll.slot_prim[i];
+        const float *v = tri_verts + size_t(9) * prim;
+        const float e1[3] = {v[3] - v[0], v[4] - v[1], v[5] - v[2]}, e2[3] = {v[6] - v[0], v[7] - v[1], v[8] - v[2]};
+        PkF4 *dst = o.ltris.data() + i * RT_TRI_STRIDE;
+        dst[0] = PkF4{v[0], v[1], v[2], e1[0]};
+        dst[1] = PkF4{e1[1], e1[2], e2[0], e2[1]};
+        dst[2] = PkF4{e2[2], 0.f, 0.f, pk_u2f(prim)};
+    }
+    static_assert(sizeof(Node) == sizeof(PkU2), "node = two words");
+    o.t.tnodes = reinterpret_cast<const PkU2 *>(o.ll.tnodes.data());
+    o.t.ltris = o.ltris.data();
+    o.t.lrefs = o.ll.lrefs.data();
+    o.t.leaf_runs = runs ? 1u : 0u;
+    o.t.n_tris = n_tris;
+    for (int i = 0; i < 6; ++i) o.t.bounds[i] = bounds[i];
+    return true;
+}
+
+void walk_ray(const PkTree &T, const RtRay &r, RtHit &hit, uint32_t cnt[3]) {
+    cnt[0] = cnt[1] = cnt[2] = 0;
+    hit.prim = -1; hit.t = 0.f; hit.b1 = 0.f; hit.b2 = 0.f;
+    float t0 = r.mint, t1 = r.maxt;
+    bool ok = true;
+    for (int i = 0; i < 3; ++i) {
+        const float invRayDir = 1.f / r.d[i];
+        float tNear = (T.bounds[i] - r.o[i]) * invRayDir, tFar = (T.bounds[3 + i] - r.o[i]) * invRayDir;
+        if (tNear > tFar) { const float tmp = tNear; tNear = tFar; tFar = tmp; }
+        t0 = tNear > t0 ? tNear : t0;
+        t1 = tFar < t1 ? tFar : t1;
+        if (t0 > t1) ok = false;
+    }
+    if (!ok || T.n_tris == 0) return;
+    const float inv[3] = {1.f / r.d[0], 1.f / r.d[1], 1.f / r.d[2]};
+    float tmin = t0, tmax = t1, maxt = r.maxt;
+    struct Todo { unsigned node; float tmax; };
+    std::vector<Todo> todo;
+    unsigned node = 0;
+    for (;;) {
+        if (maxt < tmin) break;
+        const PkU2 nd = T.tnodes[node];
+        ++cnt[0];
+        const unsigned axis = nd.x & 3u;
+        if (axis != 3u) {
+            const float split = pk_u2f(nd.x);
+            const float tplane = (split - r.o[axis]) * inv[axis];
+            const bool belowFirst = (r.o[axis] < split) || (r.o[axis] == split && r.d[axis] >= 0.f);
+            const unsigned first = belowFirst ? node + 1u : nd.y, second = belowFirst ? nd.y : node + 1u;
+            if (tplane > tmax || tplane <= 0.f) node = first;
+            else if (tplane < tmin) node = second;
+            else { todo.push_back(Todo{second, tmax}); node = first; tmax = tplane; }
+            continue;
+        }
+        unsigned cur = (nd.x >> 2) | (nd.y & ~RT_LE_POS);
+        unsigned cursor = (nd.y & RT_LE_POS) << ((nd.y >> 30) & 1u);
+        const bool multi = (nd.y & RT_LE_MORE) != 0u;
+        while (cur != RT_LE_NONE) {
+            const PkF4 *q = T.ltris + (cur & RT_LE_POS);
+            unsigned nxt;
+            if (T.leaf_runs) { nxt = cursor > 1u ? cur + RT_TRI_STRIDE : RT_LE_NONE; --cursor; }
+            else if (cur >= (RT_LE_MORE | RT_LE_LIST)) nxt = T.lrefs[cursor++];
+            else nxt = int(cur) < 0 ? cursor : RT_LE_NONE;
+            ++cnt[2]; if (multi) ++cnt[1];
+            const float p1[3] = {q[0].x, q[0].y, q[0].z}, e1[3] = {q[0].w, q[1].x, q[1].y}, e2[3] = {q[1].z, q[1].w, q[2].x};
+            const float *d = r.d;
+            const float s1[3] = {(d[1] * e2[2]) - (d[2] * e2[1]), (d[2] * e2[0]) - (d[0] * e2[2]), (d[0] * e2[1]) - (d[1] * e2[0])};
+            const float divisor = s1[0] * e1[0] + s1[1] * e1[1] + s1[2] * e1[2];
+            cur = nxt;
+            if (divisor == 0.f) continue;
+            const float invDivisor = 1.f / divisor;
+            const float dd[3] = {r.o[0] - p1[0], r.o[1] - p1[1], r.o[2] - p1[2]};
+            const float b1 = (dd[0] * s1[0] + dd[1] * s1[1] + dd[2] * s1[2]) * invDivisor;
+            if (b1 < 0.f || b1 > 1.f) continue;
+            const float s2[3] = {(dd[1] * e1[2]) - (dd[2] * e1[1]), (dd[2] * e1[0]) - (dd[0] * e1[2]), (dd[0] * e1[1]) - (dd[1] * e1[0])};
+            const float b2 = (d[0] * s2[0] + d[1] * s2[1] + d[2] * s2[2]) * invDivisor;
+            if (b2 < 0.f || b1 + b2 > 1.f) continue;
+            const float t = (e2[0] * s2[0] + e2[1] * s2[1] + e2[2] * s2[2]) * invDivisor;
+            if (t < r.mint || t > maxt) continue;
+            maxt = t; hit.prim = int(pk_f2u(q[2].w)); hit.b1 = b1; hit.b2 = b2;
+        }
+        if (todo.empty()) break;
+        node = todo.back().node; tmin = tmax; tmax = todo.back().tmax; todo.pop_back();
+    }
+    hit.t = hit.prim >= 0 ? maxt : 0.f;
+}
+
+}
+}
+
+using namespace rt;
+
+extern "C" int rt_packet_walk_host(const uint32_t *nodes, uint32_t n_nodes, const uint32_t *leaf_refs, uint32_t n_leaf_refs, const float *bounds,
+                                   const float *tri_verts, uint32_t n_tris, int runs, const RtRay *rays, uint32_t n_rays,
+                                   uint32_t budget, uint32_t ring_entries, uint32_t spill_entries,
+                                   RtHit *packet_hits, uint32_t *packet_counts, RtHit *ray_hits, uint32_t *ray_counts, uint8_t *wave_status) {
+    if (!nodes || !n_nodes || !bounds || (n_tris && !tri_verts) || (n_leaf_refs && !leaf_refs) || (n_rays && !rays)) return RT_EINVAL;
+    if (!packet_hits || !packet_counts || !ray_hits || !ray_counts || !wave_status) return RT_EINVAL;
+    if (ring_entries < 1 || ring_entries > RT_PK_RING) return RT_EINVAL;
+    try {
+        HostTree ht;
+        if (!host_tree(nodes, n_nodes, leaf_refs, n_leaf_refs, bounds, tri_verts, n_tris, runs != 0, ht)) return RT_EINVAL;
+        for (uint32_t i = 0; i < n_rays; ++i) walk_ray(ht.t, rays[i], ray_hits[i], ray_counts + size_t(3) * i);
+        const PkU4 z4 = {0u, 0u, 0u, 0u}; const PkF2 z2 = {0.f, 0.f};
+        std::vector<PkU4> hdr(ring_entries, z4), spill(size_t(spill_entries ? spill_entries : 1) * 64, z4);
+        std::vector<PkF2> tm(size_t(ring_entries) * 64, z2);
+        std::unique_ptr<PkLanes<64>> L(new PkLanes<64>());
+        const uint32_t n_waves = (n_rays + 63) / 64;
+        for (uint32_t w = 0; w < n_waves; ++w) {
+            const uint32_t n = n_rays - w * 64 < 64 ? n_rays - w * 64 : 64;
+            const unsigned long long valid = n == 64 ? ~0ull : (1ull << n) - 1ull;
+            for (uint32_t l = 0; l < 64; ++l) {
+                const RtRay &r = rays[size_t(w) * 64 + (l < n ? l : 0)];
+                L->ox[l] = r.o[0]; L->oy[l] = r.o[1]; L->oz[l] = r.o[2]; L->dx[l] = r.d[0]; L->dy[l] = r.d[1]; L->dz[l] = r.d[2];
+                L->mint[l] = r.mint; L->maxt[l] = r.maxt;
+            }
+            unsigned next_area = 0;
+            PkStack S{};
+            S.hdr = hdr.data(); S.tm = tm.data(); S.ns = int(ring_entries);
+            S.spill = nullptr; S.pool = spill_entries ? spill.data() : nullptr; S.next_area = &next_area; S.n_areas = 1; S.cap = spill_entries;
+            const int st = pk_walk<64, true>(ht.t, S, *L, valid, budget);
+            wave_status[w] = uint8_t(st);
+            for (uint32_t l = 0; l < n; ++l) {
+                RtHit &h = packet_hits[size_t(w) * 64 + l];
+                uint32_t *c = packet_counts + (size_t(w) * 64 + l) * 3;
+                if (st != PK_OK) { h.prim = RT_PK_ABORTED; h.t = 0.f; h.b1 = 0.f; h.b2 = 0.f; c[0] = c[1] = c[2] = 0; continue; }
+                h.prim = L->prim[l]; h.t = h.prim >= 0 ? L->maxt[l] : 0.f; h.b1 = L->b1[l]; h.b2 = L->b2[l];
+                c[0] = L->c_nodes[l]; c[1] = L->c_refs[l]; c[2] = L->c_tris[l];
+            }
+        }
+    } catch (const std::bad_alloc &) { return RT_ENOMEM; }
+    catch (...) { return RT_ESTATE; }
+    return RT_OK;
+}
diff --git a/pbrt-v1_amd/csrc/hip/rt_device.h b/pbrt-v1_amd/csrc/hip/rt_device.h
--- a/pbrt-v1_amd/csrc/hip/rt_device.h
+++ b/pbrt-v1_amd/csrc/hip/rt_device.h
@@ -132,6 +132,9 @@
     unsigned wt_nd;
     const unsigned *wt_recbase;
     int dens_cap;
+    const float4 *cam_hits;
+    int packets;
+    unsigned packet_budget;
 #ifdef RT_TAIL_PROBE
     unsigned long long *probe;
 #endif
diff --git a/pbrt-v1_amd/csrc/hip/rt_host.h b/pbrt-v1_amd/csrc/hip/rt_host.h
--- a/pbrt-v1_amd/csrc/hip/rt_host.h
+++ b/pbrt-v1_amd/csrc/hip/rt_host.h
@@ -93,6 +93,11 @@
     float4 *trace_buf = nullptr; size_t trace_cap = 0;
     int n_cus = 0;
     unsigned *trace_qc = nullptr;
+    float4 *cam_hits = nullptr; size_t cam_hits_cap = 0;
+    uint4 *pk_pool = nullptr; size_t pk_pool_cap = 0;
+    unsigned *pk_ctl = nullptr;
+    hipEvent_t pk_ev0 = nullptr, pk_ev1 = nullptr;
+    unsigned pk_waves = 0;
 };
 #define RT_PIPE_QN 4096
 #define RT_PIPE_TIMED 256
@@ -124,6 +129,9 @@
     catch (const std::exception &e) { return rt::fail(RT_ESTATE, std::string(what) + ": " + e.what()); }
 }
 
+int packet_prepare(RtScene *s, unsigned long long count, bool *fits);
+int packet_launch(RtScene *s, unsigned long long first, unsigned count, unsigned budget, bool counting);
+
 struct FilmGather { int which = 0, grx = 0, gry = 0, cols = 0, rows = 0, slot_ncs = 0; size_t slot_lds = 0, col_bytes = 0; };
 int film_gather_plan(RtScene *s, const rt::DevFrame &fr, FilmGather &g);
 int film_gather_launch(RtScene *s, const rt::DevFrame &fr, const FilmGather &g, const rt::DevFrame *dfr, int row0, int row_end);
diff --git a/pbrt-v1_amd/csrc/hip/rt_kernels.hip b/pbrt-v1_amd/csrc/hip/rt_kernels.hip
--- a/pbrt-v1_amd/csrc/hip/rt_kernels.hip
+++ b/pbrt-v1_amd/csrc/hip/rt_kernels.hip
@@ -298,6 +298,10 @@
             if (fr.mega_tile > 4096 || fr.total_work > 0xffffffffull) fr.mega_tile = 0;
         }
         if (fr.trav_mode != 3 || fr.high_occupancy) fr.trav_mode = 2;
+        fr.packets = rd->integrator != RT_INTEGRATOR_PATH ? 1 : 0;
+        if (const char *e = knob("PBRT_HIP_PACKETS")) fr.packets = std::atoi(e) != 0;
+        fr.packet_budget = 4096u;
+        if (const char *e = knob("PBRT_HIP_PACKET_BUDGET")) fr.packet_budget = unsigned(std::max(1, std::atoi(e)));
     }
     fr.work_counter = s->work_counter; fr.counters = s->counters; fr.spill = s->spill; fr.n_threads = s->n_threads;
     fr.frames = s->frames;
@@ -354,6 +358,29 @@
         if (any) occ[i] = prim >= 0 ? 1 : 0;
         else { hits[i].prim = prim; hits[i].t = host[i].y; hits[i].b1 = host[i].z; hits[i].b2 = host[i].w; }
     }
+    return RT_OK;
+}
+static bool packets_possible(const RtScene *s) {
+    return s->accel_kind == RT_ACCEL_KDTREE && !s->has_ext && !s->volume.present && s->dev.cam.type == RT_CAMERA_PERSPECTIVE && !(s->dev.cam.lens_radius > 0.f);
+}
+int rt_trace_camera_packets(RtScene *s, const RtRenderDesc *rd, uint64_t first, uint32_t count, RtHit *hits_out) {
+    if (!s || !rd || !hits_out) return fail(RT_EINVAL, "null argument");
+    if (first % 64u) return fail(RT_EINVAL, "rt_trace_camera_packets: first must be a multiple of 64 (a packet is 64 consecutive work items)");
+    if (!packets_possible(s)) return fail(RT_EINVAL, "rt_trace_camera_packets: needs a kd-tree of triangles, no medium and a perspective camera without a lens");
+    HIPCHK(hipSetDevice(s->device));
+    if (count == 0) return RT_OK;
+    DevFrame fr; int rc = make_frame(s, rd, fr, false); if (rc) return rc;
+    if (first + count > fr.total_work) return fail(RT_EINVAL, "rt_trace_camera_packets: range beyond the frame's work list");
+    fr.mega_tile = 0;
+    if (fr.shard_count == 1) { fr.tile_w = fr.tile_h = fr.tiles_x = 0; fr.tile_pixels = 1; fr.total_work = fr.total_pixels * fr.spp; }
+    bool fits = false;
+    rc = packet_prepare(s, count, &fits); if (rc) return rc;
+    if (!fits) return fail(RT_ENOMEM, "rt_trace_camera_packets: the hit buffer does not fit the memory budget");
+    HIPCHK(hipMemcpyAsync(s->dev_frame, &fr, sizeof(DevFrame), hipMemcpyHostToDevice, s->stream));
+    rc = packet_launch(s, first, count, fr.packet_budget, s->counting); if (rc) return rc;
+    static_assert(sizeof(RtHit) == sizeof(float4), "a hit record is 16 bytes");
+    HIPCHK(hipMemcpyAsync(hits_out, s->cam_hits, size_t(count) * sizeof(float4), hipMemcpyDeviceToHost, s->stream));
+    HIPCHK(hipStreamSynchronize(s->stream));
     return RT_OK;
 }
 int rt_trace_closest(RtScene *s, const RtRay *rays, uint32_t n, RtHit *hits_out) { return trace_common(s, rays, n, 0, hits_out, nullptr); }
@@ -428,6 +455,7 @@
     HIPCHK(hipMemcpyAsync(s->filter_dev, rd->filter_table, 256 * sizeof(float), hipMemcpyHostToDevice, s->stream));
     { hipError_t pre = hipGetLastError(); if (pre != hipSuccess) return fail(RT_EDEVICE, std::string("pending HIP error before launch: ") + hipGetErrorString(pre)); }
     s->rendered = true;
+    s->pk_waves = 0;
     if (fr.pipeline) {
         rc = render_pipeline(s, rd, fr, vol_levels, vol_nmax, vol_samp_words); if (rc) return rc;
         s->last_weighted = false;
@@ -531,9 +559,16 @@
         HIPCHK(hipMemsetAsync(probe, 0, n_waves * 4 * sizeof(unsigned long long), s->stream));
         fr.probe = probe;
 #endif
+        fr.cam_hits = nullptr;
+        if (fr.packets && packets_possible(s) && !s->counting) {
+            bool fits = false;
+            rc = packet_prepare(s, fr.total_work, &fits); if (rc) return rc;
+            if (fits) fr.cam_hits = s->cam_hits;
+        }
         HIPCHK(hipMemcpyAsync(s->dev_frame, &fr, sizeof(DevFrame), hipMemcpyHostToDevice, s->stream));
         HIPCHK(hipMemsetAsync(s->work_counter, 0, 64 * sizeof(unsigned long long), s->stream));
         HIPCHK(hipEventRecord(s->ev0, s->stream));
+        if (fr.cam_hits) { rc = packet_launch(s, 0, unsigned(fr.total_work), fr.packet_budget, false); if (rc) return rc; }
         hipLaunchKernelGGL(render_kernel_of(variant), dim3(s->grids[variant]), dim3(RT_BLOCK), 0, s->stream,
                            (const DevScene *)s->dev_scene, (const DevFrame *)s->dev_frame);
         HIPCHK(hipGetLastError());
diff --git a/pbrt-v1_amd/csrc/hip/rt_packet.h b/pbrt-v1_amd/csrc/hip/rt_packet.h
--- /dev/null
+++ b/pbrt-v1_amd/csrc/hip/rt_packet.h
@@ -0,0 +1,260 @@
+#pragma once
+#include "rt_leaf_entries.h"
+#include <stdint.h>
+#include <string.h>
+
+#if defined(RT_PK_HOST)
+namespace rt {
+struct PkF2 { float x, y; };
+struct PkF4 { float x, y, z, w; };
+struct PkU2 { unsigned x, y; };
+struct PkU4 { unsigned x, y, z, w; };
+}
+#define PK_DEV static inline
+#define PK_K
+#define PK_G
+#define PK_L
+#define PK_NL 64
+#else
+#include "rt_device.h"
+namespace rt {
+typedef float2 PkF2;
+typedef float4 PkF4;
+typedef uint2 PkU2;
+typedef uint4 PkU4;
+}
+#define PK_DEV RT_DEV
+#if defined(__HIP_DEVICE_COMPILE__)
+#define PK_K __attribute__((address_space(4)))
+#else
+#define PK_K
+#endif
+#define PK_G RT_G
+#define PK_L RT_L
+#define PK_NL 1
+#endif
+
+namespace rt {
+
+enum { PK_OK = 0, PK_ABORT_SPLIT = 1, PK_ABORT_BUDGET = 2, PK_ABORT_SPILL = 3 };
+#define RT_PK_ABORTED int(0x80000000u)
+#ifndef RT_PK_RING
+#define RT_PK_RING 24
+#endif
+#define RT_PK_SPILL_CAP 40
+
+#if defined(RT_PK_HOST)
+PK_DEV unsigned pk_f2u(float f) { unsigned u; memcpy(&u, &f, 4); return u; }
+PK_DEV float pk_u2f(unsigned u) { float f; memcpy(&f, &u, 4); return f; }
+PK_DEV int pk_lane(int l) { return l; }
+PK_DEV unsigned pk_uniform(unsigned v) { return v; }
+template <class F> PK_DEV unsigned long long pk_ballot(F f) {
+    unsigned long long m = 0;
+    for (int l = 0; l < 64; ++l) if (f(l)) m |= 1ull << l;
+    return m;
+}
+#else
+PK_DEV unsigned pk_f2u(float f) { return __float_as_uint(f); }
+PK_DEV float pk_u2f(unsigned u) { return __uint_as_float(u); }
+PK_DEV int pk_lane(int) { return int(__lane_id()); }
+PK_DEV unsigned pk_uniform(unsigned v) { return unsigned(__builtin_amdgcn_readfirstlane(int(v))); }
+template <class F> PK_DEV unsigned long long pk_ballot(F f) { return __ballot(f(0)); }
+#endif
+#define PK_FOR(l) for (int l = 0; l < PK_NL; ++l)
+#define PK_BIT(l) (1ull << pk_lane(l))
+
+struct PkTree {
+    const PkU2 PK_K *tnodes;
+    const PkF4 PK_K *ltris;
+    const unsigned PK_K *lrefs;
+    unsigned leaf_runs, n_tris;
+    float bounds[6];
+};
+
+struct PkStack {
+    PkU4 PK_L *hdr;
+    PkF2 PK_L *tm;
+    int ns;
+    PkU4 PK_G *spill;
+    PkU4 PK_G *pool;
+    unsigned PK_G *next_area;
+    unsigned n_areas, cap;
+    int sp, sbase, top, bslot;
+};
+
+template <int NL> struct PkLanes {
+    float ox[NL], oy[NL], oz[NL], dx[NL], dy[NL], dz[NL], ix[NL], iy[NL], iz[NL];
+    float mint[NL], maxt[NL], tmin[NL], tmax[NL], b1[NL], b2[NL];
+    int prim[NL];
+    unsigned c_nodes[NL], c_refs[NL], c_tris[NL];
+};
+
+PK_DEV float pk_sel(unsigned axis, float x, float y, float z) { return axis == 0u ? x : (axis == 1u ? y : z); }
+
+PK_DEV bool pk_spill_alloc(PkStack &S) {
+    if (!S.pool || S.cap == 0u) return false;
+    unsigned idx = 0u;
+#if defined(RT_PK_HOST)
+    idx = (*S.next_area)++;
+#else
+    if (__lane_id() == 0u) idx = atomicAdd((unsigned *)S.next_area, 1u);
+    idx = pk_uniform(idx);
+#endif
+    if (idx >= S.n_areas) return false;
+    S.spill = S.pool + size_t(idx) * S.cap * 64u;
+    return true;
+}
+
+template <int NL>
+PK_DEV bool pk_push(PkStack &S, unsigned node, unsigned long long mask, const float (&tmin_e)[NL], const float (&tmax_e)[NL]) {
+    if (S.sp - S.sbase == S.ns) {
+        if (!S.spill && !pk_spill_alloc(S)) return false;
+        if (unsigned(S.sbase) >= S.cap) return false;
+        const PkU4 h = S.hdr[S.bslot];
+        const unsigned long long hm = (unsigned long long)h.z << 32 | h.y;
+        PK_FOR(l) {
+            const PkF2 t = S.tm[S.bslot * 64 + pk_lane(l)];
+            PkU4 r; r.x = pk_f2u(t.x); r.y = pk_f2u(t.y); r.z = h.x; r.w = unsigned((hm >> pk_lane(l)) & 1ull);
+            S.spill[size_t(S.sbase) * 64u + unsigned(pk_lane(l))] = r;
+        }
+        S.bslot = S.bslot + 1 == S.ns ? 0 : S.bslot + 1;
+        ++S.sbase;
+    }
+    PkU4 h; h.x = node; h.y = unsigned(mask); h.z = unsigned(mask >> 32); h.w = 0u;
+    S.hdr[S.top] = h;
+    PK_FOR(l) { PkF2 t; t.x = tmin_e[l]; t.y = tmax_e[l]; S.tm[S.top * 64 + pk_lane(l)] = t; }
+    S.top = S.top + 1 == S.ns ? 0 : S.top + 1;
+    ++S.sp;
+    return true;
+}
+template <int NL>
+PK_DEV void pk_pop(PkStack &S, unsigned &node, unsigned long long &mask, float (&tmin_e)[NL], float (&tmax_e)[NL]) {
+    if (S.sp > S.sbase) {
+        S.top = S.top == 0 ? S.ns - 1 : S.top - 1;
+        --S.sp;
+        const PkU4 h = S.hdr[S.top];
+        node = pk_uniform(h.x);
+        mask = (unsigned long long)pk_uniform(h.z) << 32 | pk_uniform(h.y);
+        PK_FOR(l) { const PkF2 t = S.tm[S.top * 64 + pk_lane(l)]; tmin_e[l] = t.x; tmax_e[l] = t.y; }
+    } else {
+        --S.sp; --S.sbase;
+        unsigned nd[NL], in[NL];
+        PK_FOR(l) {
+            const PkU4 r = S.spill[size_t(S.sp) * 64u + unsigned(pk_lane(l))];
+            tmin_e[l] = pk_u2f(r.x); tmax_e[l] = pk_u2f(r.y); nd[l] = r.z; in[l] = r.w;
+        }
+        node = pk_uniform(nd[0]);
+        mask = pk_ballot([&](int l) { return in[l] != 0u; });
+    }
+}
+
+template <int NL, bool COUNT>
+PK_DEV int pk_walk(const PkTree &T, PkStack &S, PkLanes<NL> &L, unsigned long long valid, unsigned budget) {
+    S.sp = S.sbase = S.top = S.bslot = 0;
+    unsigned long long mask = pk_ballot([&](int l) {
+        float t0 = L.mint[l], t1 = L.maxt[l];
+        bool ok = true;
+        for (int i = 0; i < 3; ++i) {
+            const float o = pk_sel(unsigned(i), L.ox[l], L.oy[l], L.oz[l]), d = pk_sel(unsigned(i), L.dx[l], L.dy[l], L.dz[l]);
+            const float invRayDir = 1.f / d;
+            float tNear = (T.bounds[i] - o) * invRayDir, tFar = (T.bounds[3 + i] - o) * invRayDir;
+            if (tNear > tFar) { const float tmp = tNear; tNear = tFar; tFar = tmp; }
+            t0 = tNear > t0 ? tNear : t0;
+            t1 = tFar < t1 ? tFar : t1;
+            if (t0 > t1) ok = false;
+        }
+        L.tmin[l] = t0; L.tmax[l] = t1;
+        L.ix[l] = 1.f / L.dx[l]; L.iy[l] = 1.f / L.dy[l]; L.iz[l] = 1.f / L.dz[l];
+        L.prim[l] = -1; L.b1[l] = 0.f; L.b2[l] = 0.f;
+        if (COUNT) { L.c_nodes[l] = 0u; L.c_refs[l] = 0u; L.c_tris[l] = 0u; }
+        return ok;
+    }) & valid;
+    if (T.n_tris == 0u) mask = 0ull;
+    unsigned long long done = ~mask;
+    unsigned node = 0u, steps = 0u;
+    for (;;) {
+        const unsigned long long dead = pk_ballot([&](int l) { return L.maxt[l] < L.tmin[l]; }) & mask;
+        done |= dead; mask &= ~dead;
+        bool descend = false;
+        if (mask) {
+            if (++steps > budget) return PK_ABORT_BUDGET;
+            const PkU2 nd = T.tnodes[pk_uniform(node)];
+            if (COUNT) PK_FOR(l) L.c_nodes[l] += (mask & PK_BIT(l)) ? 1u : 0u;
+            const unsigned axis = nd.x & 3u;
+            if (axis != 3u) {
+                const float split = pk_u2f(nd.x);
+                float tp[NL], e_tmin[NL], e_tmax[NL];
+                PK_FOR(l) {
+                    const float oa = pk_sel(axis, L.ox[l], L.oy[l], L.oz[l]), ia = pk_sel(axis, L.ix[l], L.iy[l], L.iz[l]);
+                    tp[l] = (split - oa) * ia;
+                }
+                const unsigned long long m_eq = pk_ballot([&](int l) { return pk_sel(axis, L.ox[l], L.oy[l], L.oz[l]) == split; }) & mask;
+                const unsigned long long m_bf = pk_ballot([&](int l) { return pk_sel(axis, L.ox[l], L.oy[l], L.oz[l]) < split; }) & mask;
+                if (m_eq || (m_bf && m_bf != mask)) return PK_ABORT_SPLIT;
+                const bool belowFirst = m_bf != 0ull;
+                const unsigned below = node + 1u, above = nd.y;
+                const unsigned first = belowFirst ? below : above, second = belowFirst ? above : below;
+                const unsigned long long m_of = pk_ballot([&](int l) { return tp[l] > L.tmax[l] || tp[l] <= 0.f; }) & mask;
+                const unsigned long long m_os = pk_ballot([&](int l) { return tp[l] < L.tmin[l]; }) & mask & ~m_of;
+                const unsigned long long m_both = mask & ~m_of & ~m_os;
+                const unsigned long long m_first = mask & ~m_os, m_second = mask & ~m_of;
+                if (m_first && m_second) {
+                    PK_FOR(l) { e_tmin[l] = (m_both & PK_BIT(l)) ? tp[l] : L.tmin[l]; e_tmax[l] = L.tmax[l]; }
+                    if (!pk_push<NL>(S, second, m_second, e_tmin, e_tmax)) return PK_ABORT_SPILL;
+                }
+                PK_FOR(l) L.tmax[l] = (m_both & PK_BIT(l)) ? tp[l] : L.tmax[l];
+                if (m_first) { node = first; mask = m_first; } else { node = second; mask = m_second; }
+                descend = true;
+            } else {
+                unsigned cur = (nd.x >> 2) | (nd.y & ~RT_LE_POS);
+                unsigned cursor = (nd.y & RT_LE_POS) << ((nd.y >> 30) & 1u);
+                const bool multi = (nd.y & RT_LE_MORE) != 0u;
+                while (cur != RT_LE_NONE) {
+                    const PkF4 PK_K *gt = T.ltris + (cur & RT_LE_POS);
+                    const PkF4 q0 = gt[0], q1 = gt[1], q2 = gt[2];
+                    unsigned nxt;
+                    if (T.leaf_runs) { nxt = cursor > 1u ? cur + RT_TRI_STRIDE : RT_LE_NONE; cursor -= 1u; }
+                    else {
+                        const bool list = cur >= (RT_LE_MORE | RT_LE_LIST);
+                        unsigned nx = 0u;
+                        if (list) nx = T.lrefs[cursor];
+                        nxt = list ? nx : (int(cur) < 0 ? cursor : RT_LE_NONE);
+                        cursor += list ? 1u : 0u;
+                    }
+                    const int prim = int(pk_f2u(q2.w));
+                    PK_FOR(l) {
+                        if (!(mask & PK_BIT(l))) continue;
+                        if (COUNT) { L.c_tris[l] += 1u; L.c_refs[l] += multi ? 1u : 0u; }
+                        const float p1x = q0.x, p1y = q0.y, p1z = q0.z, e1x = q0.w, e1y = q1.x, e1z = q1.y, e2x = q1.z, e2y = q1.w, e2z = q2.x;
+                        const float dx = L.dx[l], dy = L.dy[l], dz = L.dz[l];
+                        const float s1x = (dy * e2z) - (dz * e2y), s1y = (dz * e2x) - (dx * e2z), s1z = (dx * e2y) - (dy * e2x);
+                        const float divisor = s1x * e1x + s1y * e1y + s1z * e1z;
+                        const float invDivisor = 1.f / divisor;
+                        const float ddx = L.ox[l] - p1x, ddy = L.oy[l] - p1y, ddz = L.oz[l] - p1z;
+                        const float b1 = (ddx * s1x + ddy * s1y + ddz * s1z) * invDivisor;
+                        const float s2x = (ddy * e1z) - (ddz * e1y), s2y = (ddz * e1x) - (ddx * e1z), s2z = (ddx * e1y) - (ddy * e1x);
+                        const float b2 = (dx * s2x + dy * s2y + dz * s2z) * invDivisor;
+                        const float t = (e2x * s2x + e2y * s2y + e2z * s2z) * invDivisor;
+                        const bool miss = (divisor == 0.f) | (b1 < 0.f) | (b1 > 1.f) | (b2 < 0.f) | (b1 + b2 > 1.f) | (t < L.mint[l]) | (t > L.maxt[l]);
+                        if (!miss) { L.prim[l] = prim; L.maxt[l] = t; L.b1[l] = b1; L.b2[l] = b2; }
+                    }
+                    cur = nxt;
+                }
+            }
+        }
+        if (!descend) {
+            for (;;) {
+                if (S.sp == 0) return PK_OK;
+                float e_tmin[NL], e_tmax[NL];
+                unsigned long long e_mask;
+                pk_pop<NL>(S, node, e_mask, e_tmin, e_tmax);
+                mask = e_mask & ~done;
+                if (!mask) continue;
+                PK_FOR(l) if (mask & PK_BIT(l)) { L.tmin[l] = e_tmin[l]; L.tmax[l] = e_tmax[l]; }
+                break;
+            }
+        }
+    }
+}
+
+}
diff --git a/pbrt-v1_amd/csrc/hip/rt_packet.hip b/pbrt-v1_amd/csrc/hip/rt_packet.hip
--- /dev/null
+++ b/pbrt-v1_amd/csrc/hip/rt_packet.hip
@@ -0,0 +1,114 @@
+#include "rt_host.h"
+#include "rt_packet.h"
+
+namespace rt {
+
+struct PkJob {
+    unsigned long long first;
+    unsigned count;
+    float4 *hits;
+    uint4 *pool;
+    unsigned *ctl;
+    unsigned n_areas, cap, budget;
+    unsigned long long *counters;
+};
+
+template <bool COUNT>
+__global__ __launch_bounds__(RT_BLOCK) void primary_packet_kernel(const DevScene *__restrict__ scp, const DevFrame *__restrict__ frp, PkJob job) {
+    __shared__ uint4 ring_hdr[(RT_BLOCK / 64) * RT_PK_RING];
+    __shared__ float2 ring_tm[(RT_BLOCK / 64) * RT_PK_RING * 64];
+    const DevScene &sc = *scp;
+    const DevFrame &fr = *frp;
+    const unsigned wv = threadIdx.x >> 6;
+    const unsigned long long i = (unsigned long long)blockIdx.x * RT_BLOCK + threadIdx.x;
+    const unsigned long long w = job.first + i;
+    const bool in_range = i < job.count;
+    bool ok = in_range;
+    Ray ray; ray.o = mk3(0.f); ray.d = mk3(0.f, 0.f, 1.f); ray.mint = 0.f; ray.maxt = 0.f;
+    if (in_range) {
+        unsigned long long pixel; int s;
+        if (fr.mega_tile > 0) { unsigned px; tile_order_to_sample(fr, unsigned(w), px, s); pixel = px; }
+        else ok = work_to_sample(fr, w, pixel, s);
+        if (ok) { Lane ln; setup_sample(sc, fr, ln, pixel, s, ray); }
+    }
+    PkTree T;
+    T.tnodes = (const PkU2 PK_K *)sc.tnodes; T.ltris = (const PkF4 PK_K *)sc.ltris; T.lrefs = (const unsigned PK_K *)sc.lrefs;
+    T.leaf_runs = sc.leaf_runs; T.n_tris = sc.n_tris;
+#pragma unroll
+    for (int k = 0; k < 6; ++k) T.bounds[k] = sc.bounds[k];
+    PkStack S;
+    S.hdr = (PkU4 PK_L *)ring_hdr + wv * RT_PK_RING; S.tm = (PkF2 PK_L *)ring_tm + wv * RT_PK_RING * 64; S.ns = RT_PK_RING;
+    S.spill = nullptr; S.pool = RT_GPTR(PkU4, job.pool); S.next_area = RT_GPTR(unsigned, job.ctl); S.n_areas = job.n_areas; S.cap = job.cap;
+    PkLanes<1> L;
+    L.ox[0] = ray.o.x; L.oy[0] = ray.o.y; L.oz[0] = ray.o.z; L.dx[0] = ray.d.x; L.dy[0] = ray.d.y; L.dz[0] = ray.d.z;
+    L.mint[0] = ray.mint; L.maxt[0] = ray.maxt;
+    const unsigned long long valid = __ballot(ok);
+    const int st = pk_walk<1, COUNT>(T, S, L, valid, job.budget);
+    float4 RT_G *out = RT_GPTR(float4, job.hits) + i;
+    if (st != PK_OK) {
+        if (in_range) *out = make_float4(__int_as_float(RT_PK_ABORTED), 0.f, 0.f, 0.f);
+        if ((threadIdx.x & 63u) == 0u) atomicAdd(job.ctl + 1, 1u);
+        return;
+    }
+    if (in_range) *out = make_float4(__int_as_float(L.prim[0]), L.prim[0] >= 0 ? L.maxt[0] : 0.f, L.b1[0], L.b2[0]);
+    if (COUNT) {
+        unsigned long long v[3] = {ok ? L.c_nodes[0] : 0u, ok ? L.c_refs[0] : 0u, ok ? L.c_tris[0] : 0u};
+#pragma unroll
+        for (int k = 0; k < 3; ++k) {
+            unsigned long long x = v[k];
+            for (int off = 32; off > 0; off >>= 1) x += __shfl_down(x, off);
+            if ((threadIdx.x & 63u) == 0u && x) atomicAdd(job.counters + 3 + k, x);
+        }
+    }
+}
+
+}
+
+int packet_prepare(RtScene *s, unsigned long long count, bool *fits) {
+    *fits = false;
+    const size_t need = size_t((count + 63) / 64 * 64);
+    if (need == 0 || count > 0xffffffffull) return RT_OK;
+    if (need > s->cam_hits_cap) {
+        size_t free_b = 0, total_b = 0;
+        HIPCHK(hipMemGetInfo(&free_b, &total_b));
+        size_t budget = (free_b + s->cam_hits_cap * sizeof(float4)) / 2;
+        if (const char *e = knob("PBRT_HIP_PIPE_MEM_MB")) budget = size_t(std::max(1, std::atoi(e))) << 20;
+        if (need * sizeof(float4) > budget) return RT_OK;
+        int rc = ensure(s, &s->cam_hits, &s->cam_hits_cap, need); if (rc) return rc;
+    }
+    const size_t areas = std::min<size_t>(need / 64, 4096);
+    {
+        int rc = ensure(s, &s->pk_pool, &s->pk_pool_cap, areas * RT_PK_SPILL_CAP * 64); if (rc) return rc;
+    }
+    if (!s->pk_ctl) { HIPCHK(hipMalloc((void **)&s->pk_ctl, 2 * sizeof(unsigned))); HIPCHK(hipEventCreate(&s->pk_ev0)); HIPCHK(hipEventCreate(&s->pk_ev1)); }
+    *fits = true;
+    return RT_OK;
+}
+
+int packet_launch(RtScene *s, unsigned long long first, unsigned count, unsigned budget, bool counting) {
+    PkJob job{};
+    job.first = first; job.count = count; job.hits = s->cam_hits; job.pool = s->pk_pool; job.ctl = s->pk_ctl;
+    job.n_areas = unsigned(s->pk_pool_cap / (size_t(RT_PK_SPILL_CAP) * 64)); job.cap = RT_PK_SPILL_CAP; job.budget = budget; job.counters = s->counters;
+    HIPCHK(hipMemsetAsync(s->pk_ctl, 0, 2 * sizeof(unsigned), s->stream));
+    HIPCHK(hipEventRecord(s->pk_ev0, s->stream));
+    const unsigned grid = (count + RT_BLOCK - 1) / RT_BLOCK;
+    if (counting) hipLaunchKernelGGL(primary_packet_kernel<true>, dim3(grid), dim3(RT_BLOCK), 0, s->stream, (const DevScene *)s->dev_scene, (const DevFrame *)s->dev_frame, job);
+    else hipLaunchKernelGGL(primary_packet_kernel<false>, dim3(grid), dim3(RT_BLOCK), 0, s->stream, (const DevScene *)s->dev_scene, (const DevFrame *)s->dev_frame, job);
+    HIPCHK(hipGetLastError());
+    HIPCHK(hipEventRecord(s->pk_ev1, s->stream));
+    s->pk_waves = (count + 63u) / 64u;
+    return RT_OK;
+}
+
+extern "C" int rt_last_packet_stats(RtScene *s, RtPacketStats *out) {
+    if (!s || !out) return fail(RT_EINVAL, "null argument");
+    std::memset(out, 0, sizeof *out);
+    if (!s->pk_waves) return RT_OK;
+    HIPCHK(hipSetDevice(s->device));
+    HIPCHK(hipEventSynchronize(s->pk_ev1));
+    unsigned ctl[2] = {0u, 0u};
+    HIPCHK(hipMemcpy(ctl, s->pk_ctl, sizeof ctl, hipMemcpyDeviceToHost));
+    out->waves = s->pk_waves; out->aborted = ctl[1]; out->spill_areas = ctl[0];
+    HIPCHK(hipEventElapsedTime(&out->ms, s->pk_ev0, s->pk_ev1));
+    return RT_OK;
+}
diff --git a/pbrt-v1_amd/csrc/hip/rt_render_kernel.h b/pbrt-v1_amd/csrc/hip/rt_render_kernel.h
--- a/pbrt-v1_amd/csrc/hip/rt_render_kernel.h
+++ b/pbrt-v1_amd/csrc/hip/rt_render_kernel.h
@@ -1,5 +1,6 @@
 #pragma once
 #include "rt_integrate.h"
+#include "rt_packet.h"
 
 namespace rt {
 
@@ -49,6 +50,7 @@
     const unsigned gtid = blockIdx.x * RT_BLOCK + threadIdx.x;
     const int lane = threadIdx.x & 63;
     constexpr bool BYV = RT_MEGA_BYV != 0 && !POOL && INTEG == RT_INTEGRATOR_PATH && !VOL && !EXT && !COUNT;
+    constexpr bool PACKETS = !COUNT && !VOL && !EXT && ACCEL == RT_ACCEL_KDTREE && INTEG != RT_INTEG_DIRECT_WEIGHTED;
     Lane ln;
     ln.vf = 0u;
     ln.stage = ST_FETCH; ln.has_ray = false; ln.fsp = 0; ln.tv.active = false; ln.tv.hit_prim = -1;
@@ -127,6 +129,14 @@
                             ln.specular = false;
                             if (COUNT) ++c_cam;
                             accel_begin<ACCEL>(ln.tv, sc, ray, false);
+                            if constexpr (PACKETS) {
+                                if (fr.cam_hits) {
+                                    const float4 h = RT_GPTR(const float4, fr.cam_hits)[w];
+                                    if (__float_as_int(h.x) != RT_PK_ABORTED) {
+                                        ln.tv.hit_prim = __float_as_int(h.x); ln.tv.maxt = ln.tv.hit_prim >= 0 ? h.y : ln.tv.maxt; ln.tv.b1 = h.z; ln.tv.b2 = h.w; ln.tv.active = false;
+                                    }
+                                }
+                            }
                             if (VOL) vol_store_ray(fr, 0, gtid, ray);
                             ln.has_ray = true; ln.stage = ST_VERTEX;
                             if (BYV) ln.vf = BV_B | BV_CUR_B;
diff --git a/pbrt-v1_amd/csrc/hip/rt_scene.hip b/pbrt-v1_amd/csrc/hip/rt_scene.hip
--- a/pbrt-v1_amd/csrc/hip/rt_scene.hip
+++ b/pbrt-v1_amd/csrc/hip/rt_scene.hip
@@ -564,6 +564,11 @@
     if (s->wt_recbase) HIPWARN(hipFree(s->wt_recbase));
     if (s->wt_rec) HIPWARN(hipFree(s->wt_rec));
     if (s->wt_pick) HIPWARN(hipFree(s->wt_pick));
+    if (s->cam_hits) HIPWARN(hipFree(s->cam_hits));
+    if (s->pk_pool) HIPWARN(hipFree(s->pk_pool));
+    if (s->pk_ctl) HIPWARN(hipFree(s->pk_ctl));
+    if (s->pk_ev0) HIPWARN(hipEventDestroy(s->pk_ev0));
+    if (s->pk_ev1) HIPWARN(hipEventDestroy(s->pk_ev1));
     if (s->wt_total) HIPWARN(hipHostFree(s->wt_total));
     if (s->wt_sums) HIPWARN(hipFree(s->wt_sums));
     for (hipEvent_t e : s->wt_ev) if (e) HIPWARN(hipEventDestroy(e));
```

Result: slower. 2135 (-37.5%).
